# weiji14/deepbedmap

Measured on NVIDIA B200. Metric: continent inference output Mpx/s, higher is better.
Workload: dtype bf16 (fp32 accumulate, fp32 residual stream)

## Files before the change

### deepbedmap_b200/_lib.py

```python
from __future__ import annotations

import ctypes
import os
from typing import Optional

_HERE = os.path.dirname(os.path.abspath(__file__))
LIB_PATH = os.environ.get("DEEPBEDMAP_B200_LIB") or os.path.join(_HERE, "libdeepbedmap_b200.so")

_P, _L, _I, _F = ctypes.c_void_p, ctypes.c_long, ctypes.c_int, ctypes.c_float

SIGNATURES = {
    "dbm_version": [],
    "dbm_launch_count": [],
    "dbm_set_sm_reserve": [_I],
    "dbm_set_deterministic": [_I],
    "dbm_conv2d_fwd_f32": [_P, _L, _P, _P, _P, _L, _I, _I, _I, _I, _I, _I, _I, _I, _I, _P],
    "dbm_conv2d_bwd_data_f32": [_P, _L, _P, _P, _L, _I, _I, _I, _I, _I, _I, _I, _I, _I, _P],
    "dbm_conv2d_bwd_weight_f32": [_P, _L, _P, _L, _P, _I, _I, _I, _I, _I, _I, _I, _I, _P],
    "dbm_bias_grad_f32": [_P, _L, _P, _I, _I, _I, _P],
    "dbm_gemm_f32": [_P, _L, _L, _L, _P, _L, _L, _L, _P, _L, _L, _L, _P, _I, _I, _I, _I, _I, _I, _P],
    "dbm_gemm_bf16": [_P, _L, _L, _L, _P, _L, _L, _L, _P, _L, _L, _L, _P, _I, _I, _I, _I, _I, _I, _P],
    "dbm_axpby_f32": [_P, _L, _P, _L, _P, _L, _F, _F, _I, _L, _P],
    "dbm_lrelu_fwd_f32": [_P, _P, _L, _P],
    "dbm_lrelu_bwd_f32": [_P, _L, _P, _L, _P, _L, _I, _L, _I, _P],
    "dbm_upsample2_fwd_f32": [_P, _P, _L, _I, _I, _P],
    "dbm_upsample2_bwd_f32": [_P, _P, _L, _I, _I, _P],
    "dbm_fill_f32": [_P, _F, _L, _P],
    "dbm_nchw_to_slab8": [_P, _L, _P, _I, _I, _I, _I, _I, _I, _P],
    "dbm_slab8_to_nchw": [_P, _I, _I, _P, _L, _I, _I, _I, _I, _P],
    "dbm_nchw_to_slab4": [_P, _L, _P, _I, _I, _I, _I, _P],
    "dbm_slab4_to_nchw": [_P, _P, _L, _I, _I, _I, _I, _I, _P],
    "dbm_pack_conv3x3_weights": [_P, _P, _I, _I, _I, _I, _P],
    "dbm_pack_conv3x3_weights_slice": [_P, _I, _I, _P, _I, _I, _I, _I, _I, _P],
    "dbm_pack_conv3x3_table": [_P, _I, _L, _P],
    "dbm_trunk_umma": [_P, _I, _I, _I, _I, _P, _I, _P, _P, _I, _P, _P],
    "dbm_trunk_umma_split": [_P, _I, _I, _I, _I, _P, _I, _P, _P, _I, _P, _P],
    "dbm_nchw_to_slab8_split": [_P, _L, _P, _I, _I, _I, _I, _P],
    "dbm_slab8f_to_nchw": [_P, _P, _L, _I, _I, _I, _I, _P],
    "dbm_flat_geometry": [_I, _I, _I, _P],
    "dbm_flat_conv3x3_seq": [_P, _I, _I, _I, _I, _I, _I, _P],
    "dbm_flat_conv3x3_chain": [_P, _P, _I, _I, _I, _I, _I, _I, _P, _P],
    "dbm_trunk_local_fwd": [_P, _I, _I, _I, _I, _P, _P, _P, _P],
    "dbm_trunk_local_bwd": [_P, _I, _I, _I, _I, _P, _P, _P],
    "dbm_flat_wgrad": [_P, _I, _I, _I, _I, _P],
    "dbm_flat_wgrad_ctas": [_P, _I, _I, _I, _I, _I, _P],
    "dbm_flat_wgrad_reduce": [_P, _I, _P],
    "dbm_flat_bias_grad": [_P, _I, _I, _I, _I, _P],
    "dbm_flat_from_nchw": [_P, _I, _P, _P, _F, _I, _I, _I, _P],
    "dbm_flat_to_nchw": [_P, _P, _P, _I, _I, _I, _I, _P],
    "dbm_flat_from_nchw_ex": [_P, _I, _I, _I, _I, _P, _P, _F, _I, _I, _I, _P],
    "dbm_flat_to_nchw_ex": [_P, _P, _P, _I, _I, _I, _I, _I, _I, _I, _P],
    "dbm_transpose_f32": [_P, _P, _I, _I, _P],
    "dbm_stem_fwd_slab8": [_P, _P, _P, _P, _P, _P, _P, _P, _I, _I, _I, _I, _I, _P],
    "dbm_stem_w1_s2d": [_P, _P, _I, _I, _I, _P],
    "dbm_pack_stem_w1": [_P, _P, _P],
    "dbm_conv3x3_umma_valid": [_P, _I, _I, _P, _P, _I, _I, _I, _P, _I, _I, _P],
    "dbm_stem_fwd_flat": [_P, _P, _P, _P, _P, _P, _P, _P, _I, _I, _I, _P],
    "dbm_deform_conv_umma": [_P, _P, _I, _P, _P, _I, _I, _I, _I, _P, _I, _I, _P, _P, _P],
    "dbm_deform_conv_umma_nchw": [_P, _P, _P, _P, _I, _I, _I, _I, _P, _P],
    "dbm_deform_sample_slab8_f32": [_P, _P, _P, _I, _I, _I, _P],
    "dbm_deform_out1_sample": [_P, _P, _I, _P, _P, _I, _I, _I, _P],
    "dbm_deform_conv_out1": [_P, _P, _I, _P, _P, _P, _P, _I, _I, _I, _P],
    "dbm_conv3x3_umma": [_P, _I, _I, _P, _P, _I, _I, _I, _I, _F, _I, _I, _P, _I, _I, _P, _I, _I, _P, _P, _P],
    "dbm_deform_sample_f32": [_P, _P, _P, _I, _I, _I, _I, _P],
    "dbm_deform_bwd_f32": [_P, _P, _P, _P, _P, _I, _I, _I, _I, _P],
    "dbm_deform1_fwd_f32": [_P, _P, _P, _P, _P, _P, _I, _I, _I, _I, _P],
    "dbm_deform1_bwd_f32": [_P, _P, _P, _P, _P, _P, _P, _I, _P, _P, _I, _I, _I, _I, _P],
    "dbm_bn_lrelu_fwd_f32": [_P, _P, _P, _P, _P, _P, _P, _P, _I, _I, _I, _F, _F, _I, _P],
    "dbm_bn_lrelu_bwd_f32": [_P, _P, _P, _P, _P, _P, _P, _P, _P, _P, _I, _I, _I, _P],
    "dbm_bn_lrelu_fwd_groups_f32": [_P, _P, _P, _P, _P, _P, _P, _P, _I, _I, _I, _I, _F, _F, _I, _P],
    "dbm_bn_lrelu_bwd_groups_f32": [_P, _P, _P, _P, _P, _P, _P, _P, _P, _P, _I, _I, _I, _I, _P],
    "dbm_ragan_loss_f32": [_P, _P, _I, _F, _F, _F, _P, _P, _P, _P],
    "dbm_gen_image_loss_f32": [_P, _P, _P, _I, _I, _I, _F, _F, _F, _P, _P, _P],
    "dbm_adam_step_f32": [_P, _P, _P, _P, _L, _F, _F, _F, _F, _I, _F, _P],
    "dbm_adam_step_dev_f32": [_P, _P, _P, _P, _L, _F, _F, _F, _F, _P, _F, _P],
    "dbm_crop_clip_f32": [_P, _I, _I, _P, _I, _I, _I, _I, _I, _I, _P],
    "dbm_place_tile_f32": [_P, _I, _I, _I, _I, _P, _I, _I, _I, _I, _I, _I, _P],
    "dbm_f32_to_i16": [_P, _P, _L, _P],
    "dbm_copy2d_async": [_P, ctypes.c_size_t, _P, ctypes.c_size_t, ctypes.c_size_t, ctypes.c_size_t, _P],
    "dbm_gather_rows_f32": [_P, _L, _P, _P, _L, _I, _P],
    "dbm_gen_create": [_I, _F, _I, ctypes.POINTER(_P)],
    "dbm_gen_destroy": [_P],
    "dbm_gen_count_params": [_P],
    "dbm_gen_num_arrays": [_P],
    "dbm_gen_array_info": [_P, _I, ctypes.POINTER(ctypes.c_char_p), ctypes.POINTER(_I), ctypes.POINTER(_I),
                           ctypes.POINTER(_L)],
    "dbm_gen_set_param": [_P, ctypes.c_char_p, _P, _I, ctypes.POINTER(_I)],
    "dbm_gen_bind_params": [_P, _P],
    "dbm_gen_mark_updated": [_P],
    "dbm_gen_set_precision": [_P, _I],
    "dbm_gen_workspace_bytes": [_P, _I, _I, _I],
    "dbm_gen_forward": [_P, _P, _P, _P, _P, _I, _I, _I, _P, _P, ctypes.c_size_t, _P],
}
TUNING_SIGNATURES = {
    "dbm_debug_set": [_I, _I],
    "dbm_debug_set_ptr": [_I, _P],
    "dbm_flat_debug_set": [_I, _I],
    "dbm_local_debug_set": [_I],
}
RESTYPES = {"dbm_launch_count": _L, "dbm_gen_count_params": _L, "dbm_gen_num_arrays": _I, "dbm_gen_workspace_bytes": ctypes.c_size_t}

_lib: Optional[ctypes.CDLL] = None
launch_count = 0


class DeepBedMapError(RuntimeError):
    pass


def load() -> ctypes.CDLL:
    global _lib
    if _lib is not None:
        return _lib
    if not os.path.exists(LIB_PATH):
        raise DeepBedMapError(
            f"{LIB_PATH} is missing: build it with `python -m deepbedmap_b200.build` "
            "(nvcc, sm_100a). deepbedmap_b200 has no CPU or PyTorch fallback.")
    lib = ctypes.CDLL(LIB_PATH)
    lib.dbm_last_error.restype = ctypes.c_char_p
    lib.dbm_last_error.argtypes = []
    for name, args in list(SIGNATURES.items()) + list(TUNING_SIGNATURES.items()):
        try:
            fn = getattr(lib, name)
        except AttributeError:
            if os.environ.get("DEEPBEDMAP_B200_LIB"):
                continue
            raise
        fn.argtypes = args
        fn.restype = RESTYPES.get(name, ctypes.c_int)
    _lib = lib
    return lib


def kernel_launches() -> int:
    return int(load().dbm_launch_count())


def call(name: str, *args) -> None:
    global launch_count
    lib = load()
    rc = getattr(lib, name)(*args)
    launch_count += 1
    if rc != 0:
        msg = lib.dbm_last_error().decode("utf-8", "replace")
        if rc == -1:
            raise ValueError(f"{name}: {msg}")
        raise DeepBedMapError(f"{name}: {msg}")
```

### deepbedmap_b200/build.py

```python
from __future__ import annotations

import hashlib
import os
import shutil
import subprocess
import sys

HERE = os.path.dirname(os.path.abspath(__file__))
CSRC = os.path.join(HERE, "csrc")
INCLUDE = os.path.join(os.path.dirname(HERE), "include")
LIB = os.path.join(HERE, "libdeepbedmap_b200.so")
TUNING_LIB = os.path.join(HERE, "libdeepbedmap_b200_tuning.so")
STAMP = os.path.join(HERE, "build", "stamp.txt")

SOURCES = ["ops.cu", "gemm_f32.cu", "gemm_bf16.cu", "umma_conv3x3.cu", "umma_trunk.cu", "umma_flat.cu", "umma_local.cu", "umma_deform.cu", "stem.cu", "deform_f32.cu", "train_ops.cu", "gen_api.cu"]
TUNING_SOURCES = ["debug_bench.cu"]
NVCC_FLAGS = [
    "-O3", "-std=c++17", "-gencode", "arch=compute_100a,code=sm_100a", "-lineinfo", "-Xcompiler", "-fPIC"]


def _nvcc() -> str:
    cand = shutil.which("nvcc") or "/usr/local/cuda/bin/nvcc"
    if not os.path.exists(cand):
        raise RuntimeError("nvcc not found; cannot build libdeepbedmap_b200.so")
    return cand


def _digest() -> str:
    h = hashlib.sha256()
    files = [os.path.join(CSRC, f) for f in sorted(os.listdir(CSRC))] + [os.path.join(INCLUDE, "deepbedmap_b200.h")]
    for f in files:
        with open(f, "rb") as fh:
            h.update(f.encode())
            h.update(fh.read())
    h.update(" ".join(NVCC_FLAGS).encode())
    return h.hexdigest()


def build(force: bool = False, verbose: bool = False) -> str:
    os.makedirs(os.path.join(HERE, "build"), exist_ok=True)
    digest = _digest()
    if not force and os.path.exists(LIB) and os.path.exists(STAMP) and open(STAMP).read().strip() == digest:
        return LIB
    nvcc = _nvcc()
    objs = []
    procs = []
    for src in SOURCES:
        obj = os.path.join(HERE, "build", src.replace(".cu", ".o"))
        cmd = [nvcc, *NVCC_FLAGS, "-I", INCLUDE, "-c", os.path.join(CSRC, src), "-o", obj]
        if verbose:
            cmd.insert(1, "-Xptxas")
            cmd.insert(2, "-v")
        procs.append((src, subprocess.Popen(cmd, stdout=subprocess.PIPE, stderr=subprocess.STDOUT, text=True)))
        objs.append(obj)
    for src, p in procs:
        out, _ = p.communicate()
        if verbose or p.returncode:
            sys.stderr.write(out)
        if p.returncode:
            raise RuntimeError(f"nvcc failed on {src}")
    cmd = [nvcc, "-shared", "-gencode", "arch=compute_100a,code=sm_100a", "-o", LIB, *objs]
    subprocess.run(cmd, check=True)
    for src in TUNING_SOURCES:
        cmd = [nvcc, *NVCC_FLAGS, "-shared", "-I", INCLUDE, os.path.join(CSRC, src), "-o", TUNING_LIB, "-L", HERE,
               "-ldeepbedmap_b200", "-Xlinker", "-rpath", "-Xlinker", "$ORIGIN"]
        subprocess.run(cmd, check=True)
    with open(STAMP, "w") as fh:
        fh.write(digest)
    return LIB


if __name__ == "__main__":
    print(build(force="--force" in sys.argv, verbose="-v" in sys.argv))
```

### deepbedmap_b200/csrc/common.cuh

```cuda
#pragma once
#include <cuda.h>
#include <cuda_bf16.h>
#include <cuda_runtime.h>
#include <stdint.h>
#include <stdio.h>

#include "../../include/deepbedmap_b200.h"

namespace dbm {

void set_error(const char* fmt, ...);
int check_launch(const char* what);

#define DBM_REQUIRE(cond, ...)            \
  do {                                    \
    if (!(cond)) {                        \
      ::dbm::set_error(__VA_ARGS__);      \
      return DBM_ERR_INVALID;             \
    }                                     \
  } while (0)

#define DBM_CUDA(expr)                                                          \
  do {                                                                          \
    cudaError_t _e = (expr);                                                    \
    if (_e != cudaSuccess) {                                                    \
      ::dbm::set_error("%s failed: %s", #expr, cudaGetErrorString(_e));         \
      return DBM_ERR_CUDA;                                                      \
    }                                                                           \
  } while (0)

constexpr float kLreluSlope = 0.2f;

__device__ __forceinline__ float lrelu(float v) { return v >= 0.f ? v : v * kLreluSlope; }

static inline int ceil_div(long a, long b) { return (int)((a + b - 1) / b); }

int num_sms();
bool deterministic();
int det_scratch(size_t bytes, void** out);
int resident_ctas(const void* kernel, int threads, size_t smem, int* resident);
int ensure_dyn_smem(const void* kernel, size_t smem);

__device__ __forceinline__ uint32_t smem_u32(const void* p) {
  return static_cast<uint32_t>(__cvta_generic_to_shared(p));
}

__device__ __forceinline__ void mbar_init(uint64_t* bar, uint32_t count) {
  asm volatile("mbarrier.init.shared::cta.b64 [%0], %1;" ::"r"(smem_u32(bar)), "r"(count));
}
__device__ __forceinline__ void fence_mbar_init() {
  asm volatile("fence.mbarrier_init.release.cluster;" ::: "memory");
}
__device__ __forceinline__ void fence_proxy_async_smem() {
  asm volatile("fence.proxy.async.shared::cta;" ::: "memory");
}
__device__ __forceinline__ void mbar_arrive_expect_tx(uint64_t* bar, uint32_t bytes) {
  asm volatile("mbarrier.arrive.expect_tx.shared::cta.b64 _, [%0], %1;" ::"r"(smem_u32(bar)),
               "r"(bytes)
               : "memory");
}
__device__ __forceinline__ void mbar_arrive(uint64_t* bar) {
  asm volatile("mbarrier.arrive.shared::cta.b64 _, [%0];" ::"r"(smem_u32(bar)) : "memory");
}
__device__ __forceinline__ bool mbar_try_wait(uint64_t* bar, uint32_t parity) {
  uint32_t ok;
  asm volatile(
      "{\n\t.reg .pred p;\n\t"
      "mbarrier.try_wait.parity.shared::cta.b64 p, [%1], %2;\n\t"
      "selp.u32 %0, 1, 0, p;\n\t}"
      : "=r"(ok)
      : "r"(smem_u32(bar)), "r"(parity)
      : "memory");
  return ok != 0;
}
__device__ __forceinline__ unsigned long long globaltimer_ns() {
  unsigned long long t;
  asm volatile("mov.u64 %0, %%globaltimer;" : "=l"(t));
  return t;
}
struct SpinGuard {
  uint32_t spins = 0;
  unsigned long long t0 = 0;
  __device__ __forceinline__ bool expired() {
    if ((++spins & 1023u) != 0) return false;
    const unsigned long long now = globaltimer_ns();
    if (t0 == 0) { t0 = now; return false; }
    return now - t0 > 20000000000ull;
  }
};

__device__ __forceinline__ void mbar_wait(uint64_t* bar, uint32_t parity) {
  uint32_t spins = 0;
  while (!mbar_try_wait(bar, parity)) {
    if (++spins > (1u << 26)) {
      printf("dbm: mbarrier wait timeout block %d thread %d\n", blockIdx.x, threadIdx.x);
      __trap();
    }
  }
}

__device__ __forceinline__ void tma_prefetch_desc(const void* tmap) {
  asm volatile("prefetch.tensormap [%0];" ::"l"(tmap) : "memory");
}
__device__ __forceinline__ void tma_load_4d(void* dst, const void* tmap, uint64_t* bar, int c0, int c1,
                                            int c2, int c3) {
  asm volatile(
      "cp.async.bulk.tensor.4d.shared::cluster.global.tile.mbarrier::complete_tx::bytes "
      "[%0], [%1, {%3, %4, %5, %6}], [%2];" ::"r"(smem_u32(dst)),
      "l"(tmap), "r"(smem_u32(bar)), "r"(c0), "r"(c1), "r"(c2), "r"(c3)
      : "memory");
}
__device__ __forceinline__ void bulk_load(void* dst, const void* src, uint32_t bytes, uint64_t* bar) {
  asm volatile(
      "cp.async.bulk.shared::cluster.global.mbarrier::complete_tx::bytes [%0], [%1], %2, [%3];" ::"r"(
          smem_u32(dst)),
      "l"(src), "r"(bytes), "r"(smem_u32(bar))
      : "memory");
}

template <uint32_t kCols>
__device__ __forceinline__ void tmem_alloc(uint32_t* dst_smem) {
  asm volatile("tcgen05.alloc.cta_group::1.sync.aligned.shared::cta.b32 [%0], %1;" ::"r"(
                   smem_u32(dst_smem)),
               "n"(kCols)
               : "memory");
  asm volatile("tcgen05.relinquish_alloc_permit.cta_group::1.sync.aligned;" ::: "memory");
}
template <uint32_t kCols>
__device__ __forceinline__ void tmem_dealloc(uint32_t taddr) {
  asm volatile("tcgen05.dealloc.cta_group::1.sync.aligned.b32 %0, %1;" ::"r"(taddr), "n"(kCols)
               : "memory");
}
__device__ __forceinline__ void tc_fence_before() {
  asm volatile("tcgen05.fence::before_thread_sync;" ::: "memory");
}
__device__ __forceinline__ void tc_fence_after() {
  asm volatile("tcgen05.fence::after_thread_sync;" ::: "memory");
}
__device__ __forceinline__ void umma_bf16(uint32_t d_tmem, uint64_t adesc, uint64_t bdesc, uint32_t idesc,
                                          uint32_t accumulate) {
  asm volatile(
      "{\n\t.reg .pred p;\n\t"
      "setp.ne.b32 p, %4, 0;\n\t"
      "tcgen05.mma.cta_group::1.kind::f16 [%0], %1, %2, %3, p;\n\t}" ::"r"(d_tmem),
      "l"(adesc), "l"(bdesc), "r"(idesc), "r"(accumulate)
      : "memory");
}
template <uint32_t kAOff, uint32_t kBOff>
__device__ __forceinline__ void umma_bf16_off(uint32_t d_tmem, uint32_t a_lo, uint32_t a_hi, uint32_t b_lo,
                                              uint32_t b_hi, uint32_t idesc, uint32_t accumulate) {
  asm volatile(
      "{\n\t.reg .pred p;\n\t.reg .b32 alo, blo;\n\t.reg .b64 ad, bd;\n\t"
      "setp.ne.b32 p, %6, 0;\n\t"
      "add.u32 alo, %1, %7;\n\t"
      "add.u32 blo, %3, %8;\n\t"
      "mov.b64 ad, {alo, %2};\n\t"
      "mov.b64 bd, {blo, %4};\n\t"
      "tcgen05.mma.cta_group::1.kind::f16 [%0], ad, bd, %5, p;\n\t}" ::"r"(d_tmem),
      "r"(a_lo), "r"(a_hi), "r"(b_lo), "r"(b_hi), "r"(idesc), "r"(accumulate), "n"(kAOff), "n"(kBOff)
      : "memory");
}
__device__ __forceinline__ void umma_commit(uint64_t* bar) {
  asm volatile("tcgen05.commit.cta_group::1.mbarrier::arrive::one.shared::cluster.b64 [%0];" ::"r"(
                   smem_u32(bar))
               : "memory");
}
__device__ __forceinline__ void tmem_ld_32x32b_x32(uint32_t taddr, uint32_t (&r)[32]) {
  asm volatile(
      "tcgen05.ld.sync.aligned.32x32b.x32.b32 "
      "{%0, %1, %2, %3, %4, %5, %6, %7, %8, %9, %10, %11, %12, %13, %14, %15, "
      "%16, %17, %18, %19, %20, %21, %22, %23, %24, %25, %26, %27, %28, %29, %30, %31}, [%32];"
      : "=r"(r[0]), "=r"(r[1]), "=r"(r[2]), "=r"(r[3]), "=r"(r[4]), "=r"(r[5]), "=r"(r[6]), "=r"(r[7]),
        "=r"(r[8]), "=r"(r[9]), "=r"(r[10]), "=r"(r[11]), "=r"(r[12]), "=r"(r[13]), "=r"(r[14]),
        "=r"(r[15]), "=r"(r[16]), "=r"(r[17]), "=r"(r[18]), "=r"(r[19]), "=r"(r[20]), "=r"(r[21]),
        "=r"(r[22]), "=r"(r[23]), "=r"(r[24]), "=r"(r[25]), "=r"(r[26]), "=r"(r[27]), "=r"(r[28]),
        "=r"(r[29]), "=r"(r[30]), "=r"(r[31])
      : "r"(taddr)
      : "memory");
}
__device__ __forceinline__ void tmem_wait_ld() {
  asm volatile("tcgen05.wait::ld.sync.aligned;" ::: "memory");
}

__device__ __forceinline__ bool elect_one_sync() {
  uint32_t pred = 0;
  asm volatile(
      "{\n\t.reg .pred P1;\n\t"
      "elect.sync _|P1, 0xFFFFFFFF;\n\t"
      "@P1 mov.s32 %0, 1;\n\t}"
      : "+r"(pred));
  return pred != 0;
}
__device__ __forceinline__ uint64_t make_desc(uint32_t lo, uint32_t hi) {
  return ((uint64_t)hi << 32) | (uint64_t)lo;
}
__device__ __forceinline__ uint32_t desc_lo(uint32_t saddr, uint32_t lbo_bytes) {
  return ((saddr & 0x3FFFFu) >> 4) | (((lbo_bytes >> 4) & 0x3FFFu) << 16);
}
__host__ __device__ constexpr uint32_t desc_hi(uint32_t sbo_bytes) {
  return ((sbo_bytes >> 4) & 0x3FFFu) | (1u << 14);
}

__device__ __forceinline__ uint64_t umma_desc_kmajor_noswz(uint32_t saddr, uint32_t lbo_bytes,
                                                           uint32_t sbo_bytes) {
  uint64_t d = 0;
  d |= (uint64_t)((saddr & 0x3FFFFu) >> 4);
  d |= (uint64_t)((lbo_bytes >> 4) & 0x3FFF) << 16;
  d |= (uint64_t)((sbo_bytes >> 4) & 0x3FFF) << 32;
  d |= (uint64_t)1 << 46;
  return d;
}
__host__ __device__ constexpr uint32_t umma_idesc_bf16(uint32_t M, uint32_t N) {
  return (1u << 4) | (1u << 7) | (1u << 10) | ((N >> 3) << 17) | ((M >> 4) << 24);
}

}
```

### deepbedmap_b200/csrc/gen_api.cu

```cuda
#include <cstring>
#include <map>
#include <string>
#include <vector>

#include "umma_common.cuh"

namespace dbm {

struct GenParam {
  std::string key;
  int ndim;
  int dims[4];
  long off, n;
};

struct ImageRef {
  size_t off = 0;
};

struct Gen {
  int nb = 12, inter = 32;
  float beta = 0.1f;
  int dev = 0;
  std::vector<GenParam> params;
  std::map<std::string, int> index;
  long total = 0;
  float* flat = nullptr;
  bool owns_flat = false;
  uint8_t* arena = nullptr;
  size_t arena_bytes = 0;
  PackEntry* pack_dev = nullptr;
  int pack_n = 0;
  long pack_max = 0;
  bool stale = true;
  std::map<std::string, size_t> img;
  size_t off_wts = 0, off_bias128 = 0, off_w1tc = 0, off_bias_off1 = 0, off_bias_off2 = 0;
  int precision = 0;
  uint8_t* arena_s = nullptr;
  size_t arena_s_bytes = 0;
  PackEntry* pack_s_dev = nullptr;
  int pack_s_n = 0;
  long pack_s_max = 0;
  bool stale_s = true;
  std::map<std::string, size_t> img_s;
  const void* tab_ws = nullptr;
  int tab_n = 0, tab_h = 0, tab_w = 0, tab_layers = 0, tab_precision = -1;
  bool tab_paired = false;
  std::vector<TrunkLayer> tab_host;
};

static const float* P(const Gen* g, const std::string& key) {
  auto it = g->index.find(key);
  return it == g->index.end() ? nullptr : g->flat + g->params[it->second].off;
}

static void add_param(Gen* g, const std::string& key, int d0, int d1 = 0, int d2 = 0, int d3 = 0) {
  GenParam p;
  p.key = key;
  p.dims[0] = d0; p.dims[1] = d1; p.dims[2] = d2; p.dims[3] = d3;
  p.ndim = d1 == 0 ? 1 : 4;
  p.n = p.ndim == 1 ? d0 : (long)d0 * d1 * d2 * d3;
  p.off = g->total;
  g->total += p.n;
  g->index[key] = (int)g->params.size();
  g->params.push_back(p);
}

static void build_inventory(Gen* g) {
  const int ic = g->inter;
  const char* stem[4] = {"X", "W1", "W2", "W3"};
  const int sc[4] = {1, 1, 2, 1}, sk[4] = {3, 30, 6, 3};
  for (int i = 0; i < 4; ++i) {
    add_param(g, std::string("input_block/conv_on_") + stem[i] + "/W", 32, sc[i], sk[i], sk[i]);
    add_param(g, std::string("input_block/conv_on_") + stem[i] + "/b", 32);
  }
  add_param(g, "pre_residual_conv_layer/W", 64, 128, 3, 3);
  add_param(g, "pre_residual_conv_layer/b", 64);
  for (int i = 0; i < g->nb; ++i)
    for (int r = 1; r <= 3; ++r) {
      const std::string pre = "residual_network/" + std::to_string(i) + "/residual_dense_block" + std::to_string(r);
      for (int k = 1; k <= 4; ++k) {
        add_param(g, pre + "/conv_layer" + std::to_string(k) + "/W", ic, 64 + (k - 1) * ic, 3, 3);
        add_param(g, pre + "/conv_layer" + std::to_string(k) + "/b", ic);
      }
      add_param(g, pre + "/conv_layer5/W", 64, 64 + 4 * ic, 3, 3);
      add_param(g, pre + "/conv_layer5/b", 64);
    }
  const char* plain[3] = {"post_residual_conv_layer", "post_upsample_conv_layer_1", "post_upsample_conv_layer_2"};
  for (int i = 0; i < 3; ++i) {
    add_param(g, std::string(plain[i]) + "/W", 64, 64, 3, 3);
    add_param(g, std::string(plain[i]) + "/b", 64);
  }
  const char* fin[2] = {"final_conv_layer1", "final_conv_layer2"};
  const int oc[2] = {64, 1};
  for (int i = 0; i < 2; ++i) {
    add_param(g, std::string(fin[i]) + "/offset_conv/W", 18, 64, 3, 3);
    add_param(g, std::string(fin[i]) + "/offset_conv/b", 18);
    add_param(g, std::string(fin[i]) + "/deform_conv/W", oc[i], 64, 3, 3);
    add_param(g, std::string(fin[i]) + "/deform_conv/b", oc[i]);
  }
}

static std::string rdb_prefix(int i, int r) {
  return "residual_network/" + std::to_string(i) + "/residual_dense_block" + std::to_string(r);
}

static int build_pack_plan(Gen* g) {
  std::vector<PackEntry> ent;
  size_t off = 0;
  auto image = [&](const std::string& name, int cin, int coutp) {
    g->img[name] = off;
    off += ((size_t)9 * cin * coutp * 2 + 255) & ~(size_t)255;
    return g->img[name];
  };
  auto entry = [&](const std::string& wkey, size_t img_off, int O, int o0, int cin, int cin_total, int c0, int coutp,
                   int ck) {
    PackEntry e;
    e.w = P(g, wkey);
    e.out = (__nv_bfloat16*)img_off;
    e.O = O; e.o0 = o0; e.Cin = cin; e.CinTotal = cin_total; e.c0 = c0; e.COUTP = coutp; e.CK = ck; e.mode = 0;
    ent.push_back(e);
  };
  const int ic = g->inter;
  entry("pre_residual_conv_layer/W", image("pre", 128, 64), 64, 0, 128, 128, 0, 64, 16);
  for (int i = 0; i < g->nb; ++i)
    for (int r = 1; r <= 3; ++r) {
      const std::string pre = rdb_prefix(i, r);
      for (int k = 1; k <= 4; ++k) {
        const int cin = 64 + (k - 1) * ic;
        entry(pre + "/conv_layer" + std::to_string(k) + "/W", image(pre + "/c" + std::to_string(k), cin, ic), ic, 0, cin,
              cin, 0, ic, 16);
      }
      entry(pre + "/conv_layer5/W", image(pre + "/c5", 64 + 4 * ic, 64), 64, 0, 64 + 4 * ic, 64 + 4 * ic, 0, 64, 16);
      if (ic == 32)
        for (int k = 1; k <= 3; k += 2) {
          const int cin = 64 + (k - 1) * 32;
          const std::string wa = pre + "/conv_layer" + std::to_string(k) + "/W";
          const std::string wb = pre + "/conv_layer" + std::to_string(k + 1) + "/W";
          const size_t both = image(pre + "/pair" + std::to_string(k), cin, 64);
          entry(wa, both, 32, 0, cin, cin, 0, 64, 16);
          entry(wb, both, 32, 32, cin, cin + 32, 0, 64, 16);
          entry(wb, image(pre + "/tail" + std::to_string(k + 1), 32, 32), 32, 0, 32, cin + 32, cin, 32, 16);
        }
    }
  entry("post_residual_conv_layer/W", image("post", 64, 64), 64, 0, 64, 64, 0, 64, 16);
  entry("post_upsample_conv_layer_1/W", image("up1", 64, 64), 64, 0, 64, 64, 0, 64, 32);
  entry("post_upsample_conv_layer_2/W", image("up2", 64, 64), 64, 0, 64, 64, 0, 64, 32);
  entry("final_conv_layer1/offset_conv/W", image("off1", 64, 32), 18, 0, 64, 64, 0, 32, 32);
  entry("final_conv_layer2/offset_conv/W", image("off2", 64, 32), 18, 0, 64, 64, 0, 32, 32);
  entry("final_conv_layer1/deform_conv/W", image("dc1", 64, 64), 64, 0, 64, 64, 0, 64, 64);
  auto raw = [&](size_t bytes) {
    const size_t o = off;
    off += (bytes + 255) & ~(size_t)255;
    return o;
  };
  g->off_wts = raw(90 * 32 * 4);
  g->off_bias128 = raw(128 * 4);
  g->off_w1tc = raw((size_t)9 * 320 * 32 * 2);
  g->off_bias_off1 = raw(32 * 4);
  g->off_bias_off2 = raw(32 * 4);
  g->arena_bytes = off;
  DBM_CUDA(cudaMalloc(&g->arena, g->arena_bytes));
  DBM_CUDA(cudaMemset(g->arena, 0, g->arena_bytes));
  long mx = 0;
  for (auto& e : ent) {
    e.out = (__nv_bfloat16*)(g->arena + (size_t)e.out);
    const long el = (long)9 * e.Cin * e.COUTP;
    if (el > mx) mx = el;
  }
  g->pack_n = (int)ent.size();
  g->pack_max = mx;
  DBM_CUDA(cudaMalloc(&g->pack_dev, ent.size() * sizeof(PackEntry)));
  DBM_CUDA(cudaMemcpy(g->pack_dev, ent.data(), ent.size() * sizeof(PackEntry), cudaMemcpyHostToDevice));
  return DBM_OK;
}

static int refresh_packed(Gen* g, cudaStream_t st) {
  if (!g->stale) return DBM_OK;
  int rc = dbm_pack_conv3x3_table(g->pack_dev, g->pack_n, g->pack_max, st);
  if (rc) return rc;
  float* wts = (float*)(g->arena + g->off_wts);
  float* bias128 = (float*)(g->arena + g->off_bias128);
  if ((rc = dbm_transpose_f32(P(g, "input_block/conv_on_X/W"), wts, 32, 9, st))) return rc;
  if ((rc = dbm_transpose_f32(P(g, "input_block/conv_on_W2/W"), wts + 9 * 32, 32, 72, st))) return rc;
  if ((rc = dbm_transpose_f32(P(g, "input_block/conv_on_W3/W"), wts + 81 * 32, 32, 9, st))) return rc;
  const char* stem[4] = {"X", "W1", "W2", "W3"};
  for (int i = 0; i < 4; ++i)
    DBM_CUDA(cudaMemcpyAsync(bias128 + 32 * i, P(g, std::string("input_block/conv_on_") + stem[i] + "/b"), 32 * 4,
                             cudaMemcpyDeviceToDevice, st));
  DBM_CUDA(cudaMemcpyAsync(g->arena + g->off_bias_off1, P(g, "final_conv_layer1/offset_conv/b"), 18 * 4,
                           cudaMemcpyDeviceToDevice, st));
  DBM_CUDA(cudaMemcpyAsync(g->arena + g->off_bias_off2, P(g, "final_conv_layer2/offset_conv/b"), 18 * 4,
                           cudaMemcpyDeviceToDevice, st));
  if ((rc = dbm_pack_stem_w1(P(g, "input_block/conv_on_W1/W"), g->arena + g->off_w1tc, st))) return rc;
  g->stale = false;
  return DBM_OK;
}

struct WsLayout {
  size_t s2d, s0, cat[2], a1, f32[3], u1, u2, f1, offs, proj, flags, table, total;
  int num_layers, units;
  bool paired;
};

static WsLayout ws_layout(const Gen* g, int n, int h, int w) {
  WsLayout L;
  const size_t H = h - 2, W = w - 2;
  size_t off = 0;
  auto take = [&](size_t bytes) {
    const size_t o = off;
    off += (bytes + 1023) & ~(size_t)1023;
    return o;
  };
  const size_t px = (size_t)n * H * W;
  const int ccs = (64 + 4 * g->inter) / 8;
  L.s2d = take((size_t)n * 40 * h * w * 16);
  L.s0 = take(px * 16 * 16);
  L.cat[0] = take(px * ccs * 16);
  L.cat[1] = take(px * ccs * 16);
  L.a1 = take(px * 64 * 4);
  for (int i = 0; i < 3; ++i) L.f32[i] = take(px * 64 * 4);
  L.u1 = take(px * 4 * 8 * 16);
  L.u2 = take(px * 16 * 8 * 16);
  L.f1 = take(px * 16 * 8 * 16);
  L.offs = take(px * 16 * 8 * 16);
  L.proj = take(px * 16 * 9 * 4);
  L.paired = g->inter == 32 && ((int)W + 15) / 16 + 2 <= 128;
  L.num_layers = 2 + g->nb * 3 * 5;
  L.units = n * (((int)H + 31) / 32) * (((int)W + 15) / 16);
  L.flags = take((size_t)L.num_layers * L.units * 4);
  L.table = take((size_t)L.num_layers * sizeof(TrunkLayer));
  L.total = off;
  return L;
}

static void build_trunk_table(Gen* g, const WsLayout& L, uint8_t* ws) {
  std::vector<TrunkLayer>& T = g->tab_host;
  T.clear();
  auto bf = [&](size_t o) { return (__nv_bfloat16*)(ws + o); };
  auto f32 = [&](size_t o) { return (float*)(ws + o); };
  auto image = [&](const std::string& name) { return (const __nv_bfloat16*)(g->arena + g->img.at(name)); };
  auto layer = [&](const __nv_bfloat16* wq, const float* bias, int cin, int cout, int in_map, int act, float beta,
                   __nv_bfloat16* out, int out_cs_total, int out_cs0, float* out_f32, const float* res1,
                   const float* res2, int up2, int in_cs0, int cout_main, int mode) {
    TrunkLayer t;
    memset(&t, 0, sizeof(t));
    t.wpacked = wq; t.bias = bias; t.out_bf16 = out; t.out_f32 = out_f32; t.res1 = res1; t.res2 = res2;
    t.stash_out = nullptr;
    t.cin = cin; t.cout = cout; t.in_map = in_map; t.in_cs0 = in_cs0; t.act = act; t.up2 = up2;
    t.out_cs_total = out_cs_total; t.out_cs0 = out_cs0; t.cout_main = cout_main; t.res1_cs_total = 16;
    t.beta = beta; t.mode = mode;
    T.push_back(t);
  };
  const int ic = g->inter, cc = 64 + 4 * ic, ccs = cc / 8;
  __nv_bfloat16* cat[2] = {bf(L.cat[0]), bf(L.cat[1])};
  float* a1 = f32(L.a1);
  float* fb[3] = {f32(L.f32[0]), f32(L.f32[1]), f32(L.f32[2])};
  layer(image("pre"), P(g, "pre_residual_conv_layer/b"), 128, 64, 0, 1, 0.f, cat[0], ccs, 0, a1, nullptr, nullptr, 0, 0,
        64, 0);
  int cur = 0, fi = 0;
  float* cur_f32 = a1;
  for (int i = 0; i < g->nb; ++i) {
    float* rrdb_in = cur_f32;
    for (int r = 1; r <= 3; ++r) {
      const std::string pre = rdb_prefix(i, r);
      auto bias = [&](int k) { return P(g, pre + "/conv_layer" + std::to_string(k) + "/b"); };
      if (L.paired) {
        for (int k = 1; k <= 3; k += 2) {
          const int cin = 64 + (k - 1) * ic;
          layer(image(pre + "/pair" + std::to_string(k)), bias(k), cin, 64, 1 + cur, 1, 0.f, cat[cur], ccs, cin / 8,
                nullptr, nullptr, nullptr, 0, 0, 32, 1);
          layer(image(pre + "/tail" + std::to_string(k + 1)), bias(k + 1), 32, 32, 1 + cur, 1, 0.f, cat[cur], ccs,
                cin / 8 + 4, nullptr, nullptr, nullptr, 0, cin / 8, 32, 2);
        }
      } else {
        for (int k = 1; k <= 4; ++k) {
          const int cin = 64 + (k - 1) * ic;
          layer(image(pre + "/c" + std::to_string(k)), bias(k), cin, ic, 1 + cur, 1, 0.f, cat[cur], ccs, cin / 8, nullptr,
                nullptr, nullptr, 0, 0, ic, 0);
        }
      }
      while (fb[fi] == cur_f32 || fb[fi] == rrdb_in) fi = (fi + 1) % 3;
      float* nxt = fb[fi];
      layer(image(pre + "/c5"), bias(5), cc, 64, 1 + cur, 0, g->beta, cat[1 - cur], ccs, 0, nxt, cur_f32,
            r == 3 ? rrdb_in : nullptr, 0, 0, 64, 0);
      cur = 1 - cur;
      cur_f32 = nxt;
    }
  }
  layer(image("post"), P(g, "post_residual_conv_layer/b"), 64, 64, 1 + cur, 0, 1.f, bf(L.u1), 8, 0, nullptr, a1, nullptr,
        1, 0, 64, 0);
}

static int build_split_pack_plan(Gen* g) {
  if (g->arena_s) return DBM_OK;
  std::vector<PackEntry> ent;
  size_t off = 0;
  auto image = [&](const std::string& name, int cin, int coutp) {
    g->img_s[name] = off;
    off += ((size_t)3 * 9 * cin * coutp * 2 + 255) & ~(size_t)255;
    return g->img_s[name];
  };
  auto entry = [&](const std::string& wkey, size_t img_off, int O, int o0, int cin, int cin_total, int c0, int coutp) {
    PackEntry e;
    e.w = P(g, wkey);
    e.out = (__nv_bfloat16*)img_off;
    e.O = O; e.o0 = o0; e.Cin = cin; e.CinTotal = cin_total; e.c0 = c0; e.COUTP = coutp; e.CK = 16; e.mode = 16;
    ent.push_back(e);
  };
  const int ic = g->inter, cc = 64 + 4 * ic;
  entry("pre_residual_conv_layer/W", image("pre", 128, 64), 64, 0, 128, 128, 0, 64);
  for (int i = 0; i < g->nb; ++i)
    for (int r = 1; r <= 3; ++r) {
      const std::string pre = rdb_prefix(i, r);
      entry(pre + "/conv_layer5/W", image(pre + "/c5", cc, 64), 64, 0, cc, cc, 0, 64);
      if (ic == 32) {
        for (int k = 1; k <= 3; k += 2) {
          const int cin = 64 + (k - 1) * 32;
          const std::string wa = pre + "/conv_layer" + std::to_string(k) + "/W";
          const std::string wb = pre + "/conv_layer" + std::to_string(k + 1) + "/W";
          const size_t both = image(pre + "/pair" + std::to_string(k), cin, 64);
          entry(wa, both, 32, 0, cin, cin, 0, 64);
          entry(wb, both, 32, 32, cin, cin + 32, 0, 64);
          entry(wb, image(pre + "/tail" + std::to_string(k + 1), 32, 32), 32, 0, 32, cin + 32, cin, 32);
        }
      } else {
        for (int k = 1; k <= 4; ++k) {
          const int cin = 64 + (k - 1) * ic;
          entry(pre + "/conv_layer" + std::to_string(k) + "/W", image(pre + "/c" + std::to_string(k), cin, ic), ic, 0, cin,
                cin, 0, ic);
        }
      }
    }
  entry("post_residual_conv_layer/W", image("post", 64, 64), 64, 0, 64, 64, 0, 64);
  entry("post_upsample_conv_layer_1/W", image("up1", 64, 64), 64, 0, 64, 64, 0, 64);
  entry("post_upsample_conv_layer_2/W", image("up2", 64, 64), 64, 0, 64, 64, 0, 64);
  g->arena_s_bytes = off;
  DBM_CUDA(cudaMalloc(&g->arena_s, off));
  DBM_CUDA(cudaMemset(g->arena_s, 0, off));
  long mx = 0;
  for (auto& e : ent) {
    e.out = (__nv_bfloat16*)(g->arena_s + (size_t)e.out);
    const long el = (long)9 * e.Cin * e.COUTP;
    if (el > mx) mx = el;
  }
  g->pack_s_n = (int)ent.size();
  g->pack_s_max = mx;
  DBM_CUDA(cudaMalloc(&g->pack_s_dev, ent.size() * sizeof(PackEntry)));
  DBM_CUDA(cudaMemcpy(g->pack_s_dev, ent.data(), ent.size() * sizeof(PackEntry), cudaMemcpyHostToDevice));
  g->stale_s = true;
  return DBM_OK;
}

struct WsSplit {
  size_t a0, s0, cat[2], a1, f32[3], u1, u2, c2f, c2, off, cols, d1, proj, flags[3], table[3], total;
  int num_layers, units[3];
  bool paired;
};

static WsSplit ws_layout_split(const Gen* g, int n, int h, int w) {
  WsSplit L;
  const size_t H = h - 2, W = w - 2;
  size_t off = 0;
  auto take = [&](size_t bytes) {
    const size_t o = off;
    off += (bytes + 1023) & ~(size_t)1023;
    return o;
  };
  const size_t px = (size_t)n * H * W, px1 = 16 * H * W;
  const int ccs = (64 + 4 * g->inter) / 8;
  L.a0 = take(px * 128 * 4);
  L.s0 = take(px * 32 * 16);
  L.cat[0] = take(px * 2 * ccs * 16);
  L.cat[1] = take(px * 2 * ccs * 16);
  L.a1 = take(px * 64 * 4);
  for (int i = 0; i < 3; ++i) L.f32[i] = take(px * 64 * 4);
  L.u1 = take(px * 4 * 16 * 16);
  L.u2 = take(px * 16 * 16 * 16);
  L.c2f = take(px * 16 * 64 * 4);
  L.c2 = take(px1 * 64 * 4);
  L.off = take(px1 * 18 * 4);
  L.cols = take(px1 * 576 * 4);
  L.d1 = take(px1 * 64 * 4);
  L.proj = take(px1 * 9 * 4);
  L.paired = g->inter == 32 && ((int)W + 15) / 16 + 2 <= 128;
  L.num_layers = 2 + g->nb * 3 * 5;
  for (int i = 0; i < 3; ++i) {
    const int hh = (int)H << i, ww = (int)W << i;
    L.units[i] = n * ((hh + 31) / 32) * ((ww + 15) / 16);
  }
  L.flags[0] = take((size_t)L.num_layers * L.units[0] * 4);
  L.flags[1] = take((size_t)L.units[1] * 4);
  L.flags[2] = take((size_t)L.units[2] * 4);
  L.table[0] = take((size_t)L.num_layers * sizeof(TrunkLayer));
  L.table[1] = take(sizeof(TrunkLayer));
  L.table[2] = take(sizeof(TrunkLayer));
  L.total = off;
  return L;
}

static int build_split_tables(Gen* g, const WsSplit& L, uint8_t* ws, std::vector<TrunkLayer>& T) {
  T.clear();
  auto bf = [&](size_t o) { return (__nv_bfloat16*)(ws + o); };
  auto f32 = [&](size_t o) { return (float*)(ws + o); };
  auto image = [&](const std::string& name) { return (const __nv_bfloat16*)(g->arena_s + g->img_s.at(name)); };
  auto layer = [&](const __nv_bfloat16* wq, const float* bias, int cin, int cout, int in_map, int act, float beta,
                   __nv_bfloat16* out, int out_cs_total, int out_cs0, float* out_f32, const float* res1,
                   const float* res2, int up2, int in_cs0, int cout_main, int mode) {
    TrunkLayer t;
    memset(&t, 0, sizeof(t));
    t.wpacked = wq; t.bias = bias; t.out_bf16 = out; t.out_f32 = out_f32; t.res1 = res1; t.res2 = res2;
    t.cin = cin; t.cout = cout; t.in_map = in_map; t.in_cs0 = in_cs0; t.act = act; t.up2 = up2;
    t.out_cs_total = out_cs_total; t.out_cs0 = out_cs0; t.cout_main = cout_main; t.res1_cs_total = 16;
    t.beta = beta; t.mode = mode;
    T.push_back(t);
  };
  const int ic = g->inter, cc = 64 + 4 * ic, ccs = cc / 8;
  DBM_REQUIRE(L.paired || ic != 32, "gen_forward (bf16x3): tiles wider than ~2000 px are not supported");
  __nv_bfloat16* cat[2] = {bf(L.cat[0]), bf(L.cat[1])};
  float* a1 = f32(L.a1);
  float* fb[3] = {f32(L.f32[0]), f32(L.f32[1]), f32(L.f32[2])};
  layer(image("pre"), P(g, "pre_residual_conv_layer/b"), 128, 64, 0, 1, 0.f, cat[0], ccs, 0, a1, nullptr, nullptr, 0, 0,
        64, 0);
  int cur = 0, fi = 0;
  float* cur_f32 = a1;
  for (int i = 0; i < g->nb; ++i) {
    float* rrdb_in = cur_f32;
    for (int r = 1; r <= 3; ++r) {
      const std::string pre = rdb_prefix(i, r);
      auto bias = [&](int k) { return P(g, pre + "/conv_layer" + std::to_string(k) + "/b"); };
      if (ic == 32) {
        for (int k = 1; k <= 3; k += 2) {
          const int cin = 64 + (k - 1) * ic;
          layer(image(pre + "/pair" + std::to_string(k)), bias(k), cin, 64, 1 + cur, 1, 0.f, cat[cur], ccs, cin / 8,
                nullptr, nullptr, nullptr, 0, 0, 32, 1);
          layer(image(pre + "/tail" + std::to_string(k + 1)), bias(k + 1), 32, 32, 1 + cur, 1, 0.f, cat[cur], ccs,
                cin / 8 + 4, nullptr, nullptr, nullptr, 0, cin / 8, 32, 2);
        }
      } else {
        for (int k = 1; k <= 4; ++k) {
          const int cin = 64 + (k - 1) * ic;
          layer(image(pre + "/c" + std::to_string(k)), bias(k), cin, ic, 1 + cur, 1, 0.f, cat[cur], ccs, cin / 8, nullptr,
                nullptr, nullptr, 0, 0, ic, 0);
        }
// ... 106 lines not shown
  Gen* g = &h->g;
  g->nb = num_residual_blocks; g->beta = residual_scaling; g->inter = inter_channels;
  cudaGetDevice(&g->dev);
  build_inventory(g);
  cudaError_t e = cudaMalloc(&g->flat, (size_t)g->total * 4);
  if (e != cudaSuccess) {
    delete h;
    set_error("gen_create: cudaMalloc of %ld parameters failed: %s", g->total, cudaGetErrorString(e));
    return DBM_ERR_CUDA;
  }
  cudaMemset(g->flat, 0, (size_t)g->total * 4);
  g->owns_flat = true;
  int rc = build_pack_plan(g);
  if (rc) {
    cudaFree(g->flat);
    delete h;
    return rc;
  }
  *out = h;
  return DBM_OK;
}

extern "C" int dbm_gen_destroy(dbm_gen* h) {
  if (!h) return DBM_OK;
  Gen* g = &h->g;
  if (g->owns_flat && g->flat) cudaFree(g->flat);
  if (g->arena) cudaFree(g->arena);
  if (g->pack_dev) cudaFree(g->pack_dev);
  if (g->arena_s) cudaFree(g->arena_s);
  if (g->pack_s_dev) cudaFree(g->pack_s_dev);
  delete h;
  return DBM_OK;
}

extern "C" long dbm_gen_count_params(const dbm_gen* h) { return h ? h->g.total : -1; }
extern "C" int dbm_gen_num_arrays(const dbm_gen* h) { return h ? (int)h->g.params.size() : -1; }

extern "C" int dbm_gen_array_info(const dbm_gen* h, int index, const char** key, int* ndim, int* dims4,
                                  long* flat_offset) {
  DBM_REQUIRE(h && index >= 0 && index < (int)h->g.params.size(), "gen_array_info: bad index %d", index);
  const GenParam& p = h->g.params[index];
  if (key) *key = p.key.c_str();
  if (ndim) *ndim = p.ndim;
  if (dims4)
    for (int i = 0; i < 4; ++i) dims4[i] = p.dims[i];
  if (flat_offset) *flat_offset = p.off;
  return DBM_OK;
}

extern "C" int dbm_gen_set_param(dbm_gen* h, const char* key, const float* host_values, int ndim, const int* dims) {
  DBM_REQUIRE(h && key && host_values && dims, "gen_set_param: null argument");
  Gen* g = &h->g;
  auto it = g->index.find(key);
  DBM_REQUIRE(it != g->index.end(), "gen_set_param: unknown key '%s'", key);
  const GenParam& p = g->params[it->second];
  bool ok = ndim == p.ndim;
  for (int i = 0; ok && i < ndim; ++i) ok = dims[i] == p.dims[i];
  DBM_REQUIRE(ok, "gen_set_param: '%s' has shape (%d,%d,%d,%d), got %d-d (%d,...)", key, p.dims[0], p.dims[1],
              p.dims[2], p.dims[3], ndim, ndim > 0 ? dims[0] : 0);
  DBM_CUDA(cudaMemcpy(g->flat + p.off, host_values, (size_t)p.n * 4, cudaMemcpyHostToDevice));
  g->stale = true;
  g->stale_s = true;
  return DBM_OK;
}

extern "C" int dbm_gen_bind_params(dbm_gen* h, float* device_flat) {
  DBM_REQUIRE(h && device_flat, "gen_bind_params: null argument");
  Gen* g = &h->g;
  DBM_REQUIRE(g->owns_flat, "gen_bind_params: parameters are already bound");
  cudaFree(g->flat);
  std::vector<PackEntry> ent(g->pack_n);
  DBM_CUDA(cudaMemcpy(ent.data(), g->pack_dev, ent.size() * sizeof(PackEntry), cudaMemcpyDeviceToHost));
  for (auto& e : ent) e.w = device_flat + (e.w - g->flat);
  DBM_CUDA(cudaMemcpy(g->pack_dev, ent.data(), ent.size() * sizeof(PackEntry), cudaMemcpyHostToDevice));
  if (g->pack_s_dev) {
    std::vector<PackEntry> es(g->pack_s_n);
    DBM_CUDA(cudaMemcpy(es.data(), g->pack_s_dev, es.size() * sizeof(PackEntry), cudaMemcpyDeviceToHost));
    for (auto& e : es) e.w = device_flat + (e.w - g->flat);
    DBM_CUDA(cudaMemcpy(g->pack_s_dev, es.data(), es.size() * sizeof(PackEntry), cudaMemcpyHostToDevice));
  }
  g->flat = device_flat;
  g->owns_flat = false;
  g->stale = true;
  g->stale_s = true;
  g->tab_ws = nullptr;
  return DBM_OK;
}

extern "C" int dbm_gen_mark_updated(dbm_gen* h) {
  DBM_REQUIRE(h != nullptr, "gen_mark_updated: null handle");
  h->g.stale = true;
  h->g.stale_s = true;
  return DBM_OK;
}

extern "C" int dbm_gen_set_precision(dbm_gen* h, int precision) {
  DBM_REQUIRE(h != nullptr, "gen_set_precision: null handle");
  DBM_REQUIRE(precision == 0 || precision == 1, "gen_set_precision: %d (0 = bf16, 1 = bf16x3)", precision);
  h->g.precision = precision;
  h->g.tab_ws = nullptr;
  return DBM_OK;
}

extern "C" size_t dbm_gen_workspace_bytes(const dbm_gen* h, int n, int h_in, int w_in) {
  if (!h || n <= 0 || h_in < 3 || w_in < 3) return 0;
  if (h->g.precision == 1) return ws_layout_split(&h->g, n, h_in, w_in).total;
  return ws_layout(&h->g, n, h_in, w_in).total;
}

extern "C" int dbm_gen_forward(dbm_gen* h, const float* x, const float* w1, const float* w2, const float* w3, int n,
                               int h_in, int w_in, float* y_out, void* workspace, size_t workspace_bytes,
                               cudaStream_t st) {
  DBM_REQUIRE(h && x && w1 && w2 && w3 && y_out && workspace, "gen_forward: null argument");
  DBM_REQUIRE(n > 0 && h_in >= 3 && w_in >= 3, "gen_forward: input %d x %d x %d too small (need >= 3 x 3)", n, h_in, w_in);
  Gen* g = &h->g;
  DBM_REQUIRE(((uintptr_t)workspace & 1023) == 0, "gen_forward: workspace must be 1024-byte aligned");
  if (g->precision == 1)
    return gen_forward_split(g, x, w1, w2, w3, n, h_in, w_in, y_out, workspace, workspace_bytes, st);
  const WsLayout L = ws_layout(g, n, h_in, w_in);
  DBM_REQUIRE(workspace_bytes >= L.total, "gen_forward: workspace of %zu bytes, need %zu (dbm_gen_workspace_bytes)",
              workspace_bytes, L.total);
  DBM_REQUIRE(((uintptr_t)workspace & 1023) == 0, "gen_forward: workspace must be 1024-byte aligned");
  uint8_t* ws = (uint8_t*)workspace;
  const int H = h_in - 2, W = w_in - 2;
  int rc = refresh_packed(g, st);
  if (rc) return rc;
  if (g->tab_ws != workspace || g->tab_n != n || g->tab_h != h_in || g->tab_w != w_in || g->tab_precision != 0) {
    build_trunk_table(g, L, ws);
    DBM_REQUIRE((int)g->tab_host.size() == L.num_layers, "gen_forward: pass table has %zu entries, expected %d",
                g->tab_host.size(), L.num_layers);
    DBM_CUDA(cudaMemcpyAsync(ws + L.table, g->tab_host.data(), g->tab_host.size() * sizeof(TrunkLayer),
                             cudaMemcpyHostToDevice, st));
    DBM_CUDA(cudaStreamSynchronize(st));
    g->tab_ws = workspace; g->tab_n = n; g->tab_h = h_in; g->tab_w = w_in; g->tab_precision = 0;
  }
  void* s2d = ws + L.s2d;
  void* s0 = ws + L.s0;
  const float* wts = (const float*)(g->arena + g->off_wts);
  const float* bias128 = (const float*)(g->arena + g->off_bias128);
  auto image = [&](const char* name) { return (const void*)(g->arena + g->img.at(name)); };
  if ((rc = dbm_stem_w1_s2d(w1, s2d, n, h_in, w_in, st))) return rc;
  if ((rc = dbm_stem_fwd_slab8(x, nullptr, w2, w3, nullptr, wts, bias128, s0, 16, 0, n, h_in, w_in, st))) return rc;
  if ((rc = dbm_conv3x3_umma_valid(s2d, 40, 320, g->arena + g->off_w1tc, P(g, "input_block/conv_on_W1/b"), n, h_in, w_in,
                                   s0, 16, 4, st)))
    return rc;
  const int ccs = (64 + 4 * g->inter) / 8;
  if ((rc = dbm_trunk_umma(ws + L.table, L.num_layers, n, H, W, s0, 16, ws + L.cat[0], ws + L.cat[1], ccs,
                           (unsigned int*)(ws + L.flags), st)))
    return rc;
  void* u1 = ws + L.u1;
  void* u2 = ws + L.u2;
  void* f1 = ws + L.f1;
  float* offs = (float*)(ws + L.offs);
  if ((rc = dbm_conv3x3_umma(u1, 8, 64, image("up1"), P(g, "post_upsample_conv_layer_1/b"), 64, n, 2 * H, 2 * W, 0.f, 1, 1,
                             u2, 8, 0, nullptr, 0, 0, nullptr, nullptr, st)))
    return rc;
  if ((rc = dbm_conv3x3_umma(u2, 8, 64, image("up2"), P(g, "post_upsample_conv_layer_2/b"), 64, n, 4 * H, 4 * W, 0.f, 1, 0,
                             f1, 8, 0, nullptr, 0, 0, nullptr, nullptr, st)))
    return rc;
  if ((rc = dbm_conv3x3_umma(f1, 8, 64, image("off1"), (const float*)(g->arena + g->off_bias_off1), 32, n, 4 * H, 4 * W,
                             0.f, 0, 0, nullptr, 0, 0, offs, 8, 0, nullptr, nullptr, st)))
    return rc;
  void* d1 = u2;
  if ((rc = dbm_deform_conv_umma(f1, offs, 8, image("dc1"), P(g, "final_conv_layer1/deform_conv/b"), n, 4 * H, 4 * W, 1, d1,
                                 8, 0, nullptr, nullptr, st)))
    return rc;
  if ((rc = dbm_conv3x3_umma(d1, 8, 64, image("off2"), (const float*)(g->arena + g->off_bias_off2), 32, n, 4 * H, 4 * W,
                             0.f, 0, 0, nullptr, 0, 0, offs, 8, 0, nullptr, nullptr, st)))
    return rc;
  return dbm_deform_conv_out1(d1, offs, 8, P(g, "final_conv_layer2/deform_conv/W"), P(g, "final_conv_layer2/deform_conv/b"),
                              y_out, (float*)(ws + L.proj), n, 4 * H, 4 * W, st);
}
```

### deepbedmap_b200/csrc/umma_common.cuh

```cuda
#pragma once
#include <utility>

#include "common.cuh"

namespace dbm {

constexpr int kTile = 16;
constexpr int kHalo = kTile + 2;

int make_slab8_tmap(CUtensorMap* tm, const void* base, int N, int CS, int H, int W, int ck, int box_w = kHalo,
                    int box_h = kHalo);

template <int COUT, int CK, int DSTRIDE, int IDX>
__device__ __forceinline__ void issue_one(uint32_t d0, uint32_t a_lo, uint32_t a_hi, uint32_t b_lo, uint32_t b_hi,
                                          uint32_t idesc, uint32_t acc) {
  constexpr int KS = CK / 16;
  constexpr int j = IDX / KS, ks = IDX % KS;
  constexpr uint32_t a_off = (uint32_t)((2 * ks) * kHalo * kHalo + 8 * j);
  constexpr uint32_t b_off = (uint32_t)((2 * ks) * (COUT / 8) * 8);
  umma_bf16_off<a_off, b_off>(d0 + (uint32_t)(j * DSTRIDE), a_lo, a_hi, b_lo, b_hi, idesc, ks != 0 ? 1u : acc);
}
template <int COUT, int CK, int DSTRIDE, int... IDX>
__device__ __forceinline__ void issue_tap(uint32_t d0, uint32_t a_lo, uint32_t a_hi, uint32_t b_lo, uint32_t b_hi,
                                          uint32_t idesc, uint32_t acc, std::integer_sequence<int, IDX...>) {
  (issue_one<COUT, CK, DSTRIDE, IDX>(d0, a_lo, a_hi, b_lo, b_hi, idesc, acc), ...);
}
template <int COUT, int CK, int DSTRIDE = COUT>
__device__ __forceinline__ void issue_stage_mmas(uint32_t d0, uint32_t a_lo, uint32_t a_hi, uint32_t b_lo,
                                                 uint32_t b_hi, uint32_t idesc, uint32_t acc0) {
  constexpr uint32_t kBTap = (uint32_t)((CK / 8) * (COUT / 8) * 8);
#pragma unroll 1
  for (uint32_t tap = 0; tap < 9; ++tap) {
    const uint32_t a_tap = a_lo + tap + (tap / 3) * (kHalo - 3);
    const uint32_t b_tap = b_lo + tap * kBTap;
    issue_tap<COUT, CK, DSTRIDE>(d0, a_tap, a_hi, b_tap, b_hi, idesc, tap != 0 ? 1u : acc0,
                        std::make_integer_sequence<int, 2 * (CK / 16)>{});
  }
}


struct TrunkLayer {
  const __nv_bfloat16* wpacked;
  const float* bias;
  __nv_bfloat16* out_bf16;
  float* out_f32;
  const float* res1;
  const float* res2;
  float* stash_out;
  int cin, cout;
  int in_map, in_cs0;
  int act, up2;
  int out_cs_total, out_cs0;
  int cout_main, res1_cs_total;
  float beta;
  int mode;
  int pad[6];
};
static_assert(sizeof(TrunkLayer) == 128, "TrunkLayer layout is part of the C ABI");


struct PackEntry {
  const float* w;
  __nv_bfloat16* out;
  int O, o0, Cin, CinTotal, c0, COUTP, CK, mode;
};
static_assert(sizeof(PackEntry) == 48, "PackEntry layout is part of the C ABI");


}
```

### deepbedmap_b200/csrc/umma_conv3x3.cu

```cuda
#include "umma_common.cuh"

namespace dbm {

static int g_debug_swap_lbo_sbo = 0;
static int g_debug_ck16 = 0;
extern int g_trunk_debug;

constexpr int kThreads = 192;

struct UmmaConvParams {
  int N, H, W, Cin;
  int tiles_x, tiles_y, num_items;
  const __nv_bfloat16* wpacked;
  const float* bias;
  float beta;
  int act, up2, swap;
  int in_off;
  __nv_bfloat16* out_bf16;
  int out_cs_total, out_cs0;
  float* out_f32;
  int out_f32_cs_total, out_f32_cs0;
  const float* res1;
  const float* res2;
};
// ... 127 lines not shown
            if (p.res1) {
#pragma unroll
              for (int s4 = 0; s4 < 8; ++s4) {
                const float4 rr = __ldg(reinterpret_cast<const float4*>(
                    p.res1 + ((((size_t)n * (COUT / 4) + (c0 / 4 + s4)) * p.H + y) * p.W + x) * 4));
                v[4 * s4 + 0] = rr.x + p.beta * v[4 * s4 + 0];
                v[4 * s4 + 1] = rr.y + p.beta * v[4 * s4 + 1];
                v[4 * s4 + 2] = rr.z + p.beta * v[4 * s4 + 2];
                v[4 * s4 + 3] = rr.w + p.beta * v[4 * s4 + 3];
              }
            }
            if (p.res2) {
#pragma unroll
              for (int s4 = 0; s4 < 8; ++s4) {
                const float4 rr = __ldg(reinterpret_cast<const float4*>(
                    p.res2 + ((((size_t)n * (COUT / 4) + (c0 / 4 + s4)) * p.H + y) * p.W + x) * 4));
                v[4 * s4 + 0] = rr.x + p.beta * v[4 * s4 + 0];
                v[4 * s4 + 1] = rr.y + p.beta * v[4 * s4 + 1];
                v[4 * s4 + 2] = rr.z + p.beta * v[4 * s4 + 2];
                v[4 * s4 + 3] = rr.w + p.beta * v[4 * s4 + 3];
              }
            }
            if (p.act) {
#pragma unroll
              for (int i = 0; i < 32; ++i) v[i] = lrelu(v[i]);
            }
            if (p.out_f32) {
#pragma unroll
              for (int s4 = 0; s4 < 8; ++s4) {
                float4 o = make_float4(v[4 * s4], v[4 * s4 + 1], v[4 * s4 + 2], v[4 * s4 + 3]);
                *reinterpret_cast<float4*>(
                    p.out_f32 +
                    ((((size_t)n * p.out_f32_cs_total + (p.out_f32_cs0 + c0 / 4 + s4)) * p.H + y) * p.W + x) * 4) = o;
              }
            }
            if (p.out_bf16) {
#pragma unroll
              for (int s8 = 0; s8 < 4; ++s8) {
                uint4 o;
                __nv_bfloat162 t0 = __floats2bfloat162_rn(v[8 * s8 + 0], v[8 * s8 + 1]);
                __nv_bfloat162 t1 = __floats2bfloat162_rn(v[8 * s8 + 2], v[8 * s8 + 3]);
                __nv_bfloat162 t2 = __floats2bfloat162_rn(v[8 * s8 + 4], v[8 * s8 + 5]);
                __nv_bfloat162 t3 = __floats2bfloat162_rn(v[8 * s8 + 6], v[8 * s8 + 7]);
                o.x = *reinterpret_cast<uint32_t*>(&t0);
                o.y = *reinterpret_cast<uint32_t*>(&t1);
                o.z = *reinterpret_cast<uint32_t*>(&t2);
                o.w = *reinterpret_cast<uint32_t*>(&t3);
                const size_t cs = (size_t)n * p.out_cs_total + (p.out_cs0 + c0 / 8 + s8);
                if (!p.up2) {
                  *reinterpret_cast<uint4*>(p.out_bf16 + ((cs * p.H + y) * p.W + x) * 8) = o;
                } else {
                  const int Ho = 2 * p.H, Wo = 2 * p.W;
                  __nv_bfloat16* base = p.out_bf16 + ((cs * Ho + 2 * y) * Wo + 2 * x) * 8;
                  *reinterpret_cast<uint4*>(base) = o;
                  *reinterpret_cast<uint4*>(base + 8) = o;
                  *reinterpret_cast<uint4*>(base + (size_t)Wo * 8) = o;
                  *reinterpret_cast<uint4*>(base + (size_t)Wo * 8 + 8) = o;
                }
              }
            }
          }
        }
      }
      tc_fence_before();
      __syncwarp();
      if (lane == 0) mbar_arrive(&tempty[buf]);
    }
  }

  tc_fence_before();
  __syncthreads();
  if (warp == 1) {
    tc_fence_after();
    tmem_dealloc<Cfg::TMEM_COLS>(tmem_base);
  }
}

typedef CUresult (*PFN_encodeTiled)(CUtensorMap*, CUtensorMapDataType, cuuint32_t, void*, const cuuint64_t*,
                                    const cuuint64_t*, const cuuint32_t*, const cuuint32_t*,
                                    CUtensorMapInterleave, CUtensorMapSwizzle, CUtensorMapL2promotion,
                                    CUtensorMapFloatOOBfill);

static PFN_encodeTiled get_encode() {
  static PFN_encodeTiled fn = nullptr;
  if (!fn) {
    void* p = nullptr;
    cudaDriverEntryPointQueryResult qres;
    if (cudaGetDriverEntryPoint("cuTensorMapEncodeTiled", &p, cudaEnableDefault, &qres) == cudaSuccess &&
        qres == cudaDriverEntryPointSuccess)
      fn = (PFN_encodeTiled)p;
  }
  return fn;
}

int make_slab8_tmap(CUtensorMap* tm, const void* base, int N, int CS, int H, int W, int ck, int box_w, int box_h) {
  PFN_encodeTiled enc = get_encode();
  DBM_REQUIRE(enc != nullptr, "cuTensorMapEncodeTiled entry point not available");
  cuuint64_t dims[4] = {(cuuint64_t)W * 8, (cuuint64_t)H, (cuuint64_t)CS, (cuuint64_t)N};
  cuuint64_t strides[3] = {(cuuint64_t)W * 16, (cuuint64_t)H * W * 16, (cuuint64_t)CS * H * W * 16};
  cuuint32_t box[4] = {(cuuint32_t)box_w * 8, (cuuint32_t)box_h, (cuuint32_t)(ck / 8), 1};
  cuuint32_t estr[4] = {1, 1, 1, 1};
  CUresult r = enc(tm, CU_TENSOR_MAP_DATA_TYPE_BFLOAT16, 4, const_cast<void*>(base), dims, strides, box, estr,
                   CU_TENSOR_MAP_INTERLEAVE_NONE, CU_TENSOR_MAP_SWIZZLE_NONE, CU_TENSOR_MAP_L2_PROMOTION_L2_256B,
                   CU_TENSOR_MAP_FLOAT_OOB_FILL_NONE);
  DBM_REQUIRE(r == CUDA_SUCCESS, "cuTensorMapEncodeTiled failed (%d) for N=%d CS=%d H=%d W=%d", (int)r, N, CS,
              H, W);
  return DBM_OK;
}

template <int COUT, int CK, int STAGES>
static int launch_umma(const CUtensorMap& tm, const UmmaConvParams& p, cudaStream_t st) {
  using Cfg = UmmaCfg<COUT, CK, STAGES>;
  if (int rc = ensure_dyn_smem((const void*)umma_conv3x3_kernel<COUT, CK, STAGES>, Cfg::SMEM)) return rc;
  int grid = p.num_items < num_sms() ? p.num_items : num_sms();
  umma_conv3x3_kernel<COUT, CK, STAGES><<<grid, kThreads, Cfg::SMEM, st>>>(tm, p);
  return check_launch("umma_conv3x3_kernel");
}

__global__ void pack_w3x3_slice_kernel(const float* __restrict__ w, __nv_bfloat16* __restrict__ out, int O, int o0,
                                       int Cin, int CinTotal, int c0, int COUTP, int CK) {
  const long total = (long)9 * Cin * COUTP;
  for (long i = blockIdx.x * (long)blockDim.x + threadIdx.x; i < total; i += (long)gridDim.x * blockDim.x) {
    long t = i;
    const int c8 = t % 8; t /= 8;
    const int o8 = t % 8; t /= 8;
    const int cg = t % (COUTP / 8); t /= (COUTP / 8);
    const int ksl = t % (CK / 8); t /= (CK / 8);
    const int tap = t % 9; t /= 9;
    const int kc = (int)t;
    const int o = cg * 8 + o8 - o0;
    const int c = kc * CK + ksl * 8 + c8;
    if (o >= 0 && o < O) out[i] = __float2bfloat16_rn(w[((long)o * CinTotal + c0 + c) * 9 + tap]);
  }
}

__device__ __forceinline__ void store8_bf16(__nv_bfloat16* dst, const float (&v)[8]) {
  __nv_bfloat162 t0 = __floats2bfloat162_rn(v[0], v[1]);
  __nv_bfloat162 t1 = __floats2bfloat162_rn(v[2], v[3]);
  __nv_bfloat162 t2 = __floats2bfloat162_rn(v[4], v[5]);
  __nv_bfloat162 t3 = __floats2bfloat162_rn(v[6], v[7]);
  uint4 o;
  o.x = *reinterpret_cast<uint32_t*>(&t0);
  o.y = *reinterpret_cast<uint32_t*>(&t1);
  o.z = *reinterpret_cast<uint32_t*>(&t2);
  o.w = *reinterpret_cast<uint32_t*>(&t3);
  *reinterpret_cast<uint4*>(dst) = o;
}

__global__ void pack_w3x3_table_kernel(const PackEntry* __restrict__ table) {
  PackEntry e = table[blockIdx.y];
  const bool split = (e.mode & 16) != 0;
  e.mode &= 15;
  if (split && !(e.mode == 0 && (e.O & 7) == 0 && (e.o0 & 7) == 0 && e.CK == 16)) return;
  if (e.mode == 0 && (e.O & 7) == 0 && (e.o0 & 7) == 0) {
    const int og = e.O / 8;
    const long total = (long)9 * (e.Cin / 8) * e.O;
    for (long i = blockIdx.x * (long)blockDim.x + threadIdx.x; i < total; i += (long)gridDim.x * blockDim.x) {
      long t = i;
      const int o8 = t % 8; t /= 8;
      const int cgl = t % og; t /= og;
      const int ksl = t % (e.CK / 8); t /= (e.CK / 8);
      const int tap = t % 9; t /= 9;
      const int kc = (int)t;
      const int o = cgl * 8 + o8;
      const int c = kc * e.CK + ksl * 8;
      const int kcd = split ? 3 * kc : kc;
      const long dst = ((((long)(kcd * 9 + tap) * (e.CK / 8) + ksl) * (e.COUTP / 8) + (e.o0 / 8 + cgl)) * 8 + o8) * 8;
      const float* src = e.w + ((long)o * e.CinTotal + e.c0 + c) * 9 + tap;
      float v[8];
#pragma unroll
      for (int c8 = 0; c8 < 8; ++c8) v[c8] = src[c8 * 9];
      store8_bf16(e.out + dst, v);
      if (split) {
        const long chunk = (long)9 * (e.CK / 8) * (e.COUTP / 8) * 64;
        store8_bf16(e.out + dst + chunk, v);
#pragma unroll
        for (int c8 = 0; c8 < 8; ++c8) v[c8] -= __bfloat162float(__float2bfloat16_rn(v[c8]));
        store8_bf16(e.out + dst + 2 * chunk, v);
      }
    }
    return;
  }
  const long total = (long)9 * (e.Cin / 8) * e.COUTP;
  for (long i = blockIdx.x * (long)blockDim.x + threadIdx.x; i < total; i += (long)gridDim.x * blockDim.x) {
    long t = i;
    const int o8 = t % 8; t /= 8;
    const int cg = t % (e.COUTP / 8); t /= (e.COUTP / 8);
    const int ksl = t % (e.CK / 8); t /= (e.CK / 8);
    const int tap = t % 9; t /= 9;
    const int kc = (int)t;
    const int on = cg * 8 + o8;
    const int cb = kc * e.CK + ksl * 8;
    float v[8];
    if (e.mode == 0) {
      const int o = on - e.o0;
      if (o < 0 || o >= e.O) continue;
      const float* src = e.w + ((long)o * e.CinTotal + e.c0 + cb) * 9 + tap;
#pragma unroll
      for (int c8 = 0; c8 < 8; ++c8) v[c8] = src[c8 * 9];
      store8_bf16(e.out + i * 8, v);
      continue;
    }
#pragma unroll
    for (int c8 = 0; c8 < 8; ++c8) {
      const int c = cb + c8;
      float x = 0.f;
      if (e.mode == 1) {
        const int kvalid = e.o0 > 0 ? e.o0 : e.Cin;
        if (on < e.O && c < kvalid) x = e.w[((long)c * e.CinTotal + e.c0 + on) * 9 + (8 - tap)];
      } else {
        const int oc = e.mode == 2 ? on : c;
        const int pc = e.mode == 2 ? c : e.c0 + on;
        const int ovalid = e.o0 > 0 ? e.o0 : (e.mode == 2 ? e.O : e.Cin);
        const int t3 = e.mode == 2 ? tap : 8 - tap;
        const int ph = pc / e.CinTotal, cc = pc - ph * e.CinTotal;
        const int ky = 2 * (t3 / 3 - 1) + (ph >> 1) + 1, kx = 2 * (t3 % 3 - 1) + (ph & 1) + 1;
        if (on < e.O && oc < ovalid && ph < 4 && ky >= 0 && ky <= 3 && kx >= 0 && kx <= 3)
          x = e.w[(((long)oc * e.CinTotal + cc) * 4 + ky) * 4 + kx];
      }
      v[c8] = x;
    }
    store8_bf16(e.out + i * 8, v);
  }
}

__global__ void pack_w3x3_kernel(const float* __restrict__ w, __nv_bfloat16* __restrict__ out, int O, int Cin,
                                 int COUTP, int CK) {
  const long total = (long)9 * Cin * COUTP;
  for (long i = blockIdx.x * (long)blockDim.x + threadIdx.x; i < total; i += (long)gridDim.x * blockDim.x) {
    long t = i;
    const int c8 = t % 8; t /= 8;
    const int o8 = t % 8; t /= 8;
    const int cg = t % (COUTP / 8); t /= (COUTP / 8);
    const int ksl = t % (CK / 8); t /= (CK / 8);
    const int tap = t % 9; t /= 9;
    const int kc = (int)t;
    const int o = cg * 8 + o8;
    const int c = kc * CK + ksl * 8 + c8;
    float v = 0.f;
    if (o < O) v = w[((long)o * Cin + c) * 9 + tap];
    out[i] = __float2bfloat16_rn(v);
  }
}

}

using namespace dbm;

extern "C" int dbm_debug_set(int key, int value) {
  if (key == 1) g_debug_swap_lbo_sbo = value;
  if (key == 2) g_debug_ck16 = value;
  if (key == 3) g_trunk_debug = value;
  return DBM_OK;
}

extern "C" int dbm_pack_conv3x3_weights(const float* w_oihw, void* packed_bf16, int cout, int cin, int cout_padded,
                                        int ck, cudaStream_t stream) {
  DBM_REQUIRE(ck == 16 || ck == 32 || ck == 64,
              "pack: K-chunk %d must be 16 / 32 (conv3x3_umma, trunk) or 64 (deform_conv_umma)", ck);
  DBM_REQUIRE(cin % ck == 0, "pack: Cin=%d must be a multiple of %d", cin, ck);
  DBM_REQUIRE(cout_padded == 32 || cout_padded == 64, "pack: padded Cout=%d must be 32 or 64", cout_padded);
  DBM_REQUIRE(cout <= cout_padded, "pack: Cout=%d > padded %d", cout, cout_padded);
  const long total = (long)9 * cin * cout_padded;
  pack_w3x3_kernel<<<ceil_div(total, 256), 256, 0, stream>>>(w_oihw, (__nv_bfloat16*)packed_bf16, cout, cin,
                                                             cout_padded, ck);
  return check_launch("pack_w3x3_kernel");
}

extern "C" int dbm_pack_conv3x3_weights_slice(const float* w_oihw, int w_cin_total, int w_c0, void* packed_bf16,
                                              int cout, int cout0, int cin, int cout_padded, int ck,
                                              cudaStream_t stream) {
  DBM_REQUIRE(ck == 16 || ck == 32 || ck == 64, "pack: K-chunk %d must be 16, 32 or 64", ck);
  DBM_REQUIRE(cin % ck == 0 && w_c0 >= 0 && w_c0 + cin <= w_cin_total, "pack: bad channel slice [%d, %d) of %d",
              w_c0, w_c0 + cin, w_cin_total);
  DBM_REQUIRE(cout_padded % 8 == 0 && cout0 >= 0 && cout0 + cout <= cout_padded, "pack: bad Cout rows [%d, %d) of %d",
              cout0, cout0 + cout, cout_padded);
  const long total = (long)9 * cin * cout_padded;
  pack_w3x3_slice_kernel<<<ceil_div(total, 256), 256, 0, stream>>>(w_oihw, (__nv_bfloat16*)packed_bf16, cout, cout0,
                                                                   cin, w_cin_total, w_c0, cout_padded, ck);
  return check_launch("pack_w3x3_slice_kernel");
}

extern "C" int dbm_pack_conv3x3_table(const void* table_dev, int num_entries, long max_elements,
                                      cudaStream_t stream) {
  DBM_REQUIRE(num_entries > 0 && num_entries <= 65535 && max_elements > 0, "pack table: bad size (%d entries)",
              num_entries);
  DBM_REQUIRE(((uintptr_t)table_dev & 7) == 0, "pack table: unaligned");
  int gx = ceil_div(max_elements / 8, 256 * 2);
  if (gx > 64) gx = 64;
  if (gx < 1) gx = 1;
  pack_w3x3_table_kernel<<<dim3(gx, num_entries), 256, 0, stream>>>((const PackEntry*)table_dev);
  return check_launch("pack_w3x3_table_kernel");
}

extern "C" int dbm_conv3x3_umma(const void* in_slab8, int in_cs_total, int cin, const void* wpacked,
                                const float* bias, int cout_padded, int n, int h, int w, float beta, int act,
                                int up2, void* out_slab8, int out_cs_total, int out_cs0, float* out_f32_slab4,
                                int out_f32_cs_total, int out_f32_cs0, const float* res1_slab4,
                                const float* res2_slab4, cudaStream_t stream) {
  DBM_REQUIRE(cin % 32 == 0 && cin <= in_cs_total * 8, "conv3x3_umma: bad Cin=%d (slabs %d)", cin, in_cs_total);
  DBM_REQUIRE(cout_padded == 32 || cout_padded == 64, "conv3x3_umma: Cout=%d must be 32 or 64", cout_padded);
  DBM_REQUIRE(n > 0 && h > 0 && w > 0, "conv3x3_umma: empty input");
  DBM_REQUIRE(out_slab8 || out_f32_slab4, "conv3x3_umma: no output");
  DBM_REQUIRE(((uintptr_t)in_slab8 & 15) == 0 && ((uintptr_t)wpacked & 15) == 0, "conv3x3_umma: unaligned");
  CUtensorMap tm;
  int rc = make_slab8_tmap(&tm, in_slab8, n, in_cs_total, h, w, 32);
// ... 44 lines not shown
```

### deepbedmap_b200/csrc/umma_local.cu

```cuda
#include "common.cuh"

namespace dbm {

constexpr int kLocThreads = 320;
constexpr int kLocStages = 5;
constexpr int kLocSoloThreads = 192;
constexpr int kLocSoloStages = 3;
constexpr int kLocStageBytes = 96 * 192;
constexpr int kLocSlabs = 24;
constexpr int kLocAcc = 192, kLocXcur = 192, kLocSlot = 256;

enum { kLocPre = 0, kLocAct = 1, kLocRdb = 2, kLocPost = 3,
       kLocBPost = 4, kLocBMask = 5, kLocBD1 = 6, kLocBPre = 7 };

struct LocalPass {
  const __nv_bfloat16* w;
  const float* bias;
  __nv_bfloat16* save;
  float* out_f32;
  const __nv_bfloat16* mask;
  const float* add_f32;
  int slab0, nk, N, col0;
  int type, ecol, out_slab, rr;
  float beta;
  float scale;
  int first;
  int pad;
};
static_assert(sizeof(LocalPass) == 96, "LocalPass layout is part of the C ABI");

struct LocalParams {
  const LocalPass* passes;
  int count;
  int n, H, W, Wp, img, halo, G0, Pg, RA;
  const __nv_bfloat16* s0;
  int in_slabs;
  int group;
  float* x0;
  float* xrr;
};

__device__ __forceinline__ void tmem_st_32x32b_x32(uint32_t taddr, const uint32_t (&r)[32]) {
  asm volatile(
      "tcgen05.st.sync.aligned.32x32b.x32.b32 [%0], "
      "{%1, %2, %3, %4, %5, %6, %7, %8, %9, %10, %11, %12, %13, %14, %15, %16, "
      "%17, %18, %19, %20, %21, %22, %23, %24, %25, %26, %27, %28, %29, %30, %31, %32};" ::"r"(taddr),
      "r"(r[0]), "r"(r[1]), "r"(r[2]), "r"(r[3]), "r"(r[4]), "r"(r[5]), "r"(r[6]), "r"(r[7]), "r"(r[8]), "r"(r[9]),
      "r"(r[10]), "r"(r[11]), "r"(r[12]), "r"(r[13]), "r"(r[14]), "r"(r[15]), "r"(r[16]), "r"(r[17]), "r"(r[18]),
      "r"(r[19]), "r"(r[20]), "r"(r[21]), "r"(r[22]), "r"(r[23]), "r"(r[24]), "r"(r[25]), "r"(r[26]), "r"(r[27]),
      "r"(r[28]), "r"(r[29]), "r"(r[30]), "r"(r[31])
      : "memory");
}
__device__ __forceinline__ void tmem_wait_st() { asm volatile("tcgen05.wait::st.sync.aligned;" ::: "memory"); }

__device__ __forceinline__ uint4 pack8f(const float* v) {
  uint4 o;
  __nv_bfloat162 t0 = __floats2bfloat162_rn(v[0], v[1]);
  __nv_bfloat162 t1 = __floats2bfloat162_rn(v[2], v[3]);
  __nv_bfloat162 t2 = __floats2bfloat162_rn(v[4], v[5]);
  __nv_bfloat162 t3 = __floats2bfloat162_rn(v[6], v[7]);
  o.x = *reinterpret_cast<uint32_t*>(&t0);
  o.y = *reinterpret_cast<uint32_t*>(&t1);
  o.z = *reinterpret_cast<uint32_t*>(&t2);
  o.w = *reinterpret_cast<uint32_t*>(&t3);
  return o;
}

template <bool BWD, bool SOLO>
__global__ void __launch_bounds__(SOLO ? kLocSoloThreads : kLocThreads, SOLO ? 2 : 1)
local_trunk_kernel(const LocalParams p) {
  constexpr int kStages = SOLO ? kLocSoloStages : kLocStages;
  constexpr int kThreads = SOLO ? kLocSoloThreads : kLocThreads;
  constexpr int kSlots = SOLO ? 1 : 2;
  extern __shared__ uint8_t smem_raw[];
  uint8_t* smem = (uint8_t*)(((uintptr_t)smem_raw + 1023) & ~(uintptr_t)1023);
  uint64_t* full = (uint64_t*)smem;
  uint64_t* empty = full + kLocStages;
  uint64_t* tfull = empty + kLocStages;
  uint64_t* act_ready = tfull + 1;
  uint64_t* in_full = act_ready + 1;
  uint64_t* a_free = in_full + 1;
  uint32_t* tmem_slot = (uint32_t*)(a_free + 1);
  const uint32_t slab_bytes = (uint32_t)p.RA * 16u;
  const uint32_t abuf_bytes = (uint32_t)kLocSlabs * slab_bytes;
  uint8_t* abuf = smem + 256;
  uint8_t* stages = abuf + kSlots * abuf_bytes;

  const int warp = threadIdx.x >> 5, lane = threadIdx.x & 31;
  for (uint32_t i = threadIdx.x; i < kSlots * abuf_bytes / 16; i += kThreads)
    reinterpret_cast<uint4*>(abuf)[i] = make_uint4(0, 0, 0, 0);
  fence_proxy_async_smem();
  if (warp == 0 && lane == 0) {
    for (int s = 0; s < kStages; ++s) { mbar_init(&full[s], 1); mbar_init(&empty[s], 1); }
    mbar_init(tfull, 1);
    mbar_init(act_ready, 4 * kSlots);
    mbar_init(in_full, 1);
    mbar_init(a_free, 1);
    fence_mbar_init();
  }
  if (warp == 1) tmem_alloc<SOLO ? 256 : 512>(tmem_slot);
  tc_fence_before();
  __syncthreads();
  tc_fence_after();
  const uint32_t tmem_base = *tmem_slot;
  const int npairs = (p.n + p.group - 1) / p.group;
  const uint32_t load_rows = (uint32_t)(2 * p.halo + p.img);

  if (warp == 0) {
    if (lane == 0) {
      int s = 0; uint32_t ph = 0; int it = 0;
      for (int pair = blockIdx.x; pair < npairs; pair += gridDim.x, ++it) {
        if (it > 0) mbar_wait(a_free, (uint32_t)((it - 1) & 1));
        const int nact = min(p.group, p.n - p.group * pair);
        mbar_arrive_expect_tx(in_full, (uint32_t)(nact * p.in_slabs) * load_rows * 16u);
        for (int g = 0; g < nact; ++g) {
          const long pos0 = (long)p.G0 + (long)(p.group * pair + g) * p.img - p.halo;
          for (int sl = 0; sl < p.in_slabs; ++sl)
            bulk_load(abuf + g * abuf_bytes + sl * slab_bytes, p.s0 + ((long)sl * p.Pg + pos0) * 8, load_rows * 16u,
                      in_full);
        }
        for (int l = 0; l < p.count; ++l) {
          const __nv_bfloat16* w = p.passes[l].w;
          const int nk = p.passes[l].nk;
          const uint32_t bytes = 96u * (uint32_t)p.passes[l].N;
          for (int g3 = 0; g3 < 3 * nk; ++g3) {
            mbar_wait(&empty[s], ph ^ 1);
            mbar_arrive_expect_tx(&full[s], bytes);
            bulk_load(stages + s * kLocStageBytes, w + (size_t)g3 * (bytes / 2), bytes, &full[s]);
            if (++s == kStages) { s = 0; ph ^= 1; }
          }
        }
      }
    }
  } else if (warp == 1) {
    const uint32_t a_hi = desc_hi(128), b_hi = desc_hi(128);
    const uint32_t ab_u = smem_u32(abuf), st_u = smem_u32(stages);
    int s = 0; uint32_t ph = 0, actph = 0; int it = 0; long gp = 0;
    for (int pair = blockIdx.x; pair < npairs; pair += gridDim.x, ++it) {
      const int nact = min(p.group, p.n - p.group * pair);
      mbar_wait(in_full, (uint32_t)(it & 1));
      for (int l = 0; l < p.count; ++l, ++gp) {
        const int N = p.passes[l].N, nk = p.passes[l].nk, slab0 = p.passes[l].slab0, col0 = p.passes[l].col0;
        const int first = p.passes[l].first;
        const uint32_t idesc = umma_idesc_bf16(128, (uint32_t)N);
        const uint32_t b_lbo = (uint32_t)(N / 8) * 128u;
        const uint32_t b_tap = (2u * b_lbo) >> 4;
        if (gp > 0) {
          mbar_wait(act_ready, actph);
          actph ^= 1;
        }
        tc_fence_after();
        for (int kc = 0; kc < nk; ++kc) {
          for (int tg = 0; tg < 3; ++tg) {
            mbar_wait(&full[s], ph);
            tc_fence_after();
            const uint32_t b_lo = desc_lo(st_u + s * kLocStageBytes, b_lbo);
            const bool last = (kc == nk - 1) && (tg == 2);
            if (elect_one_sync()) {
              for (int g = 0; g < nact; ++g) {
                const uint32_t a_lo = desc_lo(ab_u + g * abuf_bytes + (uint32_t)(slab0 + 2 * kc) * slab_bytes, slab_bytes);
                const uint32_t d = tmem_base + (uint32_t)(g * kLocSlot + col0);
#pragma unroll
                for (int t = 0; t < 3; ++t) {
                  const uint32_t a_off = (uint32_t)(tg * p.Wp + t);
                  const uint32_t acc = (first && kc == 0 && tg == 0 && t == 0) ? 0u : 1u;
                  umma_bf16(d, make_desc(a_lo + a_off, a_hi), make_desc(b_lo + (uint32_t)t * b_tap, b_hi), idesc, acc);
                }
              }
              umma_commit(&empty[s]);
              if (last) umma_commit(tfull);
            }
            __syncwarp();
            if (++s == kStages) { s = 0; ph ^= 1; }
          }
        }
      }
      if (elect_one_sync()) umma_commit(a_free);
      __syncwarp();
    }
  } else {
    const int q = warp & 3;
    const int g = (warp - 2) >> 2;
    const int m = 32 * q + lane;
    const int y = m / p.Wp, x = m - y * p.Wp;
    uint8_t* arow = abuf + g * abuf_bytes + (uint32_t)(p.halo + m) * 16u;
    const uint32_t tbase = tmem_base + ((uint32_t)(32 * q) << 16) + (uint32_t)(g * kLocSlot);
    uint32_t tph = 0;
    for (int pair = blockIdx.x; pair < npairs; pair += gridDim.x) {
      const int im = g < p.group ? p.group * pair + g : p.n;
      const bool interior = im < p.n && m < p.img && y >= 1 && y <= p.H && x >= 1 && x <= p.W;
      const long gpos = (long)p.G0 + (long)im * p.img + m;
      float* x0p = p.x0 + ((size_t)im * 16 * 128 + m) * 4;
      float* xrp = p.xrr + ((size_t)im * 16 * 128 + m) * 4;
      if constexpr (BWD) {
        for (int l = 0; l < p.count; ++l) {
          const LocalPass& P = p.passes[l];
          const int type = P.type;
          const int nh = type == kLocBMask ? 1 : (type == kLocBPre ? 4 : 2);
          const bool has_mask = P.mask != nullptr;
          uint4 mk[4];
          if (has_mask && interior) {
#pragma unroll
            for (int s8 = 0; s8 < 4; ++s8)
              mk[s8] = *reinterpret_cast<const uint4*>(P.mask + ((size_t)s8 * p.Pg + gpos) * 8);
          }
          mbar_wait(tfull, tph);
          tph ^= 1;
          tc_fence_after();
          for (int h = 0; h < nh; ++h) {
            uint32_t acc[32];
            float v[32];
            tmem_ld_32x32b_x32(tbase + (uint32_t)(P.ecol + 32 * h), acc);
            if (h == 1 && has_mask && interior) {
#pragma unroll
              for (int s8 = 0; s8 < 4; ++s8)
                mk[s8] = *reinterpret_cast<const uint4*>(P.mask + ((size_t)(4 + s8) * p.Pg + gpos) * 8);
            }
            tmem_wait_ld();
#pragma unroll
            for (int i = 0; i < 32; ++i) v[i] = __uint_as_float(acc[i]);
            if (type == kLocBPre) {
              if (interior) {
#pragma unroll
                for (int c4 = 0; c4 < 8; ++c4)
                  *reinterpret_cast<float4*>(P.out_f32 + ((size_t)(8 * h + c4) * p.Pg + gpos) * 4) =
                      make_float4(v[4 * c4], v[4 * c4 + 1], v[4 * c4 + 2], v[4 * c4 + 3]);
              }
              continue;
            }
            if (type == kLocBD1) {
              uint32_t xc[32];
              tmem_ld_32x32b_x32(tbase + (uint32_t)(kLocXcur + 32 * h), xc);
              tmem_wait_ld();
#pragma unroll
              for (int i = 0; i < 32; ++i) v[i] = __fmaf_rn(P.beta, __uint_as_float(xc[i]), v[i]);
              if (interior && P.add_f32 != nullptr) {
#pragma unroll
                for (int c4 = 0; c4 < 8; ++c4) {
                  const float4 t = *reinterpret_cast<const float4*>(P.add_f32 + ((size_t)(8 * h + c4) * p.Pg + gpos) * 4);
                  v[4 * c4] += t.x; v[4 * c4 + 1] += t.y; v[4 * c4 + 2] += t.z; v[4 * c4 + 3] += t.w;
                }
              }
              if (interior && P.rr) {
#pragma unroll
                for (int c4 = 0; c4 < 8; ++c4) {
                  const float4 t = *reinterpret_cast<const float4*>(xrp + (size_t)(8 * h + c4) * 512);
                  v[4 * c4] += t.x; v[4 * c4 + 1] += t.y; v[4 * c4 + 2] += t.z; v[4 * c4 + 3] += t.w;
                }
              }
            }
            if (has_mask && interior) {
#pragma unroll
              for (int s8 = 0; s8 < 4; ++s8) {
                const uint32_t w4[4] = {mk[s8].x, mk[s8].y, mk[s8].z, mk[s8].w};
#pragma unroll
                for (int j = 0; j < 4; ++j) {
                  if (w4[j] & 0x00008000u) v[8 * s8 + 2 * j] *= kLreluSlope;
                  if (w4[j] & 0x80000000u) v[8 * s8 + 2 * j + 1] *= kLreluSlope;
                }
              }
            }
            if (type == kLocBPost || (type == kLocBD1 && !has_mask)) {
              uint32_t xs[32];
#pragma unroll
              for (int i = 0; i < 32; ++i) xs[i] = __float_as_uint(v[i]);
              tmem_st_32x32b_x32(tbase + (uint32_t)(kLocXcur + 32 * h), xs);
              if (interior && (type == kLocBPost || P.rr)) {
#pragma unroll
                for (int c4 = 0; c4 < 8; ++c4)
                  *reinterpret_cast<float4*>(xrp + (size_t)(8 * h + c4) * 512) =
                      make_float4(v[4 * c4], v[4 * c4 + 1], v[4 * c4 + 2], v[4 * c4 + 3]);
              }
            }
            const float sc = P.scale;
#pragma unroll
            for (int i = 0; i < 32; ++i) v[i] *= sc;
#pragma unroll
            for (int s8 = 0; s8 < 4; ++s8) {
              const uint4 o = pack8f(v + 8 * s8);
              if (interior) {
                *reinterpret_cast<uint4*>(arow + (size_t)(P.out_slab + 4 * h + s8) * slab_bytes) = o;
                if (P.save != nullptr) *reinterpret_cast<uint4*>(P.save + ((size_t)(4 * h + s8) * p.Pg + gpos) * 8) = o;
              }
            }
          }
          tmem_wait_st();
          tc_fence_before();
          fence_proxy_async_smem();
          __syncwarp();
          if (lane == 0) mbar_arrive(act_ready);
        }
        continue;
      }
      for (int l = 0; l < p.count; ++l) {
        const LocalPass& P = p.passes[l];
        const int type = P.type;
        const int nh = type == kLocAct ? 1 : 2;
        float b0[32];
#pragma unroll
        for (int i4 = 0; i4 < 8; ++i4) {
          const float4 t = __ldg(reinterpret_cast<const float4*>(P.bias) + i4);
          b0[4 * i4] = t.x; b0[4 * i4 + 1] = t.y; b0[4 * i4 + 2] = t.z; b0[4 * i4 + 3] = t.w;
        }
        mbar_wait(tfull, tph);
        tph ^= 1;
        tc_fence_after();
        uint4 keep[8];
        for (int h = 0; h < nh; ++h) {
          uint32_t acc[32];
          float v[32];
          tmem_ld_32x32b_x32(tbase + (uint32_t)(P.ecol + 32 * h), acc);
          if (h == 1) {
#pragma unroll
            for (int i4 = 0; i4 < 8; ++i4) {
              const float4 t = __ldg(reinterpret_cast<const float4*>(P.bias) + 8 + i4);
              b0[4 * i4] = t.x; b0[4 * i4 + 1] = t.y; b0[4 * i4 + 2] = t.z; b0[4 * i4 + 3] = t.w;
            }
          }
          tmem_wait_ld();
#pragma unroll
          for (int i = 0; i < 32; ++i) v[i] = __fadd_rn(__uint_as_float(acc[i]), b0[i]);
          if (type == kLocPre || type == kLocAct) {
#pragma unroll
            for (int i = 0; i < 32; ++i) v[i] = lrelu(v[i]);
          }
          if (type == kLocRdb) {
            uint32_t xc[32];
            tmem_ld_32x32b_x32(tbase + (uint32_t)(kLocXcur + 32 * h), xc);
            tmem_wait_ld();
#pragma unroll
            for (int i = 0; i < 32; ++i) v[i] = __fmaf_rn(P.beta, v[i], __uint_as_float(xc[i]));
            if (P.rr) {
              if (interior) {
#pragma unroll
                for (int c4 = 0; c4 < 8; ++c4) {
                  const float4 t = *reinterpret_cast<const float4*>(xrp + (size_t)(8 * h + c4) * 512);
                  v[4 * c4] = __fmaf_rn(P.beta, v[4 * c4], t.x);
                  v[4 * c4 + 1] = __fmaf_rn(P.beta, v[4 * c4 + 1], t.y);
                  v[4 * c4 + 2] = __fmaf_rn(P.beta, v[4 * c4 + 2], t.z);
                  v[4 * c4 + 3] = __fmaf_rn(P.beta, v[4 * c4 + 3], t.w);
                }
              }
            }
          }
          if (type == kLocPost) {
            if (interior) {
#pragma unroll
              for (int c4 = 0; c4 < 8; ++c4) {
                const float4 t = *reinterpret_cast<const float4*>(x0p + (size_t)(8 * h + c4) * 512);
                v[4 * c4] += t.x; v[4 * c4 + 1] += t.y; v[4 * c4 + 2] += t.z; v[4 * c4 + 3] += t.w;
                if (P.out_f32 != nullptr)
                  *reinterpret_cast<float4*>(P.out_f32 + ((size_t)(8 * h + c4) * p.Pg + gpos) * 4) =
                      make_float4(v[4 * c4], v[4 * c4 + 1], v[4 * c4 + 2], v[4 * c4 + 3]);
              }
              if (P.save != nullptr) {
                const int Ho = 2 * p.H, Wo = 2 * p.W;
#pragma unroll
                for (int s8 = 0; s8 < 4; ++s8) {
                  const uint4 o = pack8f(v + 8 * s8);
                  __nv_bfloat16* base =
                      P.save + ((((size_t)im * 8 + 4 * h + s8) * Ho + 2 * (y - 1)) * Wo + 2 * (x - 1)) * 8;
                  *reinterpret_cast<uint4*>(base) = o;
                  *reinterpret_cast<uint4*>(base + 8) = o;
                  *reinterpret_cast<uint4*>(base + (size_t)Wo * 8) = o;
                  *reinterpret_cast<uint4*>(base + (size_t)Wo * 8 + 8) = o;
                }
              }
            }
            continue;
          }
          if (type == kLocPre || type == kLocRdb) {
            uint32_t xs[32];
#pragma unroll
            for (int i = 0; i < 32; ++i) xs[i] = __float_as_uint(v[i]);
            tmem_st_32x32b_x32(tbase + (uint32_t)(kLocXcur + 32 * h), xs);
            if (interior && (type == kLocPre || P.rr)) {
#pragma unroll
              for (int c4 = 0; c4 < 8; ++c4) {
                const float4 t = make_float4(v[4 * c4], v[4 * c4 + 1], v[4 * c4 + 2], v[4 * c4 + 3]);
                *reinterpret_cast<float4*>(xrp + (size_t)(8 * h + c4) * 512) = t;
                if (type == kLocPre) *reinterpret_cast<float4*>(x0p + (size_t)(8 * h + c4) * 512) = t;
              }
            }
          }
#pragma unroll
          for (int s8 = 0; s8 < 4; ++s8) {
            const uint4 o = pack8f(v + 8 * s8);
            keep[4 * h + s8] = o;
            if (interior) *reinterpret_cast<uint4*>(arow + (size_t)(P.out_slab + 4 * h + s8) * slab_bytes) = o;
          }
        }
        tmem_wait_st();
        tc_fence_before();
        fence_proxy_async_smem();
        __syncwarp();
        if (lane == 0) mbar_arrive(act_ready);
        if (P.save != nullptr && interior && type != kLocPost) {
#pragma unroll
          for (int s8 = 0; s8 < 8; ++s8)
            if (s8 < 4 * nh) *reinterpret_cast<uint4*>(P.save + ((size_t)s8 * p.Pg + gpos) * 8) = keep[s8];
        }
      }
    }
  }

  tc_fence_before();
  __syncthreads();
  if (warp == 1) {
    tc_fence_after();
    tmem_dealloc<SOLO ? 256 : 512>(tmem_base);
  }
}

}

using namespace dbm;

static int g_local_group = 0;

static int local_trunk_launch(bool bwd, const void* passes_dev, int count, int n, int h, int w, const void* in_flat,
                              float* x0_scratch, float* xrr_scratch, cudaStream_t stream) {
  const char* who = bwd ? "trunk_local_bwd" : "trunk_local_fwd";
  DBM_REQUIRE(passes_dev && count > 0 && n > 0 && h > 0 && w > 0, "%s: empty problem", who);
  DBM_REQUIRE(in_flat && xrr_scratch && (bwd || x0_scratch), "%s: null buffer", who);
  LocalParams p;
  p.passes = (const LocalPass*)passes_dev;
  p.count = count;
  p.n = n; p.H = h; p.W = w; p.Wp = w + 2; p.img = (h + 2) * (w + 2);
  DBM_REQUIRE(p.img <= 128, "%s: a padded image of %dx%d is %d positions; the image-resident kernel holds at most 128 "
              "(use the flat chain / tiled kernels)", who, h + 2, w + 2, p.img);
  p.halo = p.Wp + 1;
  p.G0 = (p.halo + 7) & ~7;
  const int tiles = (n * p.img + 127) / 128;
  p.Pg = p.G0 + tiles * 128 + p.G0;
  p.s0 = (const __nv_bfloat16*)in_flat; p.in_slabs = bwd ? 8 : 16;
  p.x0 = x0_scratch; p.xrr = xrr_scratch;
  const bool solo = g_local_group == 3 || (g_local_group == 0 && n > num_sms());
  size_t smem;
  if (solo) {
    p.RA = 2 * p.halo + p.img;
    p.group = 1;
    smem = 1024 + 256 + (size_t)kLocSlabs * p.RA * 16 + (size_t)kLocSoloStages * kLocStageBytes;
  } else {
    p.RA = 128 + 2 * p.halo;
    p.group = (g_local_group == 1 || g_local_group == 2) ? g_local_group : 1;
    smem = 1024 + 256 + 2 * (size_t)kLocSlabs * p.RA * 16 + (size_t)kLocStages * kLocStageBytes;
  }
  DBM_REQUIRE(smem <= 227 * 1024, "%s: image width %d needs %zu bytes of shared memory", who, w, smem);
  const void* kfn = bwd ? (solo ? (const void*)local_trunk_kernel<true, true> : (const void*)local_trunk_kernel<true, false>)
                        : (solo ? (const void*)local_trunk_kernel<false, true> : (const void*)local_trunk_kernel<false, false>);
  if (int rc = ensure_dyn_smem(kfn, smem)) return rc;
  const int npairs = (n + p.group - 1) / p.group;
  const int cap = solo ? 2 * num_sms() : num_sms();
  const int grid = npairs < cap ? npairs : cap;
  if (bwd && solo) local_trunk_kernel<true, true><<<grid, kLocSoloThreads, smem, stream>>>(p);
  else if (bwd) local_trunk_kernel<true, false><<<grid, kLocThreads, smem, stream>>>(p);
  else if (solo) local_trunk_kernel<false, true><<<grid, kLocSoloThreads, smem, stream>>>(p);
  else local_trunk_kernel<false, false><<<grid, kLocThreads, smem, stream>>>(p);
  return check_launch(bwd ? "local_trunk_kernel<bwd>" : "local_trunk_kernel<fwd>");
}

extern "C" int dbm_local_debug_set(int value) {
  g_local_group = value;
  return DBM_OK;
}

extern "C" int dbm_trunk_local_fwd(const void* passes_dev, int count, int n, int h, int w, const void* s0_flat,
                                   float* x0_scratch, float* xrr_scratch, cudaStream_t stream) {
  return local_trunk_launch(false, passes_dev, count, n, h, w, s0_flat, x0_scratch, xrr_scratch, stream);
}

extern "C" int dbm_trunk_local_bwd(const void* passes_dev, int count, int n, int h, int w, const void* gpost_flat,
                                   float* dxrr_scratch, cudaStream_t stream) {
  return local_trunk_launch(true, passes_dev, count, n, h, w, gpost_flat, nullptr, dxrr_scratch, stream);
}
```

### deepbedmap_b200/flat.py

```python
from __future__ import annotations

import ctypes

import numpy as np
import torch

from . import ops

EPI_DTYPE = np.dtype([("bias", "<u8"), ("add1", "<u8"), ("add2", "<u8"), ("mask", "<u8"), ("out_f32", "<u8"),
                      ("out_bf16", "<u8"), ("s1", "<f4"), ("beta", "<f4"), ("beta2", "<f4"), ("out_scale", "<f4"),
                      ("act", "<i4"), ("pad", "<i4")])
assert EPI_DTYPE.itemsize == 72
LAUNCH_DTYPE = np.dtype([("in", "<u8"), ("wpacked", "<u8"), ("cin", "<i4"), ("nout", "<i4"), ("ny", "<i4"), ("pad", "<i4"),
                         ("w_chunk_stride", "<i8"), ("blk", EPI_DTYPE, (6,))])
assert LAUNCH_DTYPE.itemsize == 472
WGRAD_UNIT_DTYPE = np.dtype([("act", "<u8"), ("gout", "<u8"), ("partial", "<u8"), ("blk0", "<i4"), ("nblk", "<i4"),
                             ("nslab", "<i4"), ("tapmask", "<i4"), ("pad", "<i4", (2,))])
assert WGRAD_UNIT_DTYPE.itemsize == 48
WGRAD_REDUCE_DTYPE = np.dtype([("partial", "<u8"), ("dw", "<u8"), ("split_stride", "<i8"), ("nsplit", "<i4"),
                               ("cin_total", "<i4"), ("c0", "<i4"), ("o0", "<i4"), ("nch", "<i4"), ("mode", "<i4")])
assert WGRAD_REDUCE_DTYPE.itemsize == 48
BIAS_GRAD_DTYPE = np.dtype([("gout", "<u8"), ("db", "<u8")])
LOCAL_PASS_DTYPE = np.dtype([("w", "<u8"), ("bias", "<u8"), ("save", "<u8"), ("out_f32", "<u8"), ("mask", "<u8"),
                             ("add_f32", "<u8"), ("slab0", "<i4"), ("nk", "<i4"), ("N", "<i4"), ("col0", "<i4"),
                             ("type", "<i4"), ("ecol", "<i4"), ("out_slab", "<i4"), ("rr", "<i4"), ("beta", "<f4"),
                             ("scale", "<f4"), ("first", "<i4"), ("pad", "<i4")])
assert LOCAL_PASS_DTYPE.itemsize == 96
LOC_PRE, LOC_ACT, LOC_RDB, LOC_POST, LOC_BPOST, LOC_BMASK, LOC_BD1, LOC_BPRE = range(8)


def local_trunk_fits(H: int, W: int) -> bool:
    return (H + 2) * (W + 2) <= 128


def local_pass(**kw):
    e = np.zeros((), dtype=LOCAL_PASS_DTYPE)
    e["scale"] = 1.0
    for k, v in kw.items():
        e[k] = v
    return e


def local_forward_table(model, pk, nrdb, beta, cat_ptr=None, out_f32=0, up2_out=0):
    P = model.p
    save = (lambda j, c: cat_ptr(j, c)) if cat_ptr is not None else (lambda j, c: 0)
    passes = [local_pass(w=pk["pre_residual_conv_layer@trunk"][0].data_ptr(),
                         bias=P["pre_residual_conv_layer/b"].data_ptr(), save=save(0, 0), slab0=0, nk=8, N=64, col0=0,
                         type=LOC_PRE, ecol=0, out_slab=0, first=1)]
    for j in range(nrdb):
        r = j % 3 + 1
        pre = model._rdb_prefix(j // 3, r)
        for s in range(5):
            last = s == 4
            passes.append(local_pass(
                w=pk[f"{pre}/stat{s}"].data_ptr(), bias=P[f"{pre}/conv_layer{s + 1}/b"].data_ptr(),
                save=save(j + 1, 0) if last else save(j, 64 + 32 * s), slab0=0 if s == 0 else 8 + 4 * (s - 1),
                nk=4 if s == 0 else 2, N=192 - 32 * s, col0=32 * s, type=LOC_RDB if last else LOC_ACT, ecol=32 * s,
                out_slab=0 if last else 8 + 4 * s, rr=int(last and r == 3), beta=beta, first=int(s == 0)))
    passes.append(local_pass(w=pk["post_residual_conv_layer@trunk"][0].data_ptr(),
                             bias=P["post_residual_conv_layer/b"].data_ptr(), out_f32=out_f32, save=up2_out, slab0=0,
                             nk=4, N=64,
                             col0=0, type=LOC_POST, ecol=0, first=1))
    return np.ascontiguousarray(np.stack(passes))
PARTIAL_FLOATS = 9 * 32 * 128


def geometry(n: int, h: int, w: int) -> dict:
    out = (ctypes.c_int * 5)()
    ops.call("dbm_flat_geometry", n, h, w, ctypes.cast(out, ctypes.c_void_p))
    return dict(P=out[0], tiles=out[1], G0=out[2], Pg=out[3], R=out[4])


def geometry_host(n: int, h: int, w: int) -> dict:
    wp = w + 2
    P = n * (h + 2) * wp
    tiles = (P + 127) // 128
    halo = wp + 1
    g0 = (halo + 7) & ~7
    return dict(P=P, tiles=tiles, G0=g0, Pg=g0 + tiles * 128 + g0, R=128 + 2 * halo)


def split_blocks(tiles: int, nsplit: int):
    nsplit = max(1, min(nsplit, tiles))
    base, rem = divmod(tiles, nsplit)
    out, b = [], 0
    for s in range(nsplit):
        k = base + (1 if s < rem else 0)
        out.append((b, k))
        b += k
    return out


def s2d_tap_mask(c0: int, nch: int, C: int) -> int:
    mask = 0
    for ph in range(c0 // C, (c0 + nch - 1) // C + 1):
        py, px = ph >> 1, ph & 1
        for ky in ((1, 2) if py == 0 else (0, 1)):
            for kx in ((1, 2) if px == 0 else (0, 1)):
                mask |= 1 << (ky * 3 + kx)
    return mask


def chunk_channels(cin: int, chunk: int = 128):
    return [(c0, min(chunk, cin - c0)) for c0 in range(0, cin, chunk)]


def rdb_plan(nrdb: int, beta: float):
    plan = []
    for j in range(nrdb):
        r = j % 3 + 1
        sigma = beta if r == 3 else 1.0
        plan.append(dict(j=j, r=r, sigma=sigma, g5_scale=beta * sigma))
    return plan


class FlatTrunk:

    NSPLIT = 3

    def __init__(self, model, n: int, H: int, W: int):
        if model.inter_channels not in (32, 64):
            raise ValueError("the tensor-core training trunk implements inter_channels 32 or 64")
        self.model = model
        self.G = G = model.inter_channels
        self.cc = cc = 64 + 4 * G
        self.n, self.H, self.W = n, H, W
        self.geom = geometry(n, H, W)
        Pg = self.geom["Pg"]
        self.Pg = Pg
        nrdb = 3 * model.num_residual_blocks
        self.nrdb = nrdb
        bf = torch.bfloat16
        zb = lambda c: torch.zeros(c // 8, Pg, 8, dtype=bf, device="cuda")
        zf = lambda c: torch.zeros(c // 4, Pg, 4, dtype=torch.float32, device="cuda")
        self.s0 = zb(128)
        self.cat = [zb(cc) for _ in range(nrdb + 1)]
        self.gcat = [zb(cc) for _ in range(nrdb)]
        self.x0 = zf(64)
        self.xring = [zf(64) for _ in range(4)]
        self.a3f = zf(64)
        self.gpost, self.gpre = zb(64), zb(64)
        self.da3f = zf(64)
        self.dX = [zf(64) for _ in range(4)]
        self.dcat = zf(cc)
        self.da0f = zf(128)
        self._pack_gen = -1
        self._built_beta = None

    def _pb(self, t, c=0):
        return t.data_ptr() + 2 * c * self.Pg

    def _pf(self, t, c=0):
        return t.data_ptr() + 4 * c * self.Pg

    def _x(self, j):
        return self.x0 if j == 0 else self.xring[j % 4]

    @staticmethod
    def _epi(**kw):
        e = np.zeros((), dtype=EPI_DTYPE)
        e["s1"] = 1.0
        e["beta"] = 1.0
        e["beta2"] = 1.0
        e["out_scale"] = 1.0
        for k, v in kw.items():
            e[k] = v
        return e

    def _launches(self, inp_ptr, slices, cin, blocks):
        out = []
        for n0, width, img in slices:
            out.append(self._launch(inp_ptr, img, cin, width, blocks[n0 // 32:(n0 + width) // 32]))
        return out

    def _launch(self, inp_ptr, wq, cin, nout, blocks):
        L = np.zeros((), dtype=LAUNCH_DTYPE)
        L["in"] = inp_ptr
        L["wpacked"] = wq.data_ptr()
        L["cin"] = cin
        L["nout"] = nout
        L["ny"] = 1
        assert len(blocks) == nout // 32
        for b, e in enumerate(blocks):
            L["blk"][b] = e
        return L

    def build(self, pk):
        m = self.model
        beta = m.residual_scaling
        if self._pack_gen == m._pack_gen and self._built_beta == beta:
            return
        P, Gr = m.p, m.g
        G, cc = self.G, self.cc
        nrdb = self.nrdb
        pb, pf, epi = self._pb, self._pf, self._epi
        plan = rdb_plan(nrdb, beta)
        fwd, bwd = [], []
        convs = []

        wq, bq = pk["pre_residual_conv_layer@trunk"]
        fwd.append(self._launch(pb(self.s0), wq, 128, 64, [
            epi(bias=bq.data_ptr() + 128 * b, act=1, out_f32=pf(self.x0, 32 * b), out_bf16=pb(self.cat[0], 32 * b))
            for b in range(2)]))
        for d in plan:
            j, r = d["j"], d["r"]
            pre = m._rdb_prefix(j // 3, r)
            cat = self.cat[j]
            for k in (1, 2, 3, 4):
                cin = 64 + G * (k - 1)
                wq, bq = pk[f"{pre}/conv_layer{k}@trunk"]
                fwd.append(self._launch(pb(cat), wq, cin, G, [
                    epi(bias=bq.data_ptr() + 128 * b, act=1, out_bf16=pb(cat, cin + 32 * b)) for b in range(G // 32)]))
            wq, bq = pk[f"{pre}/conv_layer5@trunk"]
# ... 455 lines not shown
```

### deepbedmap_b200/model.py

```python
from __future__ import annotations

from collections import OrderedDict
from typing import Dict, Optional

import numpy as np
import torch

from . import layout, ops
from . import npz as npz_io


TRUNK_LAYER_DTYPE = np.dtype([("wpacked", "<u8"), ("bias", "<u8"), ("out_bf16", "<u8"), ("out_f32", "<u8"),
                              ("res1", "<u8"), ("res2", "<u8"), ("stash_out", "<u8"), ("cin", "<i4"), ("cout", "<i4"),
                              ("in_map", "<i4"), ("in_cs0", "<i4"), ("act", "<i4"), ("up2", "<i4"),
                              ("out_cs_total", "<i4"), ("out_cs0", "<i4"), ("cout_main", "<i4"),
                              ("res1_cs_total", "<i4"), ("beta", "<f4"), ("mode", "<i4"), ("pad", "<i4", (6,))])
assert TRUNK_LAYER_DTYPE.itemsize == 128
PACK_ENTRY_DTYPE = np.dtype([("w", "<u8"), ("out", "<u8"), ("O", "<i4"), ("o0", "<i4"), ("Cin", "<i4"),
                             ("CinTotal", "<i4"), ("c0", "<i4"), ("COUTP", "<i4"), ("CK", "<i4"), ("mode", "<i4")])
assert PACK_ENTRY_DTYPE.itemsize == 48


class Variable:

# ... 392 lines not shown
            for r in (3, 2, 1):
                j -= 1
                cat = cats[j]
                pre = self._rdb_prefix(i, r)
                d5 = ops.empty(n, 64, H, W)
                ops.axpby(d_rdb_out, 0, None, 0, d5, 0, 64, beta, 0.0)
                ops.conv2d_bwd_weight(cat, 0, cc, d5, 0, G[f"{pre}/conv_layer5/W"], 3, 1, 1, db=G[f"{pre}/conv_layer5/b"])
                dcat = ops.empty(n, cc, H, W)
                ops.conv2d_bwd_data(d5, 0, P[f"{pre}/conv_layer5/W"], dcat, 0, cc, 3, 1, 1)
                ops.axpby(dcat, 0, d_rdb_out, 0, dcat, 0, 64, 1.0, 1.0)
                for k in (4, 3, 2, 1):
                    cin = 64 + (k - 1) * g
                    ops.lrelu_bwd(dcat, cin, cat, cin, dcat, cin, g)
                    ops.conv2d_bwd_weight(cat, 0, cin, dcat, cin, G[f"{pre}/conv_layer{k}/W"], 3, 1, 1,
                                          db=G[f"{pre}/conv_layer{k}/b"])
                    ops.conv2d_bwd_data(dcat, cin, P[f"{pre}/conv_layer{k}/W"], dcat, 0, cin, 3, 1, 1, accumulate=True)
                d_rdb_out = ops.empty(n, 64, H, W)
                ops.axpby(dcat, 0, None, 0, d_rdb_out, 0, 64, 1.0, 0.0)
            dcur = ops.empty(n, 64, H, W)
            ops.axpby(d_rdb_out, 0, d_rrdb_out, 0, dcur, 0, 64, 1.0, 1.0)
            ready(f"residual_network/{i}/")
        da1 = ops.empty(n, 64, H, W)
        ops.axpby(dcur, 0, da3, 0, da1, 0, 64, 1.0, 1.0)
        ops.lrelu_bwd(da1, 0, cats[0], 0, da1, 0, 64)
        ops.conv2d_bwd_weight(c["a0"], 0, 128, da1, 0, G["pre_residual_conv_layer/W"], 3, 1, 1,
                              db=G["pre_residual_conv_layer/b"])
        da0 = ops.empty(n, 128, H, W)
        ops.conv2d_bwd_data(da1, 0, P["pre_residual_conv_layer/W"], da0, 0, 128, 3, 1, 1)
        self._stem_bwd(c, da0, ready)

    def _stem_bwd(self, c, da0, ready):
        G = self.g
        ops.conv2d_bwd_weight(c["x"], 0, 1, da0, 0, G["input_block/conv_on_X/W"], 3, 1, 0, db=G["input_block/conv_on_X/b"])
        ops.conv2d_bwd_weight(c["w1"], 0, 1, da0, 32, G["input_block/conv_on_W1/W"], 30, 10, 0,
                              db=G["input_block/conv_on_W1/b"])
        ops.conv2d_bwd_weight(c["w2"], 0, 2, da0, 64, G["input_block/conv_on_W2/W"], 6, 2, 0,
                              db=G["input_block/conv_on_W2/b"])
        ops.conv2d_bwd_weight(c["w3"], 0, 1, da0, 96, G["input_block/conv_on_W3/W"], 3, 1, 0,
                              db=G["input_block/conv_on_W3/b"])
        ready("input_block/", "pre_residual_conv_layer")
        self._ctx = None

    PACK_INFER = ("io", "trunk16", "infer", "deform")
    PACK_INFER_LOCAL = ("io", "stat", "infer", "deform")
    PACK_TRAIN_LOCAL = ("io", "stat", "dgrad", "deform")
    PACK_TRAIN_CHAIN = ("io", "trunk16", "stat", "dgrad", "deform")
    PACK_SPLIT = ("split",)

    def _pack(self, groups=None):
        if groups is None:
            groups = self.PACK_INFER
        P = self.p
        if self._pack_plan is None:
            pk = {}
            entries = {g: [] for g in ("io", "trunk16", "infer", "stat", "dgrad", "deform", "split")}
            pad_biases = []

            def image(cin, cout_padded):
                return ops.zeros(9 * cin * cout_padded, dtype=torch.bfloat16)

            def entry(grp, w, out, o, o0, cin, cin_total, c0, coutp, ck, mode=0):
                entries[grp].append((w.data_ptr(), out.data_ptr(), o, o0, cin, cin_total, c0, coutp, ck, mode))

            def add(key, cout_padded, trunk=None, ck=32, grp="infer"):
                w, b = P[f"{key}/W"], P[f"{key}/b"]
                o, cin = w.shape[0], w.shape[1]
                if b.numel() < cout_padded:
                    bp = ops.zeros(cout_padded)
                    pad_biases.append((bp, b))
                else:
                    bp = b
                img = image(cin, cout_padded)
                entry(grp, w, img, o, 0, cin, cin, 0, cout_padded, ck)
                pk[key] = (img, bp)
                if trunk is not None:
                    img16 = image(cin, cout_padded)
                    entry(trunk, w, img16, o, 0, cin, cin, 0, cout_padded, 16)
                    pk[key + "@trunk"] = (img16, bp)
                    if self.train_precision == "bf16":
                        slices = []
                        for c0 in range(0, cin, 192):
                            wdt = min(192, cin - c0)
                            imgd = image(wdt, o)
                            entry("dgrad", w, imgd, wdt, 0, o, cin, c0, wdt, 16, mode=1)
                            slices.append((c0, wdt, imgd))
                        if len(slices) == 1:
                            pk[key + "@dgrad"] = slices[0][2]
                        pk[key + "@dgrad_slices"] = slices

            add("pre_residual_conv_layer", 64, trunk="io")
            for i in range(self.num_residual_blocks):
                for r in (1, 2, 3):
                    pre = self._rdb_prefix(i, r)
                    for k in (1, 2, 3, 4):
                        add(f"{pre}/conv_layer{k}", self.inter_channels, trunk="trunk16")
                    add(f"{pre}/conv_layer5", 64, trunk="trunk16")
            add("post_residual_conv_layer", 64, trunk="io")
            if self.inter_channels == 32:
                for i in range(self.num_residual_blocks):
                    for r in (1, 2, 3):
                        pre = self._rdb_prefix(i, r)
                        for k in (1, 3):
                            cin = 64 + (k - 1) * 32
                            wa, wb = P[f"{pre}/conv_layer{k}/W"], P[f"{pre}/conv_layer{k + 1}/W"]
                            both = image(cin, 64)
                            entry("infer", wa, both, 32, 0, cin, cin, 0, 64, 16)
                            entry("infer", wb, both, 32, 32, cin, cin + 32, 0, 64, 16)
                            pk[f"{pre}/pair{k}"] = (both, P[f"{pre}/conv_layer{k}/b"])
                            tail = image(32, 32)
                            entry("infer", wb, tail, 32, 0, 32, cin + 32, cin, 32, 16)
                            pk[f"{pre}/tail{k + 1}"] = (tail, P[f"{pre}/conv_layer{k + 1}/b"])
                for i in range(self.num_residual_blocks):
                    for r in (1, 2, 3):
                        pre = self._rdb_prefix(i, r)
                        for s_ in range(5):
                            cblk, c0 = (64, 0) if s_ == 0 else (32, 64 + 32 * (s_ - 1))
                            ncol = 192 - 32 * s_
                            stat = image(cblk, ncol)
                            for k in range(s_ + 1, 6):
                                entry("stat", P[f"{pre}/conv_layer{k}/W"], stat, 64 if k == 5 else 32, 32 * (k - 1 - s_),
                                      cblk, 64 + 32 * (k - 1), c0, ncol, 16)
                            pk[f"{pre}/stat{s_}"] = stat
            if self.precision == "bf16x3":
                def add_split(name, slices, cin, coutp, bias):
                    img = ops.zeros(3 * 9 * cin * coutp, dtype=torch.bfloat16)
                    for wkey, o, o0, cin_total, c0 in slices:
                        entry("split", P[wkey], img, o, o0, cin, cin_total, c0, coutp, 16, mode=16)
                    pk[name + "@split"] = (img, bias)

                g_ = self.inter_channels
                for key in ("pre_residual_conv_layer", "post_residual_conv_layer", "post_upsample_conv_layer_1",
                            "post_upsample_conv_layer_2"):
                    w = P[f"{key}/W"]
                    add_split(key, [(f"{key}/W", w.shape[0], 0, w.shape[1], 0)], w.shape[1], 64, P[f"{key}/b"])
                for i in range(self.num_residual_blocks):
                    for r in (1, 2, 3):
                        pre = self._rdb_prefix(i, r)
                        add_split(f"{pre}/conv_layer5", [(f"{pre}/conv_layer5/W", 64, 0, 64 + 4 * g_, 0)], 64 + 4 * g_, 64,
                                  P[f"{pre}/conv_layer5/b"])
                        if g_ == 32:
                            for k in (1, 3):
                                cin = 64 + (k - 1) * 32
                                add_split(f"{pre}/pair{k}", [(f"{pre}/conv_layer{k}/W", 32, 0, cin, 0),
                                                             (f"{pre}/conv_layer{k + 1}/W", 32, 32, cin + 32, 0)], cin, 64,
                                          P[f"{pre}/conv_layer{k}/b"])
                                add_split(f"{pre}/tail{k + 1}", [(f"{pre}/conv_layer{k + 1}/W", 32, 0, cin + 32, cin)], 32,
                                          32, P[f"{pre}/conv_layer{k + 1}/b"])
                        else:
                            for k in (1, 2, 3, 4):
                                cin = 64 + (k - 1) * g_
                                add_split(f"{pre}/conv_layer{k}", [(f"{pre}/conv_layer{k}/W", g_, 0, cin, 0)], cin, g_,
                                          P[f"{pre}/conv_layer{k}/b"])
            for key in ("post_upsample_conv_layer_1", "post_upsample_conv_layer_2"):
                add(key, 64)
            add("final_conv_layer1/offset_conv", 32)
            add("final_conv_layer2/offset_conv", 32)
            add("final_conv_layer1/deform_conv", 64, ck=64, grp="deform")
            taps = {k: int(P[f"input_block/conv_on_{k}/W"][0].numel()) for k in ("X", "W1", "W2", "W3")}
            pk["stem"] = (ops.empty(taps["W1"], 32), ops.empty(taps["X"] + taps["W2"] + taps["W3"], 32), ops.empty(128))
            pk["stem_w1_tc"] = ops.empty(9 * 320 * 32, dtype=torch.bfloat16)
            tables = {}
            for g, ent in entries.items():
                if ent:
                    table = np.array(ent, dtype=PACK_ENTRY_DTYPE)
                    tables[g] = dict(table=torch.from_numpy(table.view(np.uint8).copy()).cuda(), n=len(ent),
                                     max_elements=max(9 * e[4] * e[7] for e in ent))
            self._pack_plan = dict(tables=tables, pad_biases=pad_biases, taps=taps)
            self._packed = pk
            self._pack_versions = {g: -1 for g in tables}
            self._pack_gen += 1
        plan, pk = self._pack_plan, self._packed
        for g in groups:
            t = plan["tables"].get(g)
            if t is None or self._pack_versions[g] == self.version:
                continue
            ops.call("dbm_pack_conv3x3_table", t["table"].data_ptr(), t["n"], t["max_elements"], ops.stream())
            if g == "infer":
                for bp, b in plan["pad_biases"]:
                    ops.axpby(b.view(1, b.numel(), 1, 1), 0, None, 0, bp.view(1, bp.numel(), 1, 1), 0, b.numel(), 1.0, 0.0)
                wt1, wts, bias128 = pk["stem"]
                r0 = 0
                for k, dst in (("W1", wt1), ("X", wts), ("W2", wts), ("W3", wts)):
                    nt = plan["taps"][k]
                    row = 0 if k == "W1" else r0
                    ops.call("dbm_transpose_f32", P[f"input_block/conv_on_{k}/W"].data_ptr(), dst[row:].data_ptr(), 32, nt,
                             ops.stream())
                    if k != "W1":
                        r0 += nt
                for j, k in enumerate(("X", "W1", "W2", "W3")):
                    ops.axpby(P[f"input_block/conv_on_{k}/b"].view(1, 32, 1, 1), 0, None, 0,
                              bias128.view(1, 128, 1, 1), 32 * j, 32, 1.0, 0.0)
                ops.call("dbm_pack_stem_w1", P["input_block/conv_on_W1/W"].data_ptr(), pk["stem_w1_tc"].data_ptr(),
                         ops.stream())
            self._pack_versions[g] = self.version
        return pk

    def _trunk_workspace(self, n, H, W):
        key = (n, H, W)
        ws = self._ws.get(key)
        pk = self._pack()
        if ws is not None and ws["version"] == (self._pack_gen, self.persistent_trunk, self.paired_trunk,
                                                self.per_layer_ck16, self.paired_convs):
            return ws
        bf = torch.bfloat16
        g = self.inter_channels
        cc = 64 + 4 * g
        ccs = cc // 8
        beta = self.residual_scaling
        paired = self.persistent_trunk and self.paired_trunk and g == 32 and (W + 15) // 16 + 2 <= 128
        if ws is None:
            ws = dict(s0=ops.empty(n, 16, H, W, 8, dtype=bf), cat=[ops.empty(n, ccs, H, W, 8, dtype=bf) for _ in range(2)],
                      a1_f32=ops.empty(n, 16, H, W, 4), f32=[ops.empty(n, 16, H, W, 4) for _ in range(3)],
                      u1=ops.empty(n, 8, 2 * H, 2 * W, 8, dtype=bf))
        cat, f32, a1_f32 = ws["cat"], ws["f32"], ws["a1_f32"]
        layers = []
        flops = []

        def layer(wkey, cin, cout, in_map, act=0, beta_=0.0, out=None, out_cs0=0, out_f32=None, res1=None, res2=None,
                  up2=0, in_cs0=0, cout_main=None, res1_cs=16, stash_out=None, raw=False, mode=0):
            trunk_pack = self.persistent_trunk or self.per_layer_ck16
            wq, bq = pk[wkey] if raw else (pk[wkey + "@trunk"] if trunk_pack else pk[wkey])
            ptr = lambda t: t.data_ptr() if t is not None else 0
            layers.append((wq.data_ptr(), bq.data_ptr(), ptr(out), ptr(out_f32), ptr(res1), ptr(res2), ptr(stash_out),
                           cin, cout, in_map, in_cs0, act, up2, out.shape[1] if out is not None else 0, out_cs0,
                           cout if cout_main is None else cout_main, res1_cs, beta_, mode, (0,) * 6))
            flops.append(2.0 * 9 * cin * cout * n * H * W)

        layer("pre_residual_conv_layer", 128, 64, 0, act=1, out=cat[0], out_f32=a1_f32)
        cur, cur_f32, fi = 0, a1_f32, 0
        for i in range(self.num_residual_blocks):
            rrdb_in = cur_f32
            for r in (1, 2, 3):
                pre = self._rdb_prefix(i, r)
                if paired:
                    for k in (1, 3):
                        cin = 64 + (k - 1) * g
                        if k not in self.paired_convs:
                            for kk in (k, k + 1):
                                ci = 64 + (kk - 1) * g
                                layer(f"{pre}/conv_layer{kk}", ci, g, 1 + cur, act=1, out=cat[cur], out_cs0=ci // 8)
                            continue
                        layer(f"{pre}/pair{k}", cin, 64, 1 + cur, act=1, out=cat[cur], out_cs0=cin // 8, cout_main=32,
                              raw=True, mode=1)
                        layer(f"{pre}/tail{k + 1}", 32, 32, 1 + cur, in_cs0=cin // 8, act=1, out=cat[cur],
                              out_cs0=cin // 8 + 4, raw=True, mode=2)
                else:
                    for k in (1, 2, 3, 4):
                        cin = 64 + (k - 1) * g
                        layer(f"{pre}/conv_layer{k}", cin, g, 1 + cur, act=1, out=cat[cur], out_cs0=cin // 8)
                while f32[fi] is cur_f32 or f32[fi] is rrdb_in:
                    fi = (fi + 1) % 3
                nxt_f32 = f32[fi]
                layer(f"{pre}/conv_layer5", cc, 64, 1 + cur, beta_=beta, out=cat[1 - cur], out_f32=nxt_f32, res1=cur_f32,
                      res2=rrdb_in if r == 3 else None)
                cur, cur_f32 = 1 - cur, nxt_f32
        layer("post_residual_conv_layer", 64, 64, 1 + cur, beta_=1.0, out=ws["u1"], res1=a1_f32, up2=1)
        table = np.array(layers, dtype=TRUNK_LAYER_DTYPE)
        ws["layers"] = layers
        ws["flops"] = float(sum(flops))
        ws["table"] = torch.from_numpy(table.view(np.uint8).copy()).cuda()
        tiles = ((H + 31) // 32) * ((W + 15) // 16)
        ws["flags"] = ops.empty(len(layers) * n * tiles, dtype=torch.int32)
        ws["version"] = (self._pack_gen, self.persistent_trunk, self.paired_trunk, self.per_layer_ck16, self.paired_convs)
        self._ws[key] = ws
        return ws

    def _run_trunk(self, ws, n, H, W):
        if self.persistent_trunk:
            ops.call("dbm_trunk_umma", ws["table"].data_ptr(), len(ws["layers"]), n, H, W, ws["s0"].data_ptr(), 16,
                     ws["cat"][0].data_ptr(), ws["cat"][1].data_ptr(), ws["cat"][0].shape[1], ws["flags"].data_ptr(),
                     ops.stream())
            return
        srcs = (ws["s0"], ws["cat"][0], ws["cat"][1])
        ops.call("dbm_debug_set", 2, int(self.per_layer_ck16))
        for (wq, bq, out, out_f32, res1, res2, _stash, cin, cout, in_map, _cs0, act, up2, out_cs_total, out_cs0, _cm,
             _r1cs, beta_, _mode, _pad) in ws["layers"]:
            inp = srcs[in_map]
            ops.call("dbm_conv3x3_umma", inp.data_ptr(), inp.shape[1], cin, wq, bq, cout, n, H, W, float(beta_), act, up2,
                     out or None, out_cs_total, out_cs0, out_f32 or None, 16, 0, res1 or None, res2 or None, ops.stream())
        ops.call("dbm_debug_set", 2, 0)

    def _local_workspace(self, n, H, W, pk):
        from . import flat
        key = ("local", n, H, W)
        ws = self._ws.get(key)
        if ws is None or ws["version"] != (self._pack_gen, self.residual_scaling):
            geom = flat.geometry(n, H, W)
            if ws is None:
                ws = dict(s0=torch.zeros(16, geom["Pg"], 8, dtype=torch.bfloat16, device="cuda"),
                          x=torch.empty(2, n * 16 * 128 * 4, dtype=torch.float32, device="cuda"),
                          u1=ops.empty(n, 8, 2 * H, 2 * W, 8, dtype=torch.bfloat16))
            tab = flat.local_forward_table(self, pk, 3 * self.num_residual_blocks, self.residual_scaling,
                                           up2_out=ws["u1"].data_ptr())
            ws["table"] = torch.from_numpy(tab.view(np.uint8).reshape(-1).copy()).cuda()
            ws["count"] = len(tab)
            ws["version"] = (self._pack_gen, self.residual_scaling)
            self._ws[key] = ws
        return ws

    def _c_forward_applies(self):
        return (self.c_model_api and self.persistent_trunk and self.paired_trunk and self.paired_convs == (1, 3)
                and not self.per_layer_ck16
                and self.stem_w1_tensor_core and not self.fuse_out_projection and self.out_channels == 1)

    def _forward_c_api(self, x, w1, w2, w3):
        import ctypes
        n, _, h, w = x.shape
        if self._cgen is None or self._cgen[1] != self.residual_scaling:
            self._c_release()
            hnd = ctypes.c_void_p()
            ops.call("dbm_gen_create", self.num_residual_blocks, float(self.residual_scaling), self.inter_channels,
                     ctypes.byref(hnd))
            ops.call("dbm_gen_bind_params", hnd, self.flat.data_ptr())
            ops.call("dbm_gen_set_precision", hnd, 1 if self.precision == "bf16x3" else 0)
            self._cgen, self._cgen_version = (hnd, self.residual_scaling), -1
        hnd = self._cgen[0]
        if self._cgen_version != self.version:
            ops.call("dbm_gen_mark_updated", hnd)
            self._cgen_version = self.version
        ws = self._cgen_ws.get((n, h, w))
        if ws is None:
            from . import _lib
            nbytes = int(_lib.load().dbm_gen_workspace_bytes(hnd, n, h, w))
            buf = torch.empty(nbytes + 1024, dtype=torch.uint8, device="cuda")
            ptr = (buf.data_ptr() + 1023) & ~1023
            ws = self._cgen_ws[(n, h, w)] = (buf, ptr, nbytes)
        y = ops.empty(n, 1, 4 * (h - 2), 4 * (w - 2))
        ops.call("dbm_gen_forward", hnd, x.data_ptr(), w1.data_ptr(), w2.data_ptr(), w3.data_ptr(), n, h, w,
                 y.data_ptr(), ws[1], ws[2], ops.stream())
        return y

    def _c_release(self):
        if getattr(self, "_cgen", None) is not None:
            try:
                torch.cuda.synchronize()
                ops.call("dbm_gen_destroy", self._cgen[0])
            except Exception:
                pass
            self._cgen, self._cgen_ws = None, {}

    def __del__(self):
        self._c_release()

    def _split_workspace(self, n, H, W, pk):
        key = ("split", n, H, W)
        ws = self._ws.get(key)
        if ws is not None and ws["version"] == (self._pack_gen, self.residual_scaling):
            return ws
        bf = torch.bfloat16
        g = self.inter_channels
        cc = 64 + 4 * g
        ccs = cc // 8
        beta = self.residual_scaling
        if ws is None:
            ws = dict(s0=ops.empty(n, 32, H, W, 8, dtype=bf), cat=[ops.empty(n, 2 * ccs, H, W, 8, dtype=bf) for _ in range(2)],
                      a1_f32=ops.empty(n, 16, H, W, 4), f32=[ops.empty(n, 16, H, W, 4) for _ in range(3)],
                      u1=ops.empty(n, 16, 2 * H, 2 * W, 8, dtype=bf), u2=ops.empty(n, 16, 4 * H, 4 * W, 8, dtype=bf),
                      c2f=ops.empty(n, 16, 4 * H, 4 * W, 4))
        cat, f32, a1_f32 = ws["cat"], ws["f32"], ws["a1_f32"]
        paired = g == 32 and (W + 15) // 16 + 2 <= 128

        def rec(wkey, cin, cout, in_map, act=0, beta_=0.0, out=None, out_cs0=0, out_f32=None, res1=None, res2=None,
                up2=0, in_cs0=0, cout_main=None, mode=0):
            wq, bq = pk[wkey + "@split"]
            ptr = lambda t: t.data_ptr() if t is not None else 0
            return (wq.data_ptr(), bq.data_ptr(), ptr(out), ptr(out_f32), ptr(res1), ptr(res2), 0, cin, cout, in_map,
                    in_cs0, act, up2, out.shape[1] // 2 if out is not None else 0, out_cs0,
                    cout if cout_main is None else cout_main, 16, beta_, mode, (0,) * 6)

        layers = [rec("pre_residual_conv_layer", 128, 64, 0, act=1, out=cat[0], out_f32=a1_f32)]
        cur, cur_f32, fi = 0, a1_f32, 0
        for i in range(self.num_residual_blocks):
            rrdb_in = cur_f32
            for r in (1, 2, 3):
                pre = self._rdb_prefix(i, r)
                if paired:
                    for k in (1, 3):
                        cin = 64 + (k - 1) * g
                        layers.append(rec(f"{pre}/pair{k}", cin, 64, 1 + cur, act=1, out=cat[cur], out_cs0=cin // 8,
                                          cout_main=32, mode=1))
                        layers.append(rec(f"{pre}/tail{k + 1}", 32, 32, 1 + cur, in_cs0=cin // 8, act=1, out=cat[cur],
                                          out_cs0=cin // 8 + 4, mode=2))
                else:
                    if g == 32:
                        raise ValueError("precision='bf16x3': tiles wider than ~2000 px are not supported")
                    for k in (1, 2, 3, 4):
                        cin = 64 + (k - 1) * g
                        layers.append(rec(f"{pre}/conv_layer{k}", cin, g, 1 + cur, act=1, out=cat[cur], out_cs0=cin // 8))
                while f32[fi] is cur_f32 or f32[fi] is rrdb_in:
                    fi = (fi + 1) % 3
                nxt_f32 = f32[fi]
                layers.append(rec(f"{pre}/conv_layer5", cc, 64, 1 + cur, beta_=beta, out=cat[1 - cur], out_f32=nxt_f32,
                                  res1=cur_f32, res2=rrdb_in if r == 3 else None))
                cur, cur_f32 = 1 - cur, nxt_f32
        layers.append(rec("post_residual_conv_layer", 64, 64, 1 + cur, beta_=1.0, out=ws["u1"], res1=a1_f32, up2=1))
        up1 = [rec("post_upsample_conv_layer_1", 64, 64, 0, act=1, out=ws["u2"], up2=1)]
        up2 = [rec("post_upsample_conv_layer_2", 64, 64, 0, act=1, out_f32=ws["c2f"])]
        dev = lambda rows: torch.from_numpy(np.array(rows, dtype=TRUNK_LAYER_DTYPE).view(np.uint8).copy()).cuda()
        units = lambda h_, w_: n * ((h_ + 31) // 32) * ((w_ + 15) // 16)
        ws.update(tables=[dev(layers), dev(up1), dev(up2)], counts=[len(layers), 1, 1],
                  flags=[ops.empty(len(layers) * units(H, W), dtype=torch.int32),
                         ops.empty(units(2 * H, 2 * W), dtype=torch.int32), ops.empty(units(4 * H, 4 * W), dtype=torch.int32)],
                  version=(self._pack_gen, self.residual_scaling))
        self._ws[key] = ws
        return ws

    def _forward_split(self, x, w1, w2, w3):
        n, _, h, w = x.shape
        H, W = h - 2, w - 2
        if self.c_model_api and self.out_channels == 1:
            return self._forward_c_api(x, w1, w2, w3)
        pk = self._pack(self.PACK_SPLIT)
        ws = self._split_workspace(n, H, W, pk)
        st = ops.stream()
        a0 = ops.empty(n, 128, H, W)
        self._stem_fp32(x, w1, w2, w3, a0)
        ops.call("dbm_nchw_to_slab8_split", a0.data_ptr(), 0, ws["s0"].data_ptr(), n, 128, H, W, st)
        del a0
        cat = ws["cat"]
        t, c, f = ws["tables"], ws["counts"], ws["flags"]
        ops.call("dbm_trunk_umma_split", t[0].data_ptr(), c[0], n, H, W, ws["s0"].data_ptr(), 16, cat[0].data_ptr(),
                 cat[1].data_ptr(), cat[0].shape[1] // 2, f[0].data_ptr(), st)
        u1, u2 = ws["u1"], ws["u2"]
        ops.call("dbm_trunk_umma_split", t[1].data_ptr(), 1, n, 2 * H, 2 * W, u1.data_ptr(), 8, u1.data_ptr(),
                 u1.data_ptr(), 8, f[1].data_ptr(), st)
        ops.call("dbm_trunk_umma_split", t[2].data_ptr(), 1, n, 4 * H, 4 * W, u2.data_ptr(), 8, u2.data_ptr(),
                 u2.data_ptr(), 8, f[2].data_ptr(), st)
        P = self.p
        y = ops.empty(n, self.out_channels, 4 * H, 4 * W)
        c2 = ops.empty(1, 64, 4 * H, 4 * W)
        per = 64 * 16 * H * W
        for i in range(n):
            ops.call("dbm_slab8f_to_nchw", ws["c2f"].data_ptr() + 4 * per * i, c2.data_ptr(), 0, 1, 64, 4 * H, 4 * W, st)
            y[i:i + 1].copy_(self._deform_head_fp32(c2))
        return y

    def _deform_head_fp32(self, c2):
        P = self.p
        n = c2.shape[0]

        def conv(key, x_):
            wt = P[f"{key}/W"]
            out = ops.empty(n, wt.shape[0], x_.shape[2], x_.shape[3])
            ops.conv2d_fwd(x_, 0, 64, wt, P[f"{key}/b"], out, 0, 3, 1, 1, act=False)
            return out

        off1 = conv("final_conv_layer1/offset_conv", c2)
        d1, _ = ops.deform_conv_fwd(c2, off1, P["final_conv_layer1/deform_conv/W"], P["final_conv_layer1/deform_conv/b"],
                                    act=True, tc=False)
        del _
        off2 = conv("final_conv_layer2/offset_conv", d1)
        if self.out_channels == 1:
            y, _ = ops.deform1_conv_fwd(d1, off2, P["final_conv_layer2/deform_conv/W"], P["final_conv_layer2/deform_conv/b"])
        else:
            y, _ = ops.deform_conv_fwd(d1, off2, P["final_conv_layer2/deform_conv/W"], P["final_conv_layer2/deform_conv/b"],
                                       act=False)
        return y

    def _forward_bf16(self, x, w1, w2, w3):
        from . import flat
        P = self.p
        n, _, h, w = x.shape
        H, W = h - 2, w - 2
        bf = torch.bfloat16
        local = self.local_trunk and self.inter_channels == 32 and flat.local_trunk_fits(H, W)
        chain = self.local_trunk and self.inter_channels != 32 and flat.local_trunk_fits(H, W)
        if not local and not chain and self._c_forward_applies():
            return self._forward_c_api(x, w1, w2, w3)
        pk = self._pack(self.PACK_INFER_LOCAL if local else self.PACK_INFER)
        wt1, wts, bias128 = pk["stem"]
        if chain:
            fc = self._ws.get(("chain", n, H, W))
            if fc is None:
                fc = self._ws[("chain", n, H, W)] = flat.FlatChainForward(self, n, H, W)
            fc.build(pk)
            ops.call("dbm_stem_fwd_flat", x.data_ptr(), w1.data_ptr(), w2.data_ptr(), w3.data_ptr(), wt1.data_ptr(),
                     wts.data_ptr(), bias128.data_ptr(), fc.s0.data_ptr(), n, h, w, ops.stream())
            a3 = fc.forward()
            u1 = ops.empty(n, 8, 2 * H, 2 * W, 8, dtype=bf)
            ops.nchw_to_slab8(ops.upsample2_fwd(a3), u1)
            ws = dict(u1=u1)
        elif local:
            ws = self._local_workspace(n, H, W, pk)
            ops.call("dbm_stem_fwd_flat", x.data_ptr(), w1.data_ptr(), w2.data_ptr(), w3.data_ptr(), wt1.data_ptr(),
                     wts.data_ptr(), bias128.data_ptr(), ws["s0"].data_ptr(), n, h, w, ops.stream())
            ops.call("dbm_trunk_local_fwd", ws["table"].data_ptr(), ws["count"], n, H, W, ws["s0"].data_ptr(),
                     ws["x"][0].data_ptr(), ws["x"][1].data_ptr(), ops.stream())
        else:
            ws = self._trunk_workspace(n, H, W)
            if self.stem_w1_tensor_core:
                s2d = ops.empty(n, 40, h, w, 8, dtype=bf)
                ops.call("dbm_stem_w1_s2d", w1.data_ptr(), s2d.data_ptr(), n, h, w, ops.stream())
                ops.call("dbm_stem_fwd_slab8", x.data_ptr(), None, w2.data_ptr(), w3.data_ptr(), None,
                         wts.data_ptr(), bias128.data_ptr(), ws["s0"].data_ptr(), 16, 0, n, h, w, ops.stream())
                ops.call("dbm_conv3x3_umma_valid", s2d.data_ptr(), 40, 320, pk["stem_w1_tc"].data_ptr(),
                         P["input_block/conv_on_W1/b"].data_ptr(), n, h, w, ws["s0"].data_ptr(), 16, 4, ops.stream())
                del s2d
            else:
                ops.call("dbm_stem_fwd_slab8", x.data_ptr(), w1.data_ptr(), w2.data_ptr(), w3.data_ptr(), wt1.data_ptr(),
                         wts.data_ptr(), bias128.data_ptr(), ws["s0"].data_ptr(), 16, 0, n, h, w, ops.stream())
            self._run_trunk(ws, n, H, W)
        u1 = ws["u1"]
        u2 = ops.empty(n, 8, 4 * H, 4 * W, 8, dtype=bf)
        wq, bq = pk["post_upsample_conv_layer_1"]
        ops.conv3x3_umma(u1, 64, wq, bq, 64, act=True, up2=True, out=u2)
        f1 = ops.empty(n, 8, 4 * H, 4 * W, 8, dtype=bf)
        wq, bq = pk["post_upsample_conv_layer_2"]
        ops.conv3x3_umma(u2, 64, wq, bq, 64, act=True, out=f1)
        del u2
        off_s = ops.empty(n, 8, 4 * H, 4 * W, 4)
        wq, bq = pk["final_conv_layer1/offset_conv"]
        ops.conv3x3_umma(f1, 64, wq, bq, 32, out_f32=off_s)
        d1 = ops.empty(n, 8, 4 * H, 4 * W, 8, dtype=bf)
        wq, bq = pk["final_conv_layer1/deform_conv"]
        if self.out_channels != 1:
            raise ValueError("the tensor-core path implements out_channels == 1 (the reference's only use)")
        proj = ops.deform_conv_umma(f1, off_s, wq, bq, d1, act=True,
                                    next_out1_w=P["final_conv_layer2/deform_conv/W"] if self.fuse_out_projection else None)
        del f1
        wq, bq = pk["final_conv_layer2/offset_conv"]
        ops.conv3x3_umma(d1, 64, wq, bq, 32, out_f32=off_s)
        if proj is not None:
            return ops.deform_out1_sample(proj, off_s, P["final_conv_layer2/deform_conv/b"])
        return ops.deform_conv_out1(d1, off_s, P["final_conv_layer2/deform_conv/W"],
                                    P["final_conv_layer2/deform_conv/b"])


class DiscriminatorModel(_Link):

    BN_EPS = 1e-5
    BN_DECAY = 0.9

    def __init__(self, *, precision: str = "bf16", seed: int = 1, init_scale: float = 0.1):
        if precision not in ("bf16", "fp32"):
            raise ValueError("precision must be 'bf16' or 'fp32'")
        self.precision = precision
        self._tc_images, self._tc, self._tc_packed_version, self._tc_pack_table = None, {}, -1, None
        self._slot = 0
        shapes = layout.discriminator_shapes()
        super().__init__(shapes, layout.init_values(shapes, seed, init_scale))
        self.persistent = OrderedDict()
        for k, shp in layout.discriminator_persistents().items():
            self.persistent[k] = ops.zeros(*shp)
            if k.endswith("avg_var"):
                ops.fill(self.persistent[k], 1.0)
        self.bn_N = {i: 0 for i in range(1, 10)}
        self.train = True
        self._ctx = None

    def load_npz(self, file, strict: bool = True):
        npz_io.load_npz(file, self, strict=strict)
        return self

    def save_npz(self, file, compression: bool = True):
        npz_io.save_npz(file, self, compression=compression)

    def __call__(self, x, train: Optional[bool] = None):
        return self.forward(x, train=train)

    def forward(self, x, train: Optional[bool] = None, save: bool = False, groups: int = 1) -> Variable:
        train = self.train if train is None else bool(train)
        x = as_device(x)
        if x.dim() != 4 or tuple(x.shape[1:]) != (1, 36, 36):
            raise ValueError(f"DiscriminatorModel expects (N,1,36,36) input, got {tuple(x.shape)}")
        P = self.p
        n = x.shape[0]
        if groups < 1 or n % groups:
            raise ValueError(f"batch of {n} does not split into {groups} groups")
        ng = n // groups
        acts = [x]
        pres = []
        a = ops.empty(n, 64, 36, 36)
        ops.conv2d_fwd(x, 0, 1, P["conv_layer0/W"], P["conv_layer0/b"], a, 0, 3, 1, 1, act=True)
        acts.append(a)
        stats = []
        hcur = 36
        cin = 64
        tc = self._tc_convs(n) if self.precision == "bf16" else None
        slot = 2
        if save:
            slot = self._slot
            self._slot ^= 1
        for i in range(1, 10):
            cout, k, s = layout.DISC_CONVS[i]
            ho, _ = ops.conv_out_hw(hcur, hcur, k, s, 1)
            if tc is not None:
                z = tc[i].forward(acts[-1], slot)
            else:
                z = ops.empty(n, cout, ho, ho)
                ops.conv2d_fwd(acts[-1], 0, cin, P[f"conv_layer{i}/W"], None, z, 0, k, s, 1)
            y = ops.empty(n, cout, ho, ho)
            mean, invstd = ops.empty(groups, cout), ops.empty(groups, cout)
            ops.call("dbm_bn_lrelu_fwd_groups_f32", z.data_ptr(), y.data_ptr(), P[f"batch_norm{i}/gamma"].data_ptr(),
                     P[f"batch_norm{i}/beta"].data_ptr(), self.persistent[f"batch_norm{i}/avg_mean"].data_ptr(),
                     self.persistent[f"batch_norm{i}/avg_var"].data_ptr(), mean.data_ptr(), invstd.data_ptr(), groups, ng,
                     cout, ho * ho, self.BN_EPS, self.BN_DECAY, int(train), ops.stream())
            pres.append(z)
            stats.append((mean, invstd))
            acts.append(y)
            hcur, cin = ho, cout
        flat = acts[-1].view(n, 512)
        l1 = ops.empty(n, 100)
        ops.gemm(flat, 512, 1, 0, P["linear_1/W"], 1, 512, 0, l1, 100, 1, 0, P["linear_1/b"], n, 100, 512, act=True)
        out = ops.empty(n, 1)
        ops.gemm(l1, 100, 1, 0, P["linear_2/W"], 1, 100, 0, out, 1, 1, 0, P["linear_2/b"], n, 1, 100)
        if save:
            if not train:
                raise ValueError("backward through eval-mode BatchNormalization is not needed by the reference")
            self._ctx = dict(acts=acts, pres=pres, stats=stats, l1=l1, n=n, tc=tc, slot=slot, groups=groups)
        return Variable(out)

    def _tc_convs(self, n):
        from . import flat
        if self._tc_images is None:
            self._tc_images = {i: flat.ConvImages(self.p[f"conv_layer{i}/W"]) for i in range(1, 10)}
        if self._tc_packed_version != self.version:
            self._tc_pack_table = flat.pack_images(list(self._tc_images.values()), self._tc_pack_table)
            self._tc_packed_version = self.version
        tc = self._tc.get(n)
        if tc is None:
            tc, h = {}, 36
            for i in range(1, 10):
                _, k, s = layout.DISC_CONVS[i]
                tc[i] = flat.FlatConv(self._tc_images[i], self.g[f"conv_layer{i}/W"], n, h, h, nslots=3)
                h = ops.conv_out_hw(h, h, k, s, 1)[0]
            self._tc[n] = tc
        return tc

    def backward(self, dlogit: torch.Tensor, on_ready=None):
        if self._ctx is None:
            raise RuntimeError("backward() needs a preceding forward(save=True)")
        ready = (lambda *pre: on_ready(*self.grad_range(pre))) if on_ready is not None else (lambda *pre: None)
        c = self._ctx
        P, G = self.p, self.g
        n = c["n"]
        acts, pres, stats, l1 = c["acts"], c["pres"], c["stats"], c["l1"]
        dlogit = dlogit.contiguous()
        ops.gemm(dlogit, 1, 1, 0, l1, 100, 1, 0, G["linear_2/W"], 100, 1, 0, None, 1, 100, n, accumulate=1)
        ops.call("dbm_bias_grad_f32", dlogit.data_ptr(), 1, G["linear_2/b"].data_ptr(), n, 1, 1, ops.stream())
        dl1 = ops.empty(n, 100)
        ops.gemm(dlogit, 1, 1, 0, P["linear_2/W"], 100, 1, 0, dl1, 100, 1, 0, None, n, 100, 1)
        ops.lrelu_bwd(dl1, 0, l1, 0, dl1, 0, 100)
        flat = acts[-1].view(n, 512)
        ops.gemm(dl1, 1, 100, 0, flat, 512, 1, 0, G["linear_1/W"], 512, 1, 0, None, 100, 512, n, accumulate=1)
        ops.call("dbm_bias_grad_f32", dl1.data_ptr(), 100, G["linear_1/b"].data_ptr(), n, 100, 1, ops.stream())
        dflat = ops.empty(n, 512, 1, 1)
        ops.gemm(dl1, 100, 1, 0, P["linear_1/W"], 512, 1, 0, dflat, 512, 1, 0, None, n, 512, 100)
        dy = dflat
        cur = torch.cuda.current_stream()
        wg = ops._aux_stream2() if c.get("tc") is not None else None
        for i in range(9, 0, -1):
            cout, k, s = layout.DISC_CONVS[i]
            z, y = pres[i - 1], acts[i + 1]
            mean, invstd = stats[i - 1]
            hw = z.shape[2] * z.shape[3]
            dz = ops.empty(*z.shape)
            groups = c.get("groups", 1)
            ng = n // groups
            scratch = ops.empty(groups, 2 * cout)
            ops.call("dbm_bn_lrelu_bwd_groups_f32", z.data_ptr(), y.data_ptr(), dy.data_ptr(), dz.data_ptr(),
                     P[f"batch_norm{i}/gamma"].data_ptr(), mean.data_ptr(), invstd.data_ptr(),
# ... 28 lines not shown
```

### deepbedmap_b200/ops.py

```python
from __future__ import annotations

import torch

from . import _lib

call = _lib.call


_AUX = None
_AUX2 = None


def _aux_stream2():
    global _AUX2
    if _AUX2 is None:
        _AUX2 = torch.cuda.Stream()
    return _AUX2


def _aux_stream():
    global _AUX
    if _AUX is None:
        _AUX = torch.cuda.Stream()
    return _AUX
# ... 21 lines not shown
    if dtype == torch.float32:
        fill(t, 0.0)
    else:
        n32 = t.numel() * t.element_size() // 4
        call("dbm_fill_f32", t.data_ptr(), 0.0, n32, stream())
    return t


def fill(t, v: float):
    _chk(t)
    call("dbm_fill_f32", t.data_ptr(), float(v), t.numel(), stream())


def conv_out_hw(h, w, k, s, p):
    return (h + 2 * p - k) // s + 1, (w + 2 * p - k) // s + 1


def conv2d_fwd(x, x_c0, cin, w, b, y, y_c0, k, s, p, act=False):
    n, cx, h, wd = x.shape
    o = w.shape[0]
    ho, wo = conv_out_hw(h, wd, k, s, p)
    assert y.shape[0] == n and y.shape[2] == ho and y.shape[3] == wo, (x.shape, y.shape)
    assert w.shape[1] == cin and x_c0 + cin <= cx and y_c0 + o <= y.shape[1]
    call("dbm_conv2d_fwd_f32", _ptr(x, x_c0 * h * wd), cx * h * wd, w.data_ptr(), b.data_ptr() if b is not None else None,
         _ptr(y, y_c0 * ho * wo), y.shape[1] * ho * wo, n, cin, h, wd, o, k, s, p, int(act), stream())


def conv2d_bwd_data(dy, dy_c0, w, dx, dx_c0, cin, k, s, p, accumulate=False):
    n, cdx, h, wd = dx.shape
    o = w.shape[0]
    ho, wo = dy.shape[2], dy.shape[3]
    call("dbm_conv2d_bwd_data_f32", _ptr(dy, dy_c0 * ho * wo), dy.shape[1] * ho * wo, w.data_ptr(),
         _ptr(dx, dx_c0 * h * wd), cdx * h * wd, n, cin, h, wd, o, k, s, p, int(accumulate), stream())


def conv2d_bwd_weight(x, x_c0, cin, dy, dy_c0, dw, k, s, p, db=None):
    n, cx, h, wd = x.shape
    o = dw.shape[0]
    ho, wo = dy.shape[2], dy.shape[3]
    call("dbm_conv2d_bwd_weight_f32", _ptr(x, x_c0 * h * wd), cx * h * wd, _ptr(dy, dy_c0 * ho * wo),
         dy.shape[1] * ho * wo, dw.data_ptr(), n, cin, h, wd, o, k, s, p, stream())
    if db is not None:
        call("dbm_bias_grad_f32", _ptr(dy, dy_c0 * ho * wo), dy.shape[1] * ho * wo, db.data_ptr(), n, o, ho * wo, stream())


def gemm(a, lda_m, lda_k, a_bs, b, ldb_k, ldb_n, b_bs, c, ldc_m, ldc_n, c_bs, bias, m, n, k, batch=1, act=False,
         accumulate=0, tc=False):
    call("dbm_gemm_bf16" if tc else "dbm_gemm_f32", a.data_ptr(), lda_m, lda_k, a_bs, b.data_ptr(), ldb_k, ldb_n, b_bs, c.data_ptr(), ldc_m,
         ldc_n, c_bs, bias.data_ptr() if bias is not None else None, m, n, k, batch, int(act), accumulate, stream())


def axpby(x, x_c0, y, y_c0, out, out_c0, channels, a, b):
    n = x.shape[0]
    hw = x.shape[2] * x.shape[3]
    call("dbm_axpby_f32", _ptr(x, x_c0 * hw), x.shape[1] * hw, _ptr(y, y_c0 * hw) if y is not None else None,
         (y.shape[1] * hw) if y is not None else 0, _ptr(out, out_c0 * hw), out.shape[1] * hw, float(a), float(b), n,
         channels * hw, stream())


def lrelu_bwd(dy, dy_c0, y, y_c0, dx, dx_c0, channels, accumulate=False):
    n = dy.shape[0]
    hw = dy.shape[2] * dy.shape[3] if dy.dim() == 4 else 1
    call("dbm_lrelu_bwd_f32", _ptr(dy, dy_c0 * hw), dy.shape[1] * hw, _ptr(y, y_c0 * hw), y.shape[1] * hw,
         _ptr(dx, dx_c0 * hw), dx.shape[1] * hw, n, channels * hw, int(accumulate), stream())


def upsample2_fwd(x):
    n, c, h, w = x.shape
    y = empty(n, c, 2 * h, 2 * w)
    call("dbm_upsample2_fwd_f32", x.data_ptr(), y.data_ptr(), n * c, h, w, stream())
    return y


def upsample2_bwd(dy):
    n, c, h2, w2 = dy.shape
    dx = empty(n, c, h2 // 2, w2 // 2)
    call("dbm_upsample2_bwd_f32", dy.data_ptr(), dx.data_ptr(), n * c, h2 // 2, w2 // 2, stream())
    return dx


def nchw_to_slab8(src, dst, dst_cs0=0):
    n, c, h, w = src.shape
    call("dbm_nchw_to_slab8", src.data_ptr(), 0, dst.data_ptr(), n, c, h, w, dst.shape[1], dst_cs0, stream())


def slab8_to_nchw(src, c, src_cs0=0):
    n, cs, h, w, _ = src.shape
    dst = empty(n, c, h, w)
    call("dbm_slab8_to_nchw", src.data_ptr(), cs, src_cs0, dst.data_ptr(), 0, n, c, h, w, stream())
    return dst


def nchw_to_slab4(src):
    n, c, h, w = src.shape
    dst = empty(n, c // 4, h, w, 4)
    call("dbm_nchw_to_slab4", src.data_ptr(), 0, dst.data_ptr(), n, c, h, w, stream())
    return dst


def slab4_to_nchw(src, c_keep):
    n, cs, h, w, _ = src.shape
    dst = empty(n, c_keep, h, w)
    call("dbm_slab4_to_nchw", src.data_ptr(), dst.data_ptr(), 0, n, cs * 4, c_keep, h, w, stream())
    return dst


def pack_conv3x3(w, cout_padded, ck=32):
    o, cin = w.shape[0], w.shape[1]
    packed = empty(9 * cin * cout_padded, dtype=torch.bfloat16)
    call("dbm_pack_conv3x3_weights", w.data_ptr(), packed.data_ptr(), o, cin, cout_padded, ck, stream())
    return packed


def deform_conv_umma(x_s8, off_s4, wpacked, bias, out_s8, act=False, out_cs0=0, next_out1_w=None):
    n, cs, h, w, _ = x_s8.shape
    assert cs == 8, "deform_conv_umma needs 64 input channels"
    proj = None
    if next_out1_w is not None:
        assert tuple(next_out1_w.shape) == (1, 64, 3, 3)
        proj = empty(n, 9, h, w)
    call("dbm_deform_conv_umma", x_s8.data_ptr(), off_s4.data_ptr(), off_s4.shape[1], wpacked.data_ptr(),
         bias.data_ptr(), n, h, w, int(act), out_s8.data_ptr(), out_s8.shape[1], out_cs0,
         next_out1_w.data_ptr() if proj is not None else None, proj.data_ptr() if proj is not None else None, stream())
    return proj


def deform_out1_sample(proj, off_s4, bias):
    n, _, h, wd = proj.shape
    y = empty(n, 1, h, wd)
    call("dbm_deform_out1_sample", proj.data_ptr(), off_s4.data_ptr(), off_s4.shape[1], bias.data_ptr(), y.data_ptr(),
         n, h, wd, stream())
    return y


def deform_conv_out1(x_s8, off_s4, w, bias):
    n, cs, h, wd, _ = x_s8.shape
    assert cs == 8 and tuple(w.shape) == (1, 64, 3, 3)
    y = empty(n, 1, h, wd)
    proj = empty(n, 9, h, wd)
    call("dbm_deform_conv_out1", x_s8.data_ptr(), off_s4.data_ptr(), off_s4.shape[1], w.data_ptr(), bias.data_ptr(),
         y.data_ptr(), proj.data_ptr(), n, h, wd, stream())
    return y


def conv3x3_umma(inp, cin, wpacked, bias, cout_padded, *, beta=0.0, act=False, up2=False, out=None, out_cs0=0,
                 out_f32=None, out_f32_cs0=0, res1=None, res2=None):
    n, cs, h, w, _ = inp.shape
    call("dbm_conv3x3_umma", inp.data_ptr(), cs, cin, wpacked.data_ptr(), bias.data_ptr(), cout_padded, n, h, w,
         float(beta), int(act), int(up2),
         out.data_ptr() if out is not None else None, out.shape[1] if out is not None else 0, out_cs0,
         out_f32.data_ptr() if out_f32 is not None else None, out_f32.shape[1] if out_f32 is not None else 0,
         out_f32_cs0, res1.data_ptr() if res1 is not None else None, res2.data_ptr() if res2 is not None else None,
         stream())


def deform_sample(x, offset):
    n, c, h, wd = x.shape
    cols = empty(n, c * 9, h * wd)
    call("dbm_deform_sample_f32", x.data_ptr(), offset.data_ptr(), cols.data_ptr(), n, c, h, wd, stream())
    return cols


def deform_sample_slab8(x8, offset):
    n, _, h, wd, _ = x8.shape
    cols = empty(n, 576, h * wd)
    call("dbm_deform_sample_slab8_f32", x8.data_ptr(), offset.data_ptr(), cols.data_ptr(), n, h, wd, stream())
    return cols


def deform_conv_fwd_fused(x, offset, wpacked_ck64, b, act=False, keep_slab8=False):
    n, c, h, wd = x.shape
    assert c == 64 and tuple(offset.shape) == (n, 18, h, wd)
    x8 = empty(n, 8, h, wd, 8, dtype=torch.bfloat16)
    nchw_to_slab8(x, x8)
    y = empty(n, 64, h, wd)
    call("dbm_deform_conv_umma_nchw", x8.data_ptr(), offset.data_ptr(), wpacked_ck64.data_ptr(), b.data_ptr(), n, h, wd,
         int(act), y.data_ptr(), stream())
    return (y, x8) if keep_slab8 else y


def deform_conv_fwd(x, offset, w, b, act=False, tc=False):
    n, c, h, wd = x.shape
    o = w.shape[0]
    hw = h * wd
    cols = empty(n, c * 9, hw)
    call("dbm_deform_sample_f32", x.data_ptr(), offset.data_ptr(), cols.data_ptr(), n, c, h, wd, stream())
    y = empty(n, o, h, wd)
    k = c * 9
    gemm(cols, 1, hw, k * hw, w, 1, k, 0, y, 1, hw, o * hw, b, hw, o, k, batch=n, act=act, tc=tc)
    return y, cols


def deform_conv_bwd(x, offset, w, cols, dy, dw, db, dx, tc=False):
    n, c, h, wd = x.shape
    o = w.shape[0]
    hw = h * wd
    k = c * 9
    cur, aux = torch.cuda.current_stream(), _aux_stream()
    aux.wait_stream(cur)
    with torch.cuda.stream(aux):
        gemm(dy, hw, 1, o * hw, cols, 1, hw, k * hw, dw, k, 1, 0, None, o, k, hw, batch=n, accumulate=2, tc=tc)
        call("dbm_bias_grad_f32", dy.data_ptr(), o * hw, db.data_ptr(), n, o, hw, stream())
    dcols = empty(n, k, hw)
    gemm(dy, 1, hw, o * hw, w, k, 1, 0, dcols, 1, hw, k * hw, None, hw, k, o, batch=n, tc=tc)
    doff = empty(n, 18, h, wd)
    call("dbm_deform_bwd_f32", x.data_ptr(), offset.data_ptr(), dcols.data_ptr(),
         dx.data_ptr() if dx is not None else None, doff.data_ptr(), n, c, h, wd, stream())
    cur.wait_stream(aux)
    return doff


def deform1_conv_fwd(x, offset, w, b):
    n, c, h, wd = x.shape
    assert tuple(w.shape) == (1, c, 3, 3)
    y = empty(n, 1, h, wd)
    proj = empty(n, 9, h, wd)
    call("dbm_deform1_fwd_f32", x.data_ptr(), offset.data_ptr(), w.data_ptr(), b.data_ptr(), y.data_ptr(),
         proj.data_ptr(), n, c, h, wd, stream())
    return y, proj


def deform1_conv_bwd(x, offset, w, proj, dy, dw, db, dx, accumulate_dx=False):
    n, c, h, wd = x.shape
    hw = h * wd
    call("dbm_bias_grad_f32", dy.data_ptr(), hw, db.data_ptr(), n, 1, hw, stream())
    doff = empty(n, 18, h, wd)
    scratch = empty(n, 9, h, wd)
    call("dbm_deform1_bwd_f32", x.data_ptr(), offset.data_ptr(), w.data_ptr(), proj.data_ptr(), dy.data_ptr(),
         dw.data_ptr(), dx.data_ptr() if dx is not None else None, int(accumulate_dx), doff.data_ptr(),
         scratch.data_ptr(), n, c, h, wd, stream())
    return doff
```

### include/deepbedmap_b200.h

```cpp
#ifndef DEEPBEDMAP_B200_H_
#define DEEPBEDMAP_B200_H_

#include <stddef.h>
#include <stdint.h>

#ifdef __cplusplus
extern "C" {
#endif

#ifndef __CUDA_RUNTIME_H__
typedef struct CUstream_st* cudaStream_t;
#endif

#define DBM_OK 0
#define DBM_ERR_INVALID (-1)
#define DBM_ERR_CUDA (-2)

int dbm_version(void);
long dbm_launch_count(void);
const char* dbm_last_error(void);
int dbm_set_deterministic(int on);
int dbm_set_sm_reserve(int n);

int dbm_conv2d_fwd_f32(const float* x, long x_batch_stride, const float* w, const float* bias, float* y,
                       long y_batch_stride, int n, int c, int h, int wd, int o, int ksize, int stride, int pad,
                       int act, cudaStream_t stream);
int dbm_conv2d_bwd_data_f32(const float* dy, long y_batch_stride, const float* w, float* dx, long x_batch_stride,
                            int n, int c, int h, int wd, int o, int ksize, int stride, int pad, int accumulate,
                            cudaStream_t stream);
int dbm_conv2d_bwd_weight_f32(const float* x, long x_batch_stride, const float* dy, long y_batch_stride, float* dw,
                              int n, int c, int h, int wd, int o, int ksize, int stride, int pad,
                              cudaStream_t stream);
int dbm_bias_grad_f32(const float* dy, long dy_batch_stride, float* db, int n, int o, int hw, cudaStream_t stream);

int dbm_gemm_f32(const float* a, long lda_m, long lda_k, long a_batch_stride, const float* b, long ldb_k, long ldb_n,
                 long b_batch_stride, float* c, long ldc_m, long ldc_n, long c_batch_stride, const float* bias, int m,
                 int n, int k, int batch, int act, int accumulate, cudaStream_t stream);
int dbm_gemm_bf16(const float* a, long lda_m, long lda_k, long a_batch_stride, const float* b, long ldb_k, long ldb_n,
                  long b_batch_stride, float* c, long ldc_m, long ldc_n, long c_batch_stride, const float* bias, int m,
                  int n, int k, int batch, int act, int accumulate, cudaStream_t stream);

int dbm_axpby_f32(const float* x, long x_bs, const float* y, long y_bs, float* out, long out_bs, float a, float b,
                  int nbatch, long inner, cudaStream_t stream);
int dbm_lrelu_fwd_f32(const float* x, float* y, long total, cudaStream_t stream);
int dbm_lrelu_bwd_f32(const float* dy, long dy_bs, const float* y, long y_bs, float* dx, long dx_bs, int nbatch,
                      long inner, int accumulate, cudaStream_t stream);
int dbm_upsample2_fwd_f32(const float* x, float* y, long planes, int h, int w, cudaStream_t stream);
int dbm_upsample2_bwd_f32(const float* dy, float* dx, long planes, int h, int w, cudaStream_t stream);
int dbm_fill_f32(float* p, float v, long n, cudaStream_t stream);
int dbm_nchw_to_slab8(const float* src, long src_batch_stride, void* dst_slab8, int n, int c, int h, int w,
                      int dst_cs_total, int dst_cs0, cudaStream_t stream);
int dbm_slab8_to_nchw(const void* src_slab8, int src_cs_total, int src_cs0, float* dst, long dst_batch_stride, int n,
                      int c, int h, int w, cudaStream_t stream);
int dbm_nchw_to_slab4(const float* src, long src_batch_stride, float* dst_slab4, int n, int c, int h, int w,
                      cudaStream_t stream);
int dbm_slab4_to_nchw(const float* src_slab4, float* dst, long dst_batch_stride, int n, int c_slab, int c_keep, int h,
                      int w, cudaStream_t stream);
int dbm_nchw_to_slab8_split(const float* src, long src_batch_stride, void* dst_slab8_split, int n, int c, int h, int w,
                            cudaStream_t stream);
int dbm_slab8f_to_nchw(const float* src_slab8f, float* dst, long dst_batch_stride, int n, int c, int h, int w,
                       cudaStream_t stream);

int dbm_pack_conv3x3_weights(const float* w_oihw, void* packed_bf16, int cout, int cin, int cout_padded, int ck,
                             cudaStream_t stream);
int dbm_pack_conv3x3_weights_slice(const float* w_oihw, int w_cin_total, int w_c0, void* packed_bf16, int cout,
                                   int cout0, int cin, int cout_padded, int ck, cudaStream_t stream);
int dbm_pack_conv3x3_table(const void* table_dev, int num_entries, long max_elements, cudaStream_t stream);
int dbm_conv3x3_umma(const void* in_slab8, int in_cs_total, int cin, const void* wpacked, const float* bias,
                     int cout_padded, int n, int h, int w, float beta, int act, int up2, void* out_slab8,
                     int out_cs_total, int out_cs0, float* out_f32_slab4, int out_f32_cs_total, int out_f32_cs0,
                     const float* res1_slab4, const float* res2_slab4, cudaStream_t stream);

int dbm_trunk_umma(const void* layers_dev, int num_layers, int n, int h, int w, const void* stem_slab8,
                   int stem_cs_total, const void* cat_a_slab8, const void* cat_b_slab8, int cat_cs_total,
                   unsigned int* flags_dev, cudaStream_t stream);
int dbm_trunk_umma_split(const void* layers_dev, int num_layers, int n, int h, int w, const void* stem_slab8,
                         int stem_cs_total, const void* cat_a_slab8, const void* cat_b_slab8, int cat_cs_total,
                         unsigned int* flags_dev, cudaStream_t stream);

int dbm_flat_geometry(int n, int h, int w, int* out5_host);
int dbm_flat_conv3x3_seq(const void* launches_host, int count, int n, int h, int w, int out_h, int out_w,
                         cudaStream_t stream);
int dbm_flat_conv3x3_chain(const void* launches_host, const void* launches_dev, int count, int n, int h, int w,
                           int out_h, int out_w, void* flags_dev, cudaStream_t stream);
int dbm_trunk_local_fwd(const void* passes_dev, int count, int n, int h, int w, const void* s0_flat,
                        float* x0_scratch, float* xrr_scratch, cudaStream_t stream);
int dbm_trunk_local_bwd(const void* passes_dev, int count, int n, int h, int w, const void* gpost_flat,
                        float* dxrr_scratch, cudaStream_t stream);
int dbm_flat_wgrad(const void* units_dev, int num_units, int n, int h, int w, cudaStream_t stream);
int dbm_flat_wgrad_ctas(const void* units_dev, int num_units, int n, int h, int w, int max_ctas, cudaStream_t stream);
int dbm_flat_wgrad_reduce(const void* entries_dev, int count, cudaStream_t stream);
int dbm_flat_bias_grad(const void* entries_dev, int count, int n, int h, int w, cudaStream_t stream);
int dbm_flat_from_nchw_ex(const float* src, int c, int src_h, int src_w, int mode, void* dst_slab8, float* dst_slab4,
                          float scale, int n, int h, int w, cudaStream_t stream);
int dbm_flat_to_nchw_ex(const float* src_slab4, const void* src_slab8, float* dst, int c, int dst_h, int dst_w, int mode,
                        int n, int h, int w, cudaStream_t stream);
int dbm_flat_from_nchw(const float* src, int c, void* dst_slab8, float* dst_slab4, float scale, int n, int h, int w,
                       cudaStream_t stream);
int dbm_flat_to_nchw(const float* src_slab4, const void* src_slab8, float* dst, int c, int n, int h, int w,
                     cudaStream_t stream);

int dbm_transpose_f32(const float* src, float* dst, int rows, int cols, cudaStream_t stream);
int dbm_stem_fwd_slab8(const float* x, const float* w1, const float* w2, const float* w3,
                       const float* w1_filter_tapmajor, const float* small_filters_tapmajor, const float* bias128,
                       void* out_slab8, int out_cs_total, int out_cs0, int n, int h, int w, cudaStream_t stream);
int dbm_stem_w1_s2d(const float* w1, void* s2d_slab8, int n, int h, int w, cudaStream_t stream);
int dbm_pack_stem_w1(const float* w1_filter, void* packed_bf16, cudaStream_t stream);
int dbm_conv3x3_umma_valid(const void* in_slab8, int in_cs_total, int cin, const void* wpacked, const float* bias,
                           int n, int h_in, int w_in, void* out_slab8, int out_cs_total, int out_cs0,
                           cudaStream_t stream);
int dbm_stem_fwd_flat(const float* x, const float* w1, const float* w2, const float* w3, const float* w1_filter_tapmajor,
                      const float* small_filters_tapmajor, const float* bias128, void* out_flat, int n, int h, int w,
                      cudaStream_t stream);

int dbm_deform_conv_umma(const void* x_slab8, const float* offset_slab4, int offset_cs_total,
                         const void* wpacked_ck64, const float* bias, int n, int h, int w, int act, void* out_slab8,
                         int out_cs_total, int out_cs0, const float* next_out1_filter, float* next_out1_proj,
                         cudaStream_t stream);
int dbm_deform_conv_umma_nchw(const void* x_slab8, const float* offset_nchw18, const void* wpacked_ck64,
                              const float* bias, int n, int h, int w, int act, float* out_nchw, cudaStream_t stream);
int dbm_deform_sample_slab8_f32(const void* x_slab8, const float* offset_nchw18, float* cols, int n, int h, int w,
                                cudaStream_t stream);
int dbm_deform_out1_sample(const float* proj, const float* offset_slab4, int offset_cs_total, const float* bias,
                           float* y, int n, int h, int w, cudaStream_t stream);
int dbm_deform_conv_out1(const void* x_slab8, const float* offset_slab4, int offset_cs_total, const float* w_f32,
                         const float* bias, float* y, float* proj_scratch, int n, int h, int w, cudaStream_t stream);

int dbm_deform_sample_f32(const float* x, const float* offset, float* cols, int n, int c, int h, int w,
                          cudaStream_t stream);
int dbm_deform_bwd_f32(const float* x, const float* offset, const float* dcols, float* dx, float* doffset, int n,
                       int c, int h, int w, cudaStream_t stream);

int dbm_deform1_fwd_f32(const float* x, const float* offset, const float* w, const float* bias, float* y, float* proj,
                        int n, int c, int h, int w_, cudaStream_t stream);
int dbm_deform1_bwd_f32(const float* x, const float* offset, const float* w, const float* proj, const float* dy,
                        float* dw, float* dx, int accumulate_dx, float* doffset, float* dproj_scratch, int n, int c,
                        int h, int w_, cudaStream_t stream);

int dbm_bn_lrelu_fwd_f32(const float* x, float* y, const float* gamma, const float* beta, float* avg_mean,
                         float* avg_var, float* save_mean, float* save_invstd, int n, int c, int hw, float eps,
                         float decay, int train, cudaStream_t stream);
int dbm_bn_lrelu_bwd_f32(const float* x, const float* y, const float* dy, float* dx, const float* gamma,
                         const float* save_mean, const float* save_invstd, float* dgamma, float* dbeta,
                         float* scratch2c, int n, int c, int hw, cudaStream_t stream);
int dbm_bn_lrelu_fwd_groups_f32(const float* x, float* y, const float* gamma, const float* beta, float* avg_mean,
                                float* avg_var, float* save_mean, float* save_invstd, int groups, int n, int c, int hw,
                                float eps, float decay, int train, cudaStream_t stream);
int dbm_bn_lrelu_bwd_groups_f32(const float* x, const float* y, const float* dy, float* dx, const float* gamma,
                                const float* save_mean, const float* save_invstd, float* dgamma, float* dbeta,
                                float* scratch, int groups, int n, int c, int hw, cudaStream_t stream);

int dbm_ragan_loss_f32(const float* real_pred, const float* fake_pred, int n, float t_real_minus_fake,
                       float t_fake_minus_real, float grad_scale, float* out2, float* d_real, float* d_fake,
                       cudaStream_t stream);
int dbm_gen_image_loss_f32(const float* y_pred, const float* y_true, const float* x_topo, int n, int h, int w,
                           float w_content, float w_topo, float w_struct, float* sums4, float* dy,
                           cudaStream_t stream);

int dbm_adam_step_f32(float* params, const float* grads, float* m, float* v, long n, float alpha, float beta1,
                      float beta2, float eps, int t, float grad_scale, cudaStream_t stream);
int dbm_adam_step_dev_f32(float* params, const float* grads, float* m, float* v, long n, float alpha, float beta1,
                          float beta2, float eps, int* t_dev, float grad_scale, cudaStream_t stream);

int dbm_crop_clip_f32(const float* src, int hs, int ws, float* dst, int c, int y0, int x0, int h, int w, int clip0,
                      cudaStream_t stream);
int dbm_place_tile_f32(const float* tile, int th, int tw, int cy, int cx, float* canvas, int ch, int cw, int ys,
                       int xs, int hh, int ww, cudaStream_t stream);

int dbm_f32_to_i16(const float* src, void* dst_i16, long n, cudaStream_t stream);

int dbm_copy2d_async(void* dst, size_t dst_pitch, const void* src, size_t src_pitch, size_t width_bytes, size_t rows,
                     cudaStream_t stream);

int dbm_gather_rows_f32(const float* src, long src_rows, const long* index_dev, float* dst, long row, int nrows,
                        cudaStream_t stream);

typedef struct dbm_gen dbm_gen;
int dbm_gen_create(int num_residual_blocks, float residual_scaling, int inter_channels, dbm_gen** out);
int dbm_gen_destroy(dbm_gen* gen);
long dbm_gen_count_params(const dbm_gen* gen);
int dbm_gen_num_arrays(const dbm_gen* gen);
int dbm_gen_array_info(const dbm_gen* gen, int index, const char** key, int* ndim, int* dims4, long* flat_offset);
int dbm_gen_set_param(dbm_gen* gen, const char* key, const float* host_values, int ndim, const int* dims);
int dbm_gen_bind_params(dbm_gen* gen, float* device_flat);
int dbm_gen_mark_updated(dbm_gen* gen);
int dbm_gen_set_precision(dbm_gen* gen, int precision);
size_t dbm_gen_workspace_bytes(const dbm_gen* gen, int n, int h, int w);
int dbm_gen_forward(dbm_gen* gen, const float* x, const float* w1, const float* w2, const float* w3, int n, int h,
                    int w, float* y_out, void* workspace, size_t workspace_bytes, cudaStream_t stream);

#ifdef __cplusplus
}
#endif
#endif
```

Measured before the change: 339.5.

## Fuse nearest-upsample into 3x3 conv via sub-pixel phase weights

Replaces the upsample-then-conv path for both post-upsample layers with a dedicated UMMA kernel. The kernel reads the low-resolution input and applies phase-decomposed weights, where 3x3 taps are summed per output sub-pixel phase and stored as a bf16 hi/lo pair. This removes the writes and reads of the 4x upsampled intermediate and cuts the MMA work per output pixel. The trunk head now writes u1 at low resolution. Pre-summing taps in bf16 with a hi/lo split changes rounding slightly, and the new kernel adds its own pipeline and TMEM scheduling logic.

```diff
diff --git a/deepbedmap_b200/_lib.py b/deepbedmap_b200/_lib.py
--- a/deepbedmap_b200/_lib.py
+++ b/deepbedmap_b200/_lib.py
@@ -62,6 +62,7 @@
     "dbm_deform_out1_sample": [_P, _P, _I, _P, _P, _I, _I, _I, _P],
     "dbm_deform_conv_out1": [_P, _P, _I, _P, _P, _P, _P, _I, _I, _I, _P],
     "dbm_conv3x3_umma": [_P, _I, _I, _P, _P, _I, _I, _I, _I, _F, _I, _I, _P, _I, _I, _P, _I, _I, _P, _P, _P],
+    "dbm_conv3x3_up2_umma": [_P, _P, _P, _I, _I, _I, _P, _P],
     "dbm_deform_sample_f32": [_P, _P, _P, _I, _I, _I, _I, _P],
     "dbm_deform_bwd_f32": [_P, _P, _P, _P, _P, _I, _I, _I, _I, _P],
     "dbm_deform1_fwd_f32": [_P, _P, _P, _P, _P, _P, _I, _I, _I, _I, _P],
diff --git a/deepbedmap_b200/build.py b/deepbedmap_b200/build.py
--- a/deepbedmap_b200/build.py
+++ b/deepbedmap_b200/build.py
@@ -13,7 +13,7 @@
 TUNING_LIB = os.path.join(HERE, "libdeepbedmap_b200_tuning.so")
 STAMP = os.path.join(HERE, "build", "stamp.txt")
 
-SOURCES = ["ops.cu", "gemm_f32.cu", "gemm_bf16.cu", "umma_conv3x3.cu", "umma_trunk.cu", "umma_flat.cu", "umma_local.cu", "umma_deform.cu", "stem.cu", "deform_f32.cu", "train_ops.cu", "gen_api.cu"]
+SOURCES = ["ops.cu", "gemm_f32.cu", "gemm_bf16.cu", "umma_conv3x3.cu", "umma_upconv.cu", "umma_trunk.cu", "umma_flat.cu", "umma_local.cu", "umma_deform.cu", "stem.cu", "deform_f32.cu", "train_ops.cu", "gen_api.cu"]
 TUNING_SOURCES = ["debug_bench.cu"]
 NVCC_FLAGS = [
     "-O3", "-std=c++17", "-gencode", "arch=compute_100a,code=sm_100a", "-lineinfo", "-Xcompiler", "-fPIC"]
diff --git a/deepbedmap_b200/csrc/common.cuh b/deepbedmap_b200/csrc/common.cuh
--- a/deepbedmap_b200/csrc/common.cuh
+++ b/deepbedmap_b200/csrc/common.cuh
@@ -118,6 +118,19 @@
       : "memory");
 }
 
+__device__ __forceinline__ uint4 pack8f(const float* v) {
+  uint4 o;
+  __nv_bfloat162 t0 = __floats2bfloat162_rn(v[0], v[1]);
+  __nv_bfloat162 t1 = __floats2bfloat162_rn(v[2], v[3]);
+  __nv_bfloat162 t2 = __floats2bfloat162_rn(v[4], v[5]);
+  __nv_bfloat162 t3 = __floats2bfloat162_rn(v[6], v[7]);
+  o.x = *reinterpret_cast<uint32_t*>(&t0);
+  o.y = *reinterpret_cast<uint32_t*>(&t1);
+  o.z = *reinterpret_cast<uint32_t*>(&t2);
+  o.w = *reinterpret_cast<uint32_t*>(&t3);
+  return o;
+}
+
 template <uint32_t kCols>
 __device__ __forceinline__ void tmem_alloc(uint32_t* dst_smem) {
   asm volatile("tcgen05.alloc.cta_group::1.sync.aligned.shared::cta.b32 [%0], %1;" ::"r"(
diff --git a/deepbedmap_b200/csrc/gen_api.cu b/deepbedmap_b200/csrc/gen_api.cu
--- a/deepbedmap_b200/csrc/gen_api.cu
+++ b/deepbedmap_b200/csrc/gen_api.cu
@@ -114,11 +114,11 @@
     return g->img[name];
   };
   auto entry = [&](const std::string& wkey, size_t img_off, int O, int o0, int cin, int cin_total, int c0, int coutp,
-                   int ck) {
+                   int ck, int mode = 0) {
     PackEntry e;
     e.w = P(g, wkey);
     e.out = (__nv_bfloat16*)img_off;
-    e.O = O; e.o0 = o0; e.Cin = cin; e.CinTotal = cin_total; e.c0 = c0; e.COUTP = coutp; e.CK = ck; e.mode = 0;
+    e.O = O; e.o0 = o0; e.Cin = cin; e.CinTotal = cin_total; e.c0 = c0; e.COUTP = coutp; e.CK = ck; e.mode = mode;
     ent.push_back(e);
   };
   const int ic = g->inter;
@@ -144,8 +144,12 @@
         }
     }
   entry("post_residual_conv_layer/W", image("post", 64, 64), 64, 0, 64, 64, 0, 64, 16);
-  entry("post_upsample_conv_layer_1/W", image("up1", 64, 64), 64, 0, 64, 64, 0, 64, 32);
-  entry("post_upsample_conv_layer_2/W", image("up2", 64, 64), 64, 0, 64, 64, 0, 64, 32);
+  for (int i = 1; i <= 2; ++i) {
+    const std::string name = "up" + std::to_string(i);
+    g->img[name] = off;
+    off += (size_t)2 * kUpPhaseBlocks * 64 * 64 * 2;
+    entry("post_upsample_conv_layer_" + std::to_string(i) + "/W", g->img[name], 64, 0, 64, 64, 0, 64, 16, 4);
+  }
   entry("final_conv_layer1/offset_conv/W", image("off1", 64, 32), 18, 0, 64, 64, 0, 32, 32);
   entry("final_conv_layer2/offset_conv/W", image("off2", 64, 32), 18, 0, 64, 64, 0, 32, 32);
   entry("final_conv_layer1/deform_conv/W", image("dc1", 64, 64), 64, 0, 64, 64, 0, 64, 64);
@@ -220,7 +224,7 @@
   L.cat[1] = take(px * ccs * 16);
   L.a1 = take(px * 64 * 4);
   for (int i = 0; i < 3; ++i) L.f32[i] = take(px * 64 * 4);
-  L.u1 = take(px * 4 * 8 * 16);
+  L.u1 = take(px * 8 * 16);
   L.u2 = take(px * 16 * 8 * 16);
   L.f1 = take(px * 16 * 8 * 16);
   L.offs = take(px * 16 * 8 * 16);
@@ -289,7 +293,7 @@
     }
   }
   layer(image("post"), P(g, "post_residual_conv_layer/b"), 64, 64, 1 + cur, 0, 1.f, bf(L.u1), 8, 0, nullptr, a1, nullptr,
-        1, 0, 64, 0);
+        0, 0, 64, 0);
 }
 
 static int build_split_pack_plan(Gen* g) {
@@ -702,11 +706,8 @@
   void* u2 = ws + L.u2;
   void* f1 = ws + L.f1;
   float* offs = (float*)(ws + L.offs);
-  if ((rc = dbm_conv3x3_umma(u1, 8, 64, image("up1"), P(g, "post_upsample_conv_layer_1/b"), 64, n, 2 * H, 2 * W, 0.f, 1, 1,
-                             u2, 8, 0, nullptr, 0, 0, nullptr, nullptr, st)))
-    return rc;
-  if ((rc = dbm_conv3x3_umma(u2, 8, 64, image("up2"), P(g, "post_upsample_conv_layer_2/b"), 64, n, 4 * H, 4 * W, 0.f, 1, 0,
-                             f1, 8, 0, nullptr, 0, 0, nullptr, nullptr, st)))
+  if ((rc = dbm_conv3x3_up2_umma(u1, image("up1"), P(g, "post_upsample_conv_layer_1/b"), n, H, W, u2, st))) return rc;
+  if ((rc = dbm_conv3x3_up2_umma(u2, image("up2"), P(g, "post_upsample_conv_layer_2/b"), n, 2 * H, 2 * W, f1, st)))
     return rc;
   if ((rc = dbm_conv3x3_umma(f1, 8, 64, image("off1"), (const float*)(g->arena + g->off_bias_off1), 32, n, 4 * H, 4 * W,
                              0.f, 0, 0, nullptr, 0, 0, offs, 8, 0, nullptr, nullptr, st)))
diff --git a/deepbedmap_b200/csrc/umma_common.cuh b/deepbedmap_b200/csrc/umma_common.cuh
--- a/deepbedmap_b200/csrc/umma_common.cuh
+++ b/deepbedmap_b200/csrc/umma_common.cuh
@@ -66,5 +66,10 @@
 };
 static_assert(sizeof(PackEntry) == 48, "PackEntry layout is part of the C ABI");
 
+constexpr int kUpPhaseBlocks = 14;
+__host__ __device__ constexpr uint32_t up_tap_mask(int p, int d) {
+  return ((p == 0 ? 0x061u : 0x430u) >> (4 * d)) & 15u;
+}
+
 
 }
diff --git a/deepbedmap_b200/csrc/umma_conv3x3.cu b/deepbedmap_b200/csrc/umma_conv3x3.cu
--- a/deepbedmap_b200/csrc/umma_conv3x3.cu
+++ b/deepbedmap_b200/csrc/umma_conv3x3.cu
@@ -303,6 +303,31 @@
   const bool split = (e.mode & 16) != 0;
   e.mode &= 15;
   if (split && !(e.mode == 0 && (e.O & 7) == 0 && (e.o0 & 7) == 0 && e.CK == 16)) return;
+  if (e.mode == 4) {
+    const int nrow = kUpPhaseBlocks * e.COUTP, nks = e.Cin / 8;
+    const long total = 2L * nks * nrow;
+    for (long i = blockIdx.x * (long)blockDim.x + threadIdx.x; i < total; i += (long)gridDim.x * blockDim.x) {
+      const int row = (int)(i % nrow), ksl = (int)((i / nrow) % nks), py = (int)(i / ((long)nrow * nks));
+      const int blk = row / e.COUTP, o = row - blk * e.COUTP;
+      const bool lo = blk >= 8;
+      const int b = lo ? blk - 8 : blk;
+      const int px = b & 1, dx = b < 4 ? 1 : 2 * px, dy = (b & 3) < 2 ? 1 : 2 * py;
+      const uint32_t my = up_tap_mask(py, dy), mx = up_tap_mask(px, dx);
+      float v[8];
+#pragma unroll
+      for (int c8 = 0; c8 < 8; ++c8) {
+        const float* src = e.w + ((long)o * e.CinTotal + e.c0 + ksl * 8 + c8) * 9;
+        float acc = 0.f;
+        for (int ky = 0; ky < 3; ++ky)
+          for (int kx = 0; kx < 3; ++kx)
+            if ((my >> ky) & (mx >> kx) & 1) acc += __bfloat162float(__float2bfloat16_rn(src[3 * ky + kx]));
+        const float hi = __bfloat162float(__float2bfloat16_rn(acc));
+        v[c8] = o >= e.O ? 0.f : lo ? acc - hi : acc;
+      }
+      store8_bf16(e.out + i * 8, v);
+    }
+    return;
+  }
   if (e.mode == 0 && (e.O & 7) == 0 && (e.o0 & 7) == 0) {
     const int og = e.O / 8;
     const long total = (long)9 * (e.Cin / 8) * e.O;
diff --git a/deepbedmap_b200/csrc/umma_local.cu b/deepbedmap_b200/csrc/umma_local.cu
--- a/deepbedmap_b200/csrc/umma_local.cu
+++ b/deepbedmap_b200/csrc/umma_local.cu
@@ -52,19 +52,6 @@
       : "memory");
 }
 __device__ __forceinline__ void tmem_wait_st() { asm volatile("tcgen05.wait::st.sync.aligned;" ::: "memory"); }
-
-__device__ __forceinline__ uint4 pack8f(const float* v) {
-  uint4 o;
-  __nv_bfloat162 t0 = __floats2bfloat162_rn(v[0], v[1]);
-  __nv_bfloat162 t1 = __floats2bfloat162_rn(v[2], v[3]);
-  __nv_bfloat162 t2 = __floats2bfloat162_rn(v[4], v[5]);
-  __nv_bfloat162 t3 = __floats2bfloat162_rn(v[6], v[7]);
-  o.x = *reinterpret_cast<uint32_t*>(&t0);
-  o.y = *reinterpret_cast<uint32_t*>(&t1);
-  o.z = *reinterpret_cast<uint32_t*>(&t2);
-  o.w = *reinterpret_cast<uint32_t*>(&t3);
-  return o;
-}
 
 template <bool BWD, bool SOLO>
 __global__ void __launch_bounds__(SOLO ? kLocSoloThreads : kLocThreads, SOLO ? 2 : 1)
@@ -354,17 +341,11 @@
                       make_float4(v[4 * c4], v[4 * c4 + 1], v[4 * c4 + 2], v[4 * c4 + 3]);
               }
               if (P.save != nullptr) {
-                const int Ho = 2 * p.H, Wo = 2 * p.W;
-#pragma unroll
-                for (int s8 = 0; s8 < 4; ++s8) {
-                  const uint4 o = pack8f(v + 8 * s8);
-                  __nv_bfloat16* base =
-                      P.save + ((((size_t)im * 8 + 4 * h + s8) * Ho + 2 * (y - 1)) * Wo + 2 * (x - 1)) * 8;
-                  *reinterpret_cast<uint4*>(base) = o;
-                  *reinterpret_cast<uint4*>(base + 8) = o;
-                  *reinterpret_cast<uint4*>(base + (size_t)Wo * 8) = o;
-                  *reinterpret_cast<uint4*>(base + (size_t)Wo * 8 + 8) = o;
-                }
+#pragma unroll
+                for (int s8 = 0; s8 < 4; ++s8)
+                  *reinterpret_cast<uint4*>(P.save +
+                                            ((((size_t)im * 8 + 4 * h + s8) * p.H + (y - 1)) * p.W + (x - 1)) * 8) =
+                      pack8f(v + 8 * s8);
               }
             }
             continue;
diff --git a/deepbedmap_b200/csrc/umma_upconv.cu b/deepbedmap_b200/csrc/umma_upconv.cu
--- /dev/null
+++ b/deepbedmap_b200/csrc/umma_upconv.cu
@@ -0,0 +1,204 @@
+#include "umma_common.cuh"
+
+namespace dbm {
+
+constexpr int kUpThreads = 320;
+constexpr int kUpTW = 8, kUpTH = 16;
+constexpr int kUpHW = kUpTW + 2, kUpHH = kUpTH + 2;
+constexpr int kUpStages = 4;
+constexpr int kUpA = kUpHW * kUpHH * 64 * 2;
+constexpr int kUpB = kUpPhaseBlocks * 64 * 64 * 2;
+constexpr int kUpALbo = kUpHW * kUpHH * 16;
+constexpr int kUpASbo = kUpHW * 16;
+constexpr int kUpBLbo = kUpPhaseBlocks * 64 * 16;
+constexpr int kUpBSbo = 128;
+constexpr int kUpSmem = kUpB + kUpStages * kUpA + 256 + 1024;
+
+struct UpConvParams {
+  int H, W;
+  int tiles_x, tiles_y, num_tiles;
+  const __nv_bfloat16* wphase;
+  const float* bias;
+  __nv_bfloat16* out;
+};
+
+template <int AOFF, int BLK, int SLOT, int NCOL>
+__device__ __forceinline__ void up_mma(uint32_t d0, uint32_t a_lo, uint32_t a_hi, uint32_t b_lo, uint32_t b_hi,
+                                       uint32_t acc) {
+  constexpr uint32_t idesc = umma_idesc_bf16(128, NCOL);
+  umma_bf16_off<(uint32_t)AOFF, (uint32_t)(BLK * 64)>(d0 + (uint32_t)(SLOT * 64), a_lo, a_hi, b_lo, b_hi, idesc, acc);
+}
+
+__device__ __forceinline__ void up_kstep(uint32_t d0, uint32_t a_c, uint32_t a_o, uint32_t a_hi, uint32_t b_lo,
+                                         uint32_t b_hi, uint32_t acc0) {
+  up_mma<kUpHW + 1, 0, 0, 128>(d0, a_c, a_hi, b_lo, b_hi, acc0);
+  up_mma<1, 2, 0, 128>(d0, a_o, a_hi, b_lo, b_hi, 1u);
+  up_mma<kUpHW + 0, 4, 0, 64>(d0, a_c, a_hi, b_lo, b_hi, 1u);
+  up_mma<kUpHW + 2, 5, 1, 64>(d0, a_c, a_hi, b_lo, b_hi, 1u);
+  up_mma<0, 6, 0, 64>(d0, a_o, a_hi, b_lo, b_hi, 1u);
+  up_mma<2, 7, 1, 64>(d0, a_o, a_hi, b_lo, b_hi, 1u);
+  up_mma<kUpHW + 1, 8, 0, 128>(d0, a_c, a_hi, b_lo, b_hi, 1u);
+  up_mma<1, 10, 0, 128>(d0, a_o, a_hi, b_lo, b_hi, 1u);
+  up_mma<kUpHW + 0, 12, 0, 64>(d0, a_c, a_hi, b_lo, b_hi, 1u);
+  up_mma<kUpHW + 2, 13, 1, 64>(d0, a_c, a_hi, b_lo, b_hi, 1u);
+}
+
+__global__ void __launch_bounds__(kUpThreads, 1)
+umma_upconv_kernel(const __grid_constant__ CUtensorMap tmap_in, const UpConvParams p) {
+  extern __shared__ uint8_t smem_raw[];
+  uint8_t* smem = (uint8_t*)(((uintptr_t)smem_raw + 1023) & ~(uintptr_t)1023);
+  uint8_t* smB = smem;
+  uint8_t* smA = smem + kUpB;
+  uint64_t* bars = (uint64_t*)(smA + kUpStages * kUpA);
+  uint64_t* full = bars;
+  uint64_t* empty = bars + kUpStages;
+  uint64_t* tfull = bars + 2 * kUpStages;
+  uint64_t* tempty = bars + 2 * kUpStages + 2;
+  uint64_t* wbar = bars + 2 * kUpStages + 4;
+  uint32_t* tmem_slot = (uint32_t*)(bars + 2 * kUpStages + 5);
+
+  const int warp = threadIdx.x >> 5;
+  const int lane = threadIdx.x & 31;
+  const int py = blockIdx.x & 1;
+  const int t0 = blockIdx.x >> 1, tstep = gridDim.x >> 1;
+  const int tiles_per_img = p.tiles_x * p.tiles_y;
+
+  if (warp == 0 && lane == 0) {
+    tma_prefetch_desc(&tmap_in);
+    for (int s = 0; s < kUpStages; ++s) {
+      mbar_init(&full[s], 1);
+      mbar_init(&empty[s], 1);
+    }
+    for (int b = 0; b < 2; ++b) {
+      mbar_init(&tfull[b], 1);
+      mbar_init(&tempty[b], 8);
+    }
+    mbar_init(wbar, 1);
+    fence_mbar_init();
+  }
+  if (warp == 1) tmem_alloc<256>(tmem_slot);
+  tc_fence_before();
+  __syncthreads();
+  tc_fence_after();
+  const uint32_t tmem_base = *tmem_slot;
+
+  if (warp == 0) {
+    if (lane == 0) {
+      mbar_arrive_expect_tx(wbar, kUpB);
+      const __nv_bfloat16* img = p.wphase + (size_t)py * (kUpB / 2);
+      for (int c = 0; c < 4; ++c) bulk_load(smB + c * (kUpB / 4), img + c * (kUpB / 8), kUpB / 4, wbar);
+      int s = 0;
+      uint32_t ph = 0;
+      for (int t = t0; t < p.num_tiles; t += tstep) {
+        const int n = t / tiles_per_img;
+        const int r = t - n * tiles_per_img;
+        const int ty = r / p.tiles_x, tx = r - ty * p.tiles_x;
+        mbar_wait(&empty[s], ph ^ 1);
+        mbar_arrive_expect_tx(&full[s], kUpA);
+        tma_load_4d(smA + s * kUpA, &tmap_in, &full[s], (tx * kUpTW - 1) * 8, ty * kUpTH - 1, 0, n);
+        if (++s == kUpStages) { s = 0; ph ^= 1; }
+      }
+    }
+  } else if (warp == 1) {
+    const uint32_t a_hi = desc_hi(kUpASbo), b_hi = desc_hi(kUpBSbo);
+    const uint32_t smA_u = smem_u32(smA);
+    const uint32_t b_lo = desc_lo(smem_u32(smB), kUpBLbo);
+    mbar_wait(wbar, 0);
+    tc_fence_after();
+    int s = 0;
+    uint32_t ph = 0;
+    int it = 0;
+    for (int t = t0; t < p.num_tiles; t += tstep, ++it) {
+      const int buf = it & 1;
+      mbar_wait(&tempty[buf], ((it >> 1) & 1) ^ 1);
+      tc_fence_after();
+      mbar_wait(&full[s], ph);
+      tc_fence_after();
+      const uint32_t d0 = tmem_base + (uint32_t)(buf * 128);
+      const uint32_t a_c = desc_lo(smA_u + s * kUpA, kUpALbo);
+      const uint32_t a_o = a_c + (uint32_t)(2 * py * kUpHW);
+      if (elect_one_sync()) {
+#pragma unroll
+        for (uint32_t ks = 0; ks < 4; ++ks)
+          up_kstep(d0, a_c + ks * (2 * kUpALbo / 16), a_o + ks * (2 * kUpALbo / 16), a_hi, b_lo + ks * (2 * kUpBLbo / 16),
+                   b_hi, ks != 0 ? 1u : 0u);
+        umma_commit(&empty[s]);
+        umma_commit(&tfull[buf]);
+      }
+      __syncwarp();
+      if (++s == kUpStages) { s = 0; ph ^= 1; }
+    }
+  } else {
+    const int q = warp & 3;
+    const int c0 = 32 * ((warp - 2) >> 2);
+    const int m = 32 * q + lane;
+    const int Ho = 2 * p.H, Wo = 2 * p.W;
+    int it = 0;
+    for (int t = t0; t < p.num_tiles; t += tstep, ++it) {
+      const int n = t / tiles_per_img;
+      const int r = t - n * tiles_per_img;
+      const int ty = r / p.tiles_x, tx = r - ty * p.tiles_x;
+      const int y = ty * kUpTH + (m >> 3), x = tx * kUpTW + (m & 7);
+      const bool valid = y < p.H && x < p.W;
+      const int buf = it & 1;
+      mbar_wait(&tfull[buf], (it >> 1) & 1);
+      tc_fence_after();
+      const uint32_t tb = tmem_base + ((uint32_t)(32 * q) << 16) + (uint32_t)(buf * 128 + c0);
+      uint32_t a0[32], a1[32];
+      tmem_ld_32x32b_x32(tb, a0);
+      tmem_ld_32x32b_x32(tb + 64, a1);
+      tmem_wait_ld();
+      tc_fence_before();
+      __syncwarp();
+      if (lane == 0) mbar_arrive(&tempty[buf]);
+      if (valid) {
+#pragma unroll
+        for (int s8 = 0; s8 < 4; ++s8) {
+          float v0[8], v1[8];
+#pragma unroll
+          for (int i = 0; i < 8; ++i) {
+            const float b = __ldg(p.bias + c0 + 8 * s8 + i);
+            v0[i] = lrelu(__uint_as_float(a0[8 * s8 + i]) + b);
+            v1[i] = lrelu(__uint_as_float(a1[8 * s8 + i]) + b);
+          }
+          const size_t cs = (size_t)n * 8 + c0 / 8 + s8;
+          __nv_bfloat16* dst = p.out + ((cs * Ho + 2 * y + py) * Wo + 2 * x) * 8;
+          *reinterpret_cast<uint4*>(dst) = pack8f(v0);
+          *reinterpret_cast<uint4*>(dst + 8) = pack8f(v1);
+        }
+      }
+    }
+  }
+
+  tc_fence_before();
+  __syncthreads();
+  if (warp == 1) {
+    tc_fence_after();
+    tmem_dealloc<256>(tmem_base);
+  }
+}
+
+}
+
+using namespace dbm;
+
+extern "C" int dbm_conv3x3_up2_umma(const void* in_slab8, const void* wphase, const float* bias, int n, int h, int w,
+                                    void* out_slab8, cudaStream_t stream) {
+  DBM_REQUIRE(n > 0 && h > 0 && w > 0, "conv3x3_up2_umma: empty input");
+  DBM_REQUIRE(in_slab8 && wphase && bias && out_slab8, "conv3x3_up2_umma: null argument");
+  DBM_REQUIRE(((uintptr_t)in_slab8 & 15) == 0 && ((uintptr_t)wphase & 15) == 0 && ((uintptr_t)out_slab8 & 15) == 0,
+              "conv3x3_up2_umma: unaligned");
+  CUtensorMap tm;
+  int rc = make_slab8_tmap(&tm, in_slab8, n, 8, h, w, 64, kUpHW, kUpHH);
+  if (rc) return rc;
+  UpConvParams p;
+  p.H = h; p.W = w;
+  p.tiles_x = ceil_div(w, kUpTW); p.tiles_y = ceil_div(h, kUpTH);
+  p.num_tiles = n * p.tiles_x * p.tiles_y;
+  p.wphase = (const __nv_bfloat16*)wphase; p.bias = bias; p.out = (__nv_bfloat16*)out_slab8;
+  if ((rc = ensure_dyn_smem((const void*)umma_upconv_kernel, kUpSmem))) return rc;
+  const int pairs = p.num_tiles < num_sms() / 2 ? p.num_tiles : num_sms() / 2;
+  const int grid = 2 * pairs;
+  umma_upconv_kernel<<<grid, kUpThreads, kUpSmem, stream>>>(tm, p);
+  return check_launch("umma_upconv_kernel");
+}
diff --git a/deepbedmap_b200/flat.py b/deepbedmap_b200/flat.py
--- a/deepbedmap_b200/flat.py
+++ b/deepbedmap_b200/flat.py
@@ -41,7 +41,7 @@
     return e
 
 
-def local_forward_table(model, pk, nrdb, beta, cat_ptr=None, out_f32=0, up2_out=0):
+def local_forward_table(model, pk, nrdb, beta, cat_ptr=None, out_f32=0, head_out=0):
     P = model.p
     save = (lambda j, c: cat_ptr(j, c)) if cat_ptr is not None else (lambda j, c: 0)
     passes = [local_pass(w=pk["pre_residual_conv_layer@trunk"][0].data_ptr(),
@@ -58,7 +58,7 @@
                 nk=4 if s == 0 else 2, N=192 - 32 * s, col0=32 * s, type=LOC_RDB if last else LOC_ACT, ecol=32 * s,
                 out_slab=0 if last else 8 + 4 * s, rr=int(last and r == 3), beta=beta, first=int(s == 0)))
     passes.append(local_pass(w=pk["post_residual_conv_layer@trunk"][0].data_ptr(),
-                             bias=P["post_residual_conv_layer/b"].data_ptr(), out_f32=out_f32, save=up2_out, slab0=0,
+                             bias=P["post_residual_conv_layer/b"].data_ptr(), out_f32=out_f32, save=head_out, slab0=0,
                              nk=4, N=64,
                              col0=0, type=LOC_POST, ecol=0, first=1))
     return np.ascontiguousarray(np.stack(passes))
diff --git a/deepbedmap_b200/model.py b/deepbedmap_b200/model.py
--- a/deepbedmap_b200/model.py
+++ b/deepbedmap_b200/model.py
@@ -568,7 +568,9 @@
                                 add_split(f"{pre}/conv_layer{k}", [(f"{pre}/conv_layer{k}/W", g_, 0, cin, 0)], cin, g_,
                                           P[f"{pre}/conv_layer{k}/b"])
             for key in ("post_upsample_conv_layer_1", "post_upsample_conv_layer_2"):
-                add(key, 64)
+                img = ops.zeros(ops.UP2_PHASE_IMAGE_ELEMENTS, dtype=torch.bfloat16)
+                entry("infer", P[f"{key}/W"], img, 64, 0, 64, 64, 0, 64, 16, mode=4)
+                pk[key] = (img, P[f"{key}/b"])
             add("final_conv_layer1/offset_conv", 32)
             add("final_conv_layer2/offset_conv", 32)
             add("final_conv_layer1/deform_conv", 64, ck=64, grp="deform")
@@ -627,7 +629,7 @@
         if ws is None:
             ws = dict(s0=ops.empty(n, 16, H, W, 8, dtype=bf), cat=[ops.empty(n, ccs, H, W, 8, dtype=bf) for _ in range(2)],
                       a1_f32=ops.empty(n, 16, H, W, 4), f32=[ops.empty(n, 16, H, W, 4) for _ in range(3)],
-                      u1=ops.empty(n, 8, 2 * H, 2 * W, 8, dtype=bf))
+                      u1=ops.empty(n, 8, H, W, 8, dtype=bf))
         cat, f32, a1_f32 = ws["cat"], ws["f32"], ws["a1_f32"]
         layers = []
         flops = []
@@ -670,7 +672,7 @@
                 layer(f"{pre}/conv_layer5", cc, 64, 1 + cur, beta_=beta, out=cat[1 - cur], out_f32=nxt_f32, res1=cur_f32,
                       res2=rrdb_in if r == 3 else None)
                 cur, cur_f32 = 1 - cur, nxt_f32
-        layer("post_residual_conv_layer", 64, 64, 1 + cur, beta_=1.0, out=ws["u1"], res1=a1_f32, up2=1)
+        layer("post_residual_conv_layer", 64, 64, 1 + cur, beta_=1.0, out=ws["u1"], res1=a1_f32)
         table = np.array(layers, dtype=TRUNK_LAYER_DTYPE)
         ws["layers"] = layers
         ws["flops"] = float(sum(flops))
@@ -705,9 +707,9 @@
             if ws is None:
                 ws = dict(s0=torch.zeros(16, geom["Pg"], 8, dtype=torch.bfloat16, device="cuda"),
                           x=torch.empty(2, n * 16 * 128 * 4, dtype=torch.float32, device="cuda"),
-                          u1=ops.empty(n, 8, 2 * H, 2 * W, 8, dtype=torch.bfloat16))
+                          u1=ops.empty(n, 8, H, W, 8, dtype=torch.bfloat16))
             tab = flat.local_forward_table(self, pk, 3 * self.num_residual_blocks, self.residual_scaling,
-                                           up2_out=ws["u1"].data_ptr())
+                                           head_out=ws["u1"].data_ptr())
             ws["table"] = torch.from_numpy(tab.view(np.uint8).reshape(-1).copy()).cuda()
             ws["count"] = len(tab)
             ws["version"] = (self._pack_gen, self.residual_scaling)
@@ -893,8 +895,8 @@
             ops.call("dbm_stem_fwd_flat", x.data_ptr(), w1.data_ptr(), w2.data_ptr(), w3.data_ptr(), wt1.data_ptr(),
                      wts.data_ptr(), bias128.data_ptr(), fc.s0.data_ptr(), n, h, w, ops.stream())
             a3 = fc.forward()
-            u1 = ops.empty(n, 8, 2 * H, 2 * W, 8, dtype=bf)
-            ops.nchw_to_slab8(ops.upsample2_fwd(a3), u1)
+            u1 = ops.empty(n, 8, H, W, 8, dtype=bf)
+            ops.nchw_to_slab8(a3, u1)
             ws = dict(u1=u1)
         elif local:
             ws = self._local_workspace(n, H, W, pk)
@@ -916,13 +918,10 @@
                 ops.call("dbm_stem_fwd_slab8", x.data_ptr(), w1.data_ptr(), w2.data_ptr(), w3.data_ptr(), wt1.data_ptr(),
                          wts.data_ptr(), bias128.data_ptr(), ws["s0"].data_ptr(), 16, 0, n, h, w, ops.stream())
             self._run_trunk(ws, n, H, W)
-        u1 = ws["u1"]
-        u2 = ops.empty(n, 8, 4 * H, 4 * W, 8, dtype=bf)
         wq, bq = pk["post_upsample_conv_layer_1"]
-        ops.conv3x3_umma(u1, 64, wq, bq, 64, act=True, up2=True, out=u2)
-        f1 = ops.empty(n, 8, 4 * H, 4 * W, 8, dtype=bf)
+        u2 = ops.conv3x3_up2_umma(ws["u1"], wq, bq)
         wq, bq = pk["post_upsample_conv_layer_2"]
-        ops.conv3x3_umma(u2, 64, wq, bq, 64, act=True, out=f1)
+        f1 = ops.conv3x3_up2_umma(u2, wq, bq)
         del u2
         off_s = ops.empty(n, 8, 4 * H, 4 * W, 4)
         wq, bq = pk["final_conv_layer1/offset_conv"]
diff --git a/deepbedmap_b200/ops.py b/deepbedmap_b200/ops.py
--- a/deepbedmap_b200/ops.py
+++ b/deepbedmap_b200/ops.py
@@ -197,6 +197,27 @@
          out_f32.data_ptr() if out_f32 is not None else None, out_f32.shape[1] if out_f32 is not None else 0,
          out_f32_cs0, res1.data_ptr() if res1 is not None else None, res2.data_ptr() if res2 is not None else None,
          stream())
+
+
+UP2_PHASE_IMAGE_ELEMENTS = 2 * 14 * 64 * 64
+
+
+def conv3x3_up2_umma(inp, wphase, bias, out=None):
+    n, cs, h, w, v = inp.shape
+    if cs != 8 or v != 8:
+        raise ValueError(f"conv3x3_up2_umma: input {tuple(inp.shape)} is not slab8 with 64 channels (N, 8, H, W, 8)")
+    for name, t, dtype, numel in (("input", inp, torch.bfloat16, inp.numel()),
+                                  ("phase image", wphase, torch.bfloat16, UP2_PHASE_IMAGE_ELEMENTS),
+                                  ("bias", bias, torch.float32, 64)):
+        if t.dtype != dtype or not t.is_cuda or not t.is_contiguous() or t.numel() != numel:
+            raise ValueError(f"conv3x3_up2_umma: {name} must be a contiguous CUDA {dtype} tensor of {numel} elements")
+    if out is None:
+        out = empty(n, 8, 2 * h, 2 * w, 8, dtype=torch.bfloat16)
+    elif (tuple(out.shape) != (n, 8, 2 * h, 2 * w, 8) or out.dtype != torch.bfloat16 or not out.is_cuda
+          or not out.is_contiguous()):
+        raise ValueError(f"conv3x3_up2_umma: out must be a contiguous CUDA bf16 tensor of shape {(n, 8, 2 * h, 2 * w, 8)}")
+    call("dbm_conv3x3_up2_umma", inp.data_ptr(), wphase.data_ptr(), bias.data_ptr(), n, h, w, out.data_ptr(), stream())
+    return out
 
 
 def deform_sample(x, offset):
diff --git a/include/deepbedmap_b200.h b/include/deepbedmap_b200.h
--- a/include/deepbedmap_b200.h
+++ b/include/deepbedmap_b200.h
@@ -70,6 +70,8 @@
                      int cout_padded, int n, int h, int w, float beta, int act, int up2, void* out_slab8,
                      int out_cs_total, int out_cs0, float* out_f32_slab4, int out_f32_cs_total, int out_f32_cs0,
                      const float* res1_slab4, const float* res2_slab4, cudaStream_t stream);
+int dbm_conv3x3_up2_umma(const void* in_slab8, const void* wphase, const float* bias, int n, int h, int w,
+                         void* out_slab8, cudaStream_t stream);
 
 int dbm_trunk_umma(const void* layers_dev, int num_layers, int n, int h, int w, const void* stem_slab8,
                    int stem_cs_total, const void* cat_a_slab8, const void* cat_b_slab8, int cat_cs_total,
```

After: 349.8, median of 6. 1.03x the previous value.
